# ucla-mobility/QuantV2X

Measured on AMD Instinct MI355X. Metric: frames/sec/node (N-agent int8 BEV fusion), higher is better.
Workload: dtype i8

## Files before the change

### include/qv2x.h

```cpp
#ifndef QV2X_H
#define QV2X_H

#include <stdint.h>

#ifdef __cplusplus
extern "C" {
#endif
#if defined(__GNUC__) || defined(__clang__)
#pragma GCC visibility push(default)
#endif

#define QV2X_OK 0
#define QV2X_EINVAL (-1)
#define QV2X_EALIGN (-2)
#define QV2X_MAX_GROUPS 4

const char* qv2x_last_error(void);
#define QV2X_ABI_VERSION 9
int qv2x_version(void);

int qv2x_fill_i8(int8_t* buf, int64_t bytes, int value, void* stream);

int64_t qv2x_voxelize_workspace_bytes(int n_points);
int qv2x_voxelize_f32(const float* points, int n_points, const float* lidar_range, const float* voxel_size, int agent,
                      int max_points, int max_voxels, void* workspace, int64_t workspace_bytes,
                      float* voxel_features, int32_t* voxel_coords, int32_t* voxel_num_points, int32_t* n_voxels, void* stream);

int64_t qv2x_voxelize_batch_workspace_bytes(int n_sweeps, const int32_t* n_points );
int qv2x_voxelize_batch_f32(const float* const* points , const int32_t* n_points , int n_sweeps,
                            const float* lidar_range, const float* voxel_size, int first_agent, int max_points, int capacity,
                            void* workspace, int64_t workspace_bytes, float* voxel_features, int32_t* voxel_coords,
                            int32_t* voxel_num_points, int32_t* voxel_counts, void* stream);

typedef struct {
    float w[64 * 10];
    float b[64];
    float d1, z1, d2, z2;
    float vox[3], off[3];
} qv2x_pfn_params;
int qv2x_pfn_scatter_i8(const float* voxel_features, const int32_t* voxel_coords, const int32_t* voxel_num_points,
                        int M, int max_points, const qv2x_pfn_params* params ,
                        int8_t* canvas, int N, int ny, int nx, void* stream);
int qv2x_pfn_unscatter_i8(const int32_t* voxel_coords, int M, int value, int8_t* canvas, int N, int ny, int nx, void* stream);

typedef struct {
    int32_t n, h, w, cin_total, stride, cout;
    int32_t ngroups;
    int32_t group_c0[QV2X_MAX_GROUPS], group_c[QV2X_MAX_GROUPS], group_zx[QV2X_MAX_GROUPS];
    int32_t out_ctotal, out_c0;
    int32_t relu;
    float out_delta, out_zp;
} qv2x_conv_desc;
int qv2x_conv3x3_i8(const qv2x_conv_desc* desc , const int8_t* in, const int8_t* w,
                    const float* scale, const int32_t* corr, const int32_t* aw, const float* bias,
                    int8_t* out, void* stream);

int qv2x_conv3x3_i8_wide_ok(const qv2x_conv_desc* desc );
int qv2x_conv3x3_i8_pack_wide(const qv2x_conv_desc* desc , const int8_t* w, int8_t* w_wide, void* stream);
int qv2x_conv3x3_i8_wide(const qv2x_conv_desc* desc , const int8_t* in, const int8_t* w_wide,
                         const float* scale, const int32_t* corr, const int32_t* aw, const float* bias,
                         int8_t* out, void* stream);

typedef struct {
    int32_t n, h, w;
    int32_t in_h, in_w;
    int32_t depth, stride0, relu;
    float out_delta[4], out_zp[4];
} qv2x_chain_desc;
int qv2x_conv3x3_i8_chain64(const qv2x_chain_desc* desc , const int8_t* in, const int8_t* w_chain,
                            const float* scale, const int32_t* corr, const int32_t* aw, const float* bias,
                            int8_t* out, void* stream);

typedef struct {
    int32_t n, h, w, cin, cout, s;
    int32_t in_zx;
    float in_delta;
    int32_t out_ctotal, out_c0, relu;
    float out_delta, out_zp;
    int32_t out_h, out_w;
} qv2x_deconv_desc;
int qv2x_deconv_i8(const qv2x_deconv_desc* desc , const int8_t* in, const float* w, const float* bias,
                   int8_t* out, void* stream);

int qv2x_deconv_i8_batch(const qv2x_deconv_desc* descs , int n, const int8_t* const* ins ,
                         const float* const* ws, const float* const* biases, int8_t* const* outs, void* stream);

typedef struct {
    int32_t n, h, w;
    int32_t levels, kc;
    int32_t in_zx;
    float in_delta;
    int32_t segs;
} qv2x_encode_desc;
int64_t qv2x_codebook_level_floats(int kc);
int qv2x_codebook_c2_f32(const float* codebook, int kc, float* c2, void* stream);
int qv2x_codebook_encode_f32(const qv2x_encode_desc* desc , const int8_t* in,
                             const float* const* level_weights ,
                             uint8_t* codes, void* stream);
int qv2x_codebook_encode_wave_f32(const qv2x_encode_desc* desc , const int8_t* in, const float* in_f32,
                                  const float* const* level_weights , uint8_t* codes, void* stream);

int qv2x_codebook_encode_collapsed_f32(const qv2x_encode_desc* desc , const int8_t* in, const float* g_packed, const float* bias,
                                       const float* tables, uint8_t* codes, void* stream);

int qv2x_codebook_encode_candidates_i8(const qv2x_encode_desc* desc , const int8_t* in, const int8_t* g_limbs, const double* bias_packed,
                                       const int32_t* tables, const float* tau , uint8_t* codes, uint32_t* list, uint32_t* counters,
                                       void* stream);
int qv2x_codebook_encode_listed_f32(const qv2x_encode_desc* desc , const int8_t* in, const float* const* level_weights ,
                                    const uint32_t* list, const uint32_t* list_count, uint8_t* codes, void* stream);

int qv2x_codebook_encode_candidates_seg_i8(const qv2x_encode_desc* desc , const int8_t* in, const int8_t* g_limbs, const double* bias_packed,
                                           const int32_t* tables, const float* tau , uint8_t* codes, uint32_t* list, uint32_t* counters,
                                           void* stream);

typedef struct {
    int32_t agents, h, w, levels, kc;
    int32_t max_cav, ego;
    int64_t code_agent_stride, code_level_stride;
    double h_metres, w_metres, discrete_ratio;
    int32_t fusion;
} qv2x_fuse_desc;
int qv2x_fuse_att_f32(const qv2x_fuse_desc* desc , const uint8_t* codes, const float* lut, const float* lut_bias,
                      const float* feats, const double* pairwise, float* fused, void* stream);

int qv2x_fuse_att_batch_f32(const qv2x_fuse_desc* desc , int n_scenes, const int64_t* scene_offset ,
                            const int32_t* scene_agents , const uint8_t* codes, const float* lut, const float* lut_bias,
                            const float* feats, const double* pairwise, float* fused, void* stream);

int qv2x_decode_lut_f32(const uint8_t* codes, int R, int levels, int kc, const float* lut, const float* lut_bias,
                        float* out, void* stream);

int qv2x_dequant_i8_f32(const int8_t* in, int n, int h, int w, int c, int zp, float delta, float* out, void* stream);

int qv2x_heads_f32(const float* x, int R, int hw, int cout, int cout_pad, const float* w, const float* bias,
                   const float* da, const float* za, float* out, void* stream);

int qv2x_fuse_heads_batch_f32(const qv2x_fuse_desc* desc , int n_scenes, const int64_t* scene_offset ,
                              const int32_t* scene_agents , const uint8_t* codes, const float* lut, const float* lut_bias,
                              const float* feats, const double* pairwise, int cout, int cout_pad, const float* w, const float* bias,
                              const float* da, const float* za, float* out, float* fused_tap, void* stream);

int qv2x_table_heads_f32(const uint8_t* codes, int R, int hw, int levels, int kc, int c0, int c1, const float* tables,
                         const float* bias, const float* da, const float* za, float* out0, float* out1, void* stream);

int qv2x_decode_heads_f32(const uint8_t* codes, int R, int hw, int levels, int kc, const float* lut, const float* lut_bias,
                          int cout, int cout_pad, const float* w, const float* bias, const float* da, const float* za,
                          float* out, void* stream);

int qv2x_single_heads_lut_f32(const uint8_t* codes, int R, int hw, int levels, int kc, int cout, const float* tables,
                              const float* bias, const float* da, const float* za, float* out, void* stream);

int qv2x_heads_pair_f32(const float* x, int R, int hw, int cout, int cout_pad, const float* w, const float* bias,
                        const float* da, const float* za, float* out,
                        const uint8_t* codes, int R1, int levels, int kc, const float* lut, const float* lut_bias,
                        int cout1, int cout_pad1, const float* w1, const float* bias1, const float* da1,
                        const float* za1, float* out1, void* stream);

typedef struct {
    int32_t h, w, anchors_per_cell, num_bins;
    float score_threshold, nms_threshold, dir_offset;
    float range[6];
    float transform[16];
    int32_t max_boxes;
    int32_t num_classes;
    int32_t range_xy_only;
    float max_extent, z_min, z_max;
} qv2x_postprocess_desc;
int64_t qv2x_postprocess_workspace_bytes(const qv2x_postprocess_desc* desc );
int qv2x_postprocess_f32(const qv2x_postprocess_desc* desc , const float* cls, const float* reg, const float* dir,
                         const float* anchors, void* workspace, int64_t workspace_bytes, float* out_corners,
                         float* out_scores, int32_t* out_labels, int32_t* out_count, void* stream);

int64_t qv2x_postprocess_batch_workspace_bytes(const qv2x_postprocess_desc* desc , int frames);
int qv2x_postprocess_batch_f32(const qv2x_postprocess_desc* desc , int frames, const float* cls, int64_t cls_frame_stride,
                               const float* reg, int64_t reg_frame_stride, const float* dir, int64_t dir_frame_stride,
                               const float* anchors, const float* transforms , void* workspace, int64_t workspace_bytes,
                               float* out_corners, float* out_scores, int32_t* out_labels, int32_t* out_count, void* stream);

int64_t qv2x_postprocess_late_workspace_bytes(const qv2x_postprocess_desc* desc , int ncav);
int qv2x_postprocess_late_f32(const qv2x_postprocess_desc* desc , int ncav, const float* const* cls, const float* const* reg,
                              const float* const* dir, const float* const* anchors, const float* transforms , void* workspace,
                              int64_t workspace_bytes, float* out_corners, float* out_scores, int32_t* out_labels, int32_t* out_count,
                              void* stream);

typedef struct {
    int32_t n, h, w;
    int32_t cin_total, cin0, cin;
    int32_t stride;
    int32_t cout;
    int32_t out_ctotal, out_c0, relu;
} qv2x_f32conv_desc;
int qv2x_conv3x3_f32(const qv2x_f32conv_desc* desc , const float* in, const float* w, const float* bias, float* out, void* stream);
int qv2x_deconv_f32(const qv2x_f32conv_desc* desc , const float* in, const float* w, const float* bias, float* out, void* stream);
int qv2x_pfn_scatter_f32(const float* voxel_features, const int32_t* voxel_coords, const int32_t* voxel_num_points, int M, int max_points,
                         const float* w, const float* b, const float* vox, const float* off, float* canvas, int N, int ny, int nx, void* stream);
int qv2x_codebook_encode_f32in(const qv2x_encode_desc* desc , const float* in, const float* const* level_weights ,
                               uint8_t* codes, void* stream);

int qv2x_pyramid_weighted_fuse_f32(const qv2x_fuse_desc* desc , int channels, const float* feats, const float* score,
                                   const double* pairwise, float* out, void* stream);


typedef struct {
    int32_t n, h, w, cin, cout, stride;
    int32_t mode, relu;
    int32_t out_ctotal, out_c0;
    float out_delta, out_zp;
    int32_t res_zx;
    float res_delta;
} qv2x_conv1x1_desc;
int qv2x_conv1x1_i8(const qv2x_conv1x1_desc* desc , const int8_t* in, const int8_t* w_frag, const float* scale,
                    const int32_t* corr, const int32_t* aw, const float* bias, const void* res, void* out, void* stream);

typedef struct {
    int32_t n, h, w, c, cg, stride, relu;
    float out_delta, out_zp;
} qv2x_gconv_desc;
int qv2x_gconv3x3_i8(const qv2x_gconv_desc* desc , const int8_t* in, const int8_t* w_frag, const float* scale,
                     const int32_t* corr, const int32_t* aw, const float* bias, int8_t* out, void* stream);

typedef struct {
    int32_t n, h, w, planes, width, cg;
    int32_t in_zx;
    float in_delta;
    float delta1, zp1, delta2, zp2, out_delta, out_zp;
} qv2x_bottleneck_desc;
int qv2x_bottleneck_i8(const qv2x_bottleneck_desc* desc , const int8_t* x, const int8_t* const* w, const float* const* scale,
                       const int32_t* const* corr, const int32_t* const* aw, const float* const* bias, int8_t* out, void* stream);

int qv2x_conv3x3_i8_res(const qv2x_conv_desc* desc , const int8_t* in, const int8_t* w, const float* scale, const int32_t* corr,
                        const int32_t* aw, const float* bias, int res_mode, const void* res, int res_zx, float res_delta,
                        int8_t* out, void* stream);

int qv2x_deconv_f32in(const qv2x_deconv_desc* desc , const float* in, const float* w, const float* bias, int8_t* out, void* stream);

int qv2x_codebook_decode_f32(const uint8_t* codes, int64_t agent_stride, int64_t level_stride, int agents, int hw, int levels,
                             int kc, int d, const float* lut, const float* bias, float* out, void* stream);

int64_t qv2x_codebook64_level_floats(int kc);
int qv2x_codebook64_c2_f32(const float* codebook, int kc, float* c2, void* stream);
int qv2x_codebook_encode64_f32(const qv2x_encode_desc* desc , int cin_total, const int8_t* in,
                               const float* const* level_weights , uint8_t* codes, void* stream);

int qv2x_codebook_encode64_f32in(const qv2x_encode_desc* desc , int cin_total, const float* in,
                                 const float* const* level_weights , uint8_t* codes, void* stream);

int qv2x_add_relu_f32(const float* a, const float* b, float* out, int64_t count, void* stream);
int qv2x_occ_sigmoid_f32(const float* in, int n, int h, int w, int c_total, float* occ, float* score, void* stream);
int qv2x_pyramid_weighted_fuse_f32p(const qv2x_fuse_desc* desc , int channels, const float* feats, const float* score,
                                    const double* pairwise, float* out, void* stream);

typedef struct {
    int32_t n, h, w, c;
    int32_t aw, corr;
    float scale, bias, out_delta, out_zp;
} qv2x_occ_desc;
int qv2x_occ_score_i8(const qv2x_occ_desc* desc , const int8_t* in, const int8_t* w, const float* score_lut, float* score,
                      uint8_t* occ_code, void* stream);

int qv2x_pyramid_weighted_fuse_i8(const qv2x_fuse_desc* desc , int channels, const int8_t* feats, int in_zx, float in_delta,
                                  const float* score, const double* pairwise, float* out, void* stream);

typedef struct {
    int32_t subm;
    int32_t k[3], s[3], p[3];
    int32_t in_shape[3], out_shape[3];
    int32_t agents, cin, cout;
    int32_t cap_in, cap_out;
    float out_delta, out_zp;
} qv2x_spconv_desc;
int qv2x_mean_vfe_f32(const float* voxel_features, const int32_t* voxel_num_points, const int32_t* n_voxels , int cap,
                      int max_points, float* out, void* stream);
int qv2x_sp_index_scatter(const int32_t* coords, const int32_t* n_rows , int cap, int agents, int D, int H, int W,
                          int32_t* volume, int set, void* stream);
int64_t qv2x_sp_out_sites_workspace_bytes(const qv2x_spconv_desc* desc );
int qv2x_sp_out_sites(const qv2x_spconv_desc* desc , const int32_t* in_coords, const int32_t* n_in, int32_t* out_volume,
                      int32_t* out_coords, int32_t* n_out, void* workspace, int64_t workspace_bytes, void* stream);
int qv2x_sp_rulebook(const qv2x_spconv_desc* desc , const int32_t* out_coords, const int32_t* n_out, const int32_t* in_volume,
                     int32_t* nbr, void* stream);
int qv2x_sp_conv_f32in(const qv2x_spconv_desc* desc , const float* feat, const int32_t* nbr, const int32_t* n_out, const float* w,
                       const float* bn_g, const float* bn_h, int8_t* out, void* stream);
int qv2x_sp_conv_i8(const qv2x_spconv_desc* desc , const int8_t* in, const int32_t* nbr, const int32_t* n_out, const int8_t* w_frag,
                    const float* scale, const int32_t* corr, const int32_t* aw, const float* bn_g, const float* bn_h, int8_t* out, void* stream);
int qv2x_sp_to_bev_i8(const int8_t* feat, const int32_t* coords, const int32_t* n_rows , int cap, int c, int c_padded, int agents,
                      int D, int H, int W, int fill, int8_t* bev, void* stream);

#define QV2X_COMM_ID_BYTES 128
int qv2x_comm_unique_id(void* id );
int qv2x_comm_init(const void* id , int world, int rank, void** comm);
int qv2x_comm_destroy(void* comm);
int qv2x_allgather_codes(void* comm, const uint8_t* send, uint8_t* recv, int64_t bytes_per_rank, void* stream);

int qv2x_pairwise_from_poses_f64(const uint8_t* gathered, int world, int64_t agent_stride_bytes, int64_t pose_offset_bytes,
                                 int max_cav, double* pairwise, void* stream);
int qv2x_pairwise_from_poses_batch_f64(const uint8_t* gathered, int world, int64_t agent_stride_bytes, int64_t pose_offset_bytes,
                                       int frames, int64_t frame_stride_bytes, int max_cav, double* pairwise, void* stream);

#define QV2X_WIRE_F32 0
#define QV2X_WIRE_U8 1
int qv2x_fuse_att_band_f32(const qv2x_fuse_desc* desc , int n_scenes, const int64_t* scene_offset ,
                           const int32_t* scene_agents , const uint8_t* codes, const float* lut, const float* lut_bias,
                           const float* feats, const double* pairwise, int64_t cell0, int64_t n_cells, float* fused, void* stream);
int qv2x_heads_band(const float* x, int n_scenes, int64_t n_cells, int cout, int cout_pad, const float* w, const float* bias,
                    const float* da, const float* za, int wire, const float* da_host , void* out, void* stream);
int qv2x_fuse_heads_band(const qv2x_fuse_desc* desc , int n_scenes, const int64_t* scene_offset ,
                         const int32_t* scene_agents , const uint8_t* codes, const float* lut, const float* lut_bias,
                         const float* feats, const double* pairwise, int64_t cell0, int64_t n_cells, int cout, int cout_pad,
                         const float* w, const float* bias, const float* da, const float* za, int wire, const float* da_host ,
                         void* out, float* fused_tap, void* stream);
int qv2x_assemble_bands(const uint8_t* slabs, int world, int64_t slab_bytes, int frames, int cout, int h, int w, int wire,
                        const float* da, const float* za, float* out, void* stream);

typedef struct {
    int32_t frames;
    int32_t det_cap;
    int32_t gt_cap;
    int32_t n_classes;
    int32_t n_ranges;
    int32_t n_thresholds;
    float ranges[4][2];
    float thresholds[4];
} qv2x_eval_desc;
int64_t qv2x_eval_workspace_bytes(const qv2x_eval_desc* desc );
int qv2x_eval_tp_fp_f32(const qv2x_eval_desc* desc , const float* det_corners, const float* det_scores, const int32_t* det_labels,
                        const int32_t* det_count, const float* gt_corners, const int32_t* gt_labels, const int32_t* gt_count,
                        void* workspace, int64_t workspace_bytes, int32_t* out_order, float* out_scores, uint8_t* out_flags,
                        int32_t* out_match, int32_t* out_gt, void* stream);

typedef struct {
    int32_t frames;
    int32_t agents;
    int32_t obj_cap;
    int32_t gt_cap;
    int32_t row_floats;
    int32_t order;
    int32_t mode;
    int32_t range_xy_only;
    float range[6];
    float iou_threshold;
} qv2x_gt_desc;
int qv2x_gt_boxes_f32(const qv2x_gt_desc* desc , const float* boxes, const uint8_t* mask, const int32_t* ids, const float* transforms,
                      const int32_t* agent_counts, float* gt_corners, int32_t* gt_labels, int32_t* gt_ids, int32_t* gt_counts,
                      int32_t* gt_totals, void* stream);

typedef struct {
    int32_t channels;
    int32_t candidates;
    int32_t n_levels;
    int32_t reserved;
    int64_t per_channel;
} qv2x_range_search_desc;
int64_t qv2x_range_search_workspace_bytes(const qv2x_range_search_desc* desc );
int qv2x_range_search_f32(const qv2x_range_search_desc* desc , const float* x, const float* delta, const float* zp, double* loss,
                          int32_t* best, void* workspace, void* stream);

#define QV2X_LSS_LOGITS 0
#define QV2X_LSS_PROBS 1
typedef struct {
    int32_t samples;
    int32_t views;
    int32_t depth_bins;
    int32_t fh, fw;
    int32_t features;
    int32_t nx[3];
    float dx[3], bx[3];
} qv2x_lss_desc;
int64_t qv2x_lss_workspace_bytes(const qv2x_lss_desc* desc );
int qv2x_lss_plan_f32(const qv2x_lss_desc* desc , const float* frustum, const float* rots, const float* trans, const float* intrins,
                      const float* post_rots, const float* post_trans, int32_t* cells_out, void* workspace, void* stream);
int qv2x_lss_splat_f32(const qv2x_lss_desc* desc , const float* depth, const float* feats, int mode, void* workspace, float* out,
                       void* stream);

typedef struct {
    int32_t views;
    int32_t h, w;
    int32_t reserved;
    int64_t view_stride;
    float out_delta, out_zp;
} qv2x_cam_stem_desc;
int qv2x_cam_stem_f32(const qv2x_cam_stem_desc* desc , const float* img, const float* wdeq, const float* bias, int8_t* out,
                      void* stream);

typedef struct {
    int32_t views;
    int32_t h, w;
    int32_t cin;
    int32_t depth_bins, features;
    float depth_delta, depth_zp;
    float feat_delta, feat_zp;
} qv2x_cam_heads_desc;
int qv2x_cam_heads_i8(const qv2x_cam_heads_desc* desc , const int8_t* in, const int8_t* w_frag, const float* scale,
                      const int32_t* corr, const int32_t* aw, const float* bias, float* depth, float* feats, void* stream);

#if defined(__GNUC__) || defined(__clang__)
#pragma GCC visibility pop
#endif
#ifdef __cplusplus
}
#endif
#endif
```

### quantv2x_amd/csrc/codebook_encode.h

```cpp
#pragma once
#include "common.h"

namespace qv2x {

constexpr int ENC_D = 256;
constexpr int ENC_WAVE_PAD = 16 * 256;

struct EncArgs {
    const int8_t* in; const float* in_f32; uint8_t* codes;
    const float* lvl[4];
    int n, h, w, levels, kc, ax, M;
    int segs, ke;
    float dx;
    int m_lo, m_hi;
    int list_slots = 1, list_tail_max = 0;
    const unsigned* list = nullptr; const unsigned* list_count = nullptr;
};

__device__ __host__ __forceinline__ int64_t level_floats_wg(int kc) { return 3LL * (ENC_D * ENC_D + ENC_D) + (int64_t)ENC_D * kc + (int64_t)kc * ENC_D + kc; }
__device__ __host__ __forceinline__ int64_t level_floats(int kc) { return level_floats_wg(kc) + 3LL * ENC_D * ENC_D + (int64_t)((kc + 63) / 64 * 64) * ENC_D + ENC_WAVE_PAD; }

struct ListPlan { int n[3], first[3], total, full; };
__device__ __forceinline__ ListPlan list_plan(const EncArgs& a) {
    ListPlan p;
    int t = 0;
#pragma unroll
    for (int c = 0; c < 3; ++c) { p.n[c] = (int)a.list_count[1 + c]; p.first[c] = t; t += (p.n[c] + 31) >> 5; }
    p.total = t;
    const int full = t / a.list_slots * a.list_slots;
    p.full = t - full > a.list_tail_max ? t : full;
    return p;
}
__device__ __forceinline__ void list_tile(const ListPlan& p, int tile, int& cls, int& i0) {
    cls = tile >= p.first[2] ? 2 : (tile >= p.first[1] ? 1 : 0);
    i0 = (tile - p.first[cls]) * 32;
}

int encode_wave_launch(const EncArgs& a, hipStream_t st);
int encode_wave_list_launch(const EncArgs& a, int waves, hipStream_t st);

}
```

### quantv2x_amd/csrc/codebook_encode.hip

```cpp
#include <cstdlib>

#include <atomic>

#include "codebook_encode.h"

namespace qv2x {

#ifdef QV2X_ENC_TRACE
__device__ unsigned long long g_enc_blk[4096][4];
#endif
#ifdef QV2X_ENC_FINE
__device__ long long g_enc_fine[2048][40];
#define EFINE(k) do { if (threadIdx.x == 0 && blockIdx.x < 2048) g_enc_fine[blockIdx.x][12 * l + (k)] = __builtin_amdgcn_s_memtime(); } while (0)
#else
#define EFINE(k) do { } while (0)
#endif

constexpr int LDF = 258;
__device__ __forceinline__ int kpos(int c) { return (c & ~3) | ((c & 1) << 1) | ((c >> 1) & 1); }
constexpr int D = 256;
#ifndef QV2X_ENC_LDS_PAD
#define QV2X_ENC_LDS_PAD 0
#endif

__device__ __forceinline__ void lds_barrier() {
    asm volatile("s_waitcnt lgkmcnt(0)" ::: "memory");
    __builtin_amdgcn_s_barrier();
}


struct GemmHead { float2 s0[4]; float b; };
__device__ __forceinline__ GemmHead gemm_head(const float2* __restrict__ wp, const float* __restrict__ bias, int wave, int lane) {
    const int par = lane >> 5, col = wave * 32 + (lane & 31);
    GemmHead h;
    h.b = bias[col];
    const float2* wl = wp + (size_t)col * 2 + par;
#pragma unroll
    for (int t = 0; t < 4; ++t) h.s0[t] = wl[(size_t)t * D * 2];
    return h;
}

template <int ERT>
__device__ __forceinline__ void gemm_rows_x32(const float* __restrict__ src, const float2* __restrict__ wp, const GemmHead& head,
                                              int wave, int lane, v16f (&acc)[ERT]) {
    const int par = lane >> 5, col = wave * 32 + (lane & 31);
    const float b = head.b;
#pragma unroll
    for (int i = 0; i < ERT; ++i)
#pragma unroll
        for (int r = 0; r < 16; ++r) acc[i][r] = b;
    const float2* wl = wp + (size_t)col * 2 + par;
    const float* al = src + (lane & 31) * LDF + 2 * par;
    auto loadB = [&](float2 (&dst)[4], int q0) {
#pragma unroll
        for (int t = 0; t < 4; ++t) dst[t] = wl[(size_t)(q0 + t) * D * 2];
    };
    auto compute4 = [&](const float2 (&bset)[4], int q0) {
        float2 av[4][ERT];
#pragma unroll
        for (int t = 0; t < 4; ++t)
#pragma unroll
            for (int i = 0; i < ERT; ++i) av[t][i] = *(const float2*)(al + i * 32 * LDF + (q0 + t) * 4);
#pragma unroll
        for (int t = 0; t < 4; ++t) {
#pragma unroll
            for (int i = 0; i < ERT; ++i) acc[i] = __builtin_amdgcn_mfma_f32_32x32x2f32(av[t][i].x, bset[t].x, acc[i], 0, 0, 0);
#pragma unroll
            for (int i = 0; i < ERT; ++i) acc[i] = __builtin_amdgcn_mfma_f32_32x32x2f32(av[t][i].y, bset[t].y, acc[i], 0, 0, 0);
        }
    };
    float2 s0[4], s1[4];
#pragma unroll
    for (int t = 0; t < 4; ++t) s0[t] = head.s0[t];
    for (int q0 = 0; q0 < 64; q0 += 8) {
        loadB(s1, q0 + 4);
        __builtin_amdgcn_sched_barrier(0);
        compute4(s0, q0);
        __builtin_amdgcn_sched_barrier(0);
        loadB(s0, q0 + 8);
        __builtin_amdgcn_sched_barrier(0);
        compute4(s1, q0 + 4);
        __builtin_amdgcn_sched_barrier(0);
    }
}

__device__ __forceinline__ unsigned long long dist_key(float d, int code) {
    unsigned b = __builtin_bit_cast(unsigned, d);
    b ^= (unsigned)((int)b >> 31) | 0x80000000u;
    return ((unsigned long long)b << 32) | (unsigned)code;
}

template <int ERT>
__device__ __forceinline__ void store_tile(float* __restrict__ dst, int wave, int lane, const v16f (&acc)[ERT]) {
#pragma unroll
    for (int i = 0; i < ERT; ++i)
#pragma unroll
        for (int r = 0; r < 16; ++r)
            dst[(i * 32 + mfma32_row(r, lane)) * LDF + kpos(wave * 32 + (lane & 31))] = acc[i][r];
}

constexpr int ENC_MAX_TILES = 16;
template <int ER> constexpr int enc_smem_floats() { return 2 * ER * LDF + 4 * ER + 4 * ER + 2 * ENC_MAX_TILES * ER + 4 * ER + QV2X_ENC_LDS_PAD; }

template <int ER, bool EXT, bool LIST = false>
__device__ __forceinline__ void encode_rows(const EncArgs& a, const int m0, float* __restrict__ smem, const unsigned* __restrict__ lst = nullptr,
                                            const int n_listed = 0, const int start = 0) {
    constexpr int ERT = ER / 32;
    const int segs = EXT ? a.segs : 1;
    float* bufA = smem;
    float* bufB = smem + ER * LDF;
    float* x2 = smem + 2 * ER * LDF;
    float* pval = x2 + 4 * ER;
    unsigned long long* pkey = (unsigned long long*)(pval + 4 * ER);
    int* code_s = (int*)(pkey + ENC_MAX_TILES * ER);

    const int tid = threadIdx.x, lane = tid & 63, wave = tid >> 6;
#ifdef QV2X_ENC_TRACE
    const unsigned long long t_start = __builtin_readcyclecounter();
    unsigned hwid, xcc;
    asm volatile("s_getreg_b32 %0, hwreg(HW_REG_HW_ID)" : "=s"(hwid));
    asm volatile("s_getreg_b32 %0, hwreg(HW_REG_XCC_ID)" : "=s"(xcc));
#endif
    {
        constexpr int TPR = 512 / ER;
        constexpr int CPT = D / TPR;
        const int row = tid / TPR, part = tid % TPR;
        int m = m0 + row;
        if (LIST) m = (int)lst[m < n_listed ? m : n_listed - 1];
        m = m < a.M ? m : a.M - 1;
        const int img = m / (a.h * a.w), rem = m - img * (a.h * a.w);
        const int y = rem / a.w, x = rem - y * a.w;
        const size_t pixel = (size_t)(img * (a.h + 2) + y + 1) * (a.w + 2) + x + 1;
        const int8_t* src = a.in + pixel * D + part * CPT;
        if (a.in_f32) {
            const float* sf = a.in_f32 + pixel * D + part * CPT;
#pragma unroll
            for (int c = 0; c < CPT / 4; ++c) {
                const v4f v = *(const v4f*)(sf + c * 4);
#pragma unroll
                for (int e = 0; e < 4; ++e) bufA[row * LDF + kpos(part * CPT + c * 4 + e)] = v[e];
            }
        } else
#pragma unroll
        for (int c = 0; c < CPT / 16; ++c) {
            const v4i raw = *(const v4i*)(src + c * 16);
#pragma unroll
            for (int e = 0; e < 16; ++e) {
                const int xs = (raw[e >> 2] << (24 - (e & 3) * 8)) >> 24;
                bufA[row * LDF + kpos(part * CPT + c * 16 + e)] = (float)(xs + a.ax) * a.dx;
            }
        }
    }
    GemmHead head = gemm_head((const float2*)a.lvl[0], a.lvl[0] + D * D, wave, lane);
    lds_barrier();

    v16f acc[ERT];
    for (int l = 0; l < a.levels; ++l) {
        const float* W = a.lvl[l];
        const float* stage_w = W;
        const float* stage_b = stage_w + D * D;
        const float* qhead_w = stage_b + D;
        const float* qhead_b = qhead_w + D * D;
        const float* lhead_w = qhead_b + D;
        const float* lhead_b = lhead_w + D * D;
        const float* cbp = lhead_b + D;
        const float* cb = cbp + (size_t)D * a.ke;
        const float* c2 = cb + (size_t)a.ke * D;

        EFINE(0);
        gemm_rows_x32(bufA, (const float2*)stage_w, head, wave, lane, acc);
        EFINE(1);
        const bool proven = LIST && l < start;
        if (proven) {
            head = gemm_head((const float2*)lhead_w, lhead_b, wave, lane);
            store_tile(bufB, wave, lane, acc);
            if (tid < ER * segs) {
                const int sg = tid / ER, r = tid - sg * ER;
                code_s[tid] = sg * a.kc + (int)a.codes[((size_t)l * segs + sg) * a.M + lst[m0 + r < n_listed ? m0 + r : n_listed - 1]];
            }
            lds_barrier();
        } else {
        head = gemm_head((const float2*)qhead_w, qhead_b, wave, lane);
        store_tile(bufB, wave, lane, acc);
        lds_barrier();
        EFINE(2);
        gemm_rows_x32(bufB, (const float2*)qhead_w, head, wave, lane, acc);
        EFINE(3);
        if (l + 1 < a.levels) head = gemm_head((const float2*)lhead_w, lhead_b, wave, lane);
        store_tile(bufA, wave, lane, acc);
        lds_barrier();
        EFINE(4);

        if (tid < ER * 4) {
            const int row = tid % ER, part = tid / ER;
            const float2* qr = (const float2*)(bufA + row * LDF + part * 64);
            float s = 0.0f;
#pragma unroll 4
            for (int j = 0; j < 16; ++j) {
                const float2 e = qr[2 * j], o = qr[2 * j + 1];
                s = fmaf(e.x, e.x, s); s = fmaf(o.x, o.x, s); s = fmaf(e.y, e.y, s); s = fmaf(o.y, o.y, s);
            }
            pval[part * ER + row] = s;
        }
        constexpr int TPR = 8 / ERT;
        const int ct0 = wave % TPR, rt = wave / TPR;
        const int ntile = (a.ke + 31) >> 5;
        float2 dhead[4];
        float c2v = 0.0f;
        if (ct0 < ntile) {
            const int code = ct0 * 32 + (lane & 31);
            const float2* cl = (const float2*)cbp + (size_t)code * 2 + (lane >> 5);
#pragma unroll
            for (int t = 0; t < 4; ++t) dhead[t] = cl[(size_t)t * a.ke * 2];
            c2v = c2[code];
        }
        lds_barrier();
        EFINE(5);
        if (tid < ER) {
            const float p0 = pval[tid], p1 = pval[ER + tid], p2 = pval[2 * ER + tid], p3 = pval[3 * ER + tid];
            if (segs == 1) x2[tid] = (p0 + p1) + (p2 + p3);
            else if (segs == 2) { x2[tid] = p0 + p1; x2[ER + tid] = p2 + p3; }
            else { x2[tid] = p0; x2[ER + tid] = p1; x2[2 * ER + tid] = p2; x2[3 * ER + tid] = p3; }
        }
        lds_barrier();
        EFINE(6);

#pragma unroll 1
        for (int ct = ct0; ct < ntile; ct += EXT ? TPR : ENC_MAX_TILES) {
            const int par = lane >> 5, code = ct * 32 + (lane & 31);
            v16f dacc;
#pragma unroll
            for (int r = 0; r < 16; ++r) dacc[r] = 0.0f;
            const float2* cl = (const float2*)cbp + (size_t)code * 2 + par;
            const float* al = bufA + (rt * 32 + (lane & 31)) * LDF + 2 * par;
            auto loadC = [&](float2 (&dst)[4], int q0) {
#pragma unroll
                for (int t = 0; t < 4; ++t) dst[t] = cl[(size_t)(q0 + t) * a.ke * 2];
            };
            auto dist4 = [&](const float2 (&bset)[4], int q0) {
                float2 av[4];
#pragma unroll
                for (int t = 0; t < 4; ++t) av[t] = *(const float2*)(al + (q0 + t) * 4);
#pragma unroll
                for (int t = 0; t < 4; ++t) {
                    dacc = __builtin_amdgcn_mfma_f32_32x32x2f32(av[t].x, bset[t].x, dacc, 0, 0, 0);
                    dacc = __builtin_amdgcn_mfma_f32_32x32x2f32(av[t].y, bset[t].y, dacc, 0, 0, 0);
                }
            };
            float2 s0[4], s1[4];
            if (ct == ct0) {
#pragma unroll
                for (int t = 0; t < 4; ++t) s0[t] = dhead[t];
            } else {
                loadC(s0, 0);
                c2v = c2[code];
            }
            for (int q0 = 0; q0 < 64; q0 += 8) {
                loadC(s1, q0 + 4);
                __builtin_amdgcn_sched_barrier(0);
                dist4(s0, q0);
                __builtin_amdgcn_sched_barrier(0);
                loadC(s0, q0 + 8);
                __builtin_amdgcn_sched_barrier(0);
                dist4(s1, q0 + 4);
                __builtin_amdgcn_sched_barrier(0);
            }
            EFINE(7);
            unsigned resk = 0xffffffffu;
            int resc = 0;
            const int l31 = lane & 31, hi = lane >> 5;
            const float* x2r = x2 + (segs == 1 ? 0 : (ct * 32) / a.kc) * ER;
#pragma unroll
            for (int r = 0; r < 16; ++r) {
                const int row = rt * 32 + mfma32_row(r, lane);
                const float d = (x2r[row] + c2v) - 2.0f * dacc[r];
                unsigned b = __builtin_bit_cast(unsigned, d);
                b ^= (unsigned)((int)b >> 31) | 0x80000000u;
                unsigned m = b, o;
                o = (unsigned)__builtin_amdgcn_update_dpp((int)m, (int)m, 0xB1, 0xf, 0xf, false); m = o < m ? o : m;
                o = (unsigned)__builtin_amdgcn_update_dpp((int)m, (int)m, 0x4E, 0xf, 0xf, false); m = o < m ? o : m;
                o = (unsigned)__builtin_amdgcn_update_dpp((int)m, (int)m, 0x141, 0xf, 0xf, false); m = o < m ? o : m;
                o = (unsigned)__builtin_amdgcn_update_dpp((int)m, (int)m, 0x140, 0xf, 0xf, false); m = o < m ? o : m;
                const auto sw = __builtin_amdgcn_permlane16_swap(m, m, false, false);
                m = sw[0] < sw[1] ? sw[0] : sw[1];
                const unsigned long long eq = __builtin_amdgcn_ballot_w64(b == m);
                const int c_lo = __builtin_ctz((unsigned)eq), c_hi = __builtin_ctz((unsigned)(eq >> 32));
                const int c = hi ? c_hi : c_lo;
                const bool mine = l31 == r;
                resk = mine ? m : resk;
                resc = mine ? c : resc;
            }
            if (l31 < 16) pkey[ct * ER + rt * 32 + mfma32_row(l31, lane)] = ((unsigned long long)resk << 32) | (unsigned)(ct * 32 + resc);
        }
        lds_barrier();
        EFINE(8);
        if (tid < ER) {
            const int tps = segs == 1 ? ntile : a.kc >> 5;
            for (int sg = 0; sg < segs; ++sg) {
                unsigned long long bk = pkey[(sg * tps) * ER + tid];
                for (int wv = 1; wv < tps; ++wv) {
                    const unsigned long long ok = pkey[(sg * tps + wv) * ER + tid];
                    bk = ok < bk ? ok : bk;
                }
                const int bi = (int)(unsigned)bk;
                code_s[sg * ER + tid] = bi;
                if (LIST) {
                    if (m0 + tid < n_listed) a.codes[((size_t)l * segs + sg) * a.M + lst[m0 + tid]] = (uint8_t)(bi - sg * a.kc);
                } else if (m0 + tid < a.m_hi) a.codes[((size_t)l * segs + sg) * a.M + m0 + tid] = (uint8_t)(bi - sg * a.kc);
            }
        }
        lds_barrier();
        EFINE(9);
        }

        if (l + 1 < a.levels) {
            const int col = wave * 32 + (lane & 31);
            const int* cs = code_s + ((wave * segs) >> 3) * ER;
            float cv[ERT][16];
#pragma unroll
            for (int i = 0; i < ERT; ++i)
#pragma unroll
                for (int r = 0; r < 16; ++r) cv[i][r] = cb[(size_t)cs[i * 32 + mfma32_row(r, lane)] * D + col];
            gemm_rows_x32(bufB, (const float2*)lhead_w, head, wave, lane, acc);
            EFINE(10);
            head = gemm_head((const float2*)a.lvl[l + 1], a.lvl[l + 1] + D * D, wave, lane);
#pragma unroll
            for (int i = 0; i < ERT; ++i)
#pragma unroll
                for (int r = 0; r < 16; ++r) bufA[(i * 32 + mfma32_row(r, lane)) * LDF + kpos(col)] = acc[i][r] - cv[i][r];
            lds_barrier();
            EFINE(11);
        }
    }
#ifdef QV2X_ENC_TRACE
    if (tid == 0 && blockIdx.x < 4096) {
        g_enc_blk[blockIdx.x][0] = t_start; g_enc_blk[blockIdx.x][1] = __builtin_readcyclecounter();
        g_enc_blk[blockIdx.x][2] = hwid; g_enc_blk[blockIdx.x][3] = xcc;
    }
#endif
}

template <int ER, bool EXT = false>
__global__ __launch_bounds__(512, ER == 32 ? 4 : 2) void codebook_encode_kernel(const EncArgs a) {
    __shared__ __attribute__((aligned(16))) float smem[enc_smem_floats<ER>()];
    encode_rows<ER, EXT>(a, a.m_lo + blockIdx.x * ER, smem);
}

template <bool EXT>
__global__ __launch_bounds__(512, 2) void codebook_encode_list_tail_kernel(const EncArgs a) {
    __shared__ __attribute__((aligned(16))) float smem[enc_smem_floats<32>()];
    const ListPlan plan = list_plan(a);
    for (int t = plan.full + (int)blockIdx.x; t < plan.total; t += (int)gridDim.x) {
        int cls, i0;
        list_tile(plan, t, cls, i0);
        encode_rows<32, EXT, true>(a, i0, smem, a.list + (size_t)cls * a.M, plan.n[cls], cls);
        __syncthreads();
    }
}

template <bool EXT>
__global__ __launch_bounds__(512, 2) void codebook_encode_mixed_kernel(const EncArgs a, const int n64) {
    __shared__ __attribute__((aligned(16))) float smem[enc_smem_floats<64>()];
    if ((int)blockIdx.x < n64) encode_rows<64, EXT>(a, a.m_lo + blockIdx.x * 64, smem);
    else encode_rows<32, EXT>(a, a.m_lo + n64 * 64 + ((int)blockIdx.x - n64) * 32, smem);
}

__global__ void codebook_c2_kernel(const float* __restrict__ cb, int kc, float* __restrict__ c2) {
    const int k = blockIdx.x * blockDim.x + threadIdx.x;
    if (k >= kc) return;
    float s[4];
    for (int q = 0; q < 4; ++q) {
        float acc = 0.0f;
        for (int i = 0; i < 64; ++i) { const float v = cb[(size_t)k * D + q * 64 + i]; acc = fmaf(v, v, acc); }
        s[q] = acc;
    }
    c2[k] = (s[0] + s[1]) + (s[2] + s[3]);
}

}

extern "C" int qv2x_codebook_c2_f32(const float* codebook, int kc, float* c2, void* stream) {
    using namespace qv2x;
    if (!codebook || !c2 || kc <= 0) return fail(QV2X_EINVAL, "qv2x_codebook_c2_f32: bad arguments");
    codebook_c2_kernel<<<(kc + 63) / 64, 64, 0, (hipStream_t)stream>>>(codebook, kc, c2);
    return hip_check(hipGetLastError(), "qv2x_codebook_c2_f32 launch");
}

extern "C" int64_t qv2x_codebook_level_floats(int kc) { return qv2x::level_floats(kc); }

static int encode_launch(const qv2x_encode_desc* d, const int8_t* in, const float* in_f32, const float* const* level_weights, uint8_t* codes, void* stream,
                         int form = 0);

extern "C" int qv2x_codebook_encode_wave_f32(const qv2x_encode_desc* d, const int8_t* in, const float* in_f32, const float* const* level_weights,
                                             uint8_t* codes, void* stream) {
    if (!in && !in_f32) return qv2x::fail(QV2X_EINVAL, "qv2x_codebook_encode_wave_f32: null pointer");
    return encode_launch(d, in_f32 ? (const int8_t*)in_f32 : in, in_f32, level_weights, codes, stream, 1);
}

extern "C" int qv2x_codebook_encode_f32(const qv2x_encode_desc* d, const int8_t* in, const float* const* level_weights,
                                        uint8_t* codes, void* stream) {
    return encode_launch(d, in, nullptr, level_weights, codes, stream);
}

extern "C" int qv2x_codebook_encode_f32in(const qv2x_encode_desc* d, const float* in, const float* const* level_weights,
                                          uint8_t* codes, void* stream) {
    if (!in) return qv2x::fail(QV2X_EINVAL, "qv2x_codebook_encode_f32in: null pointer");
    return encode_launch(d, (const int8_t*)in, in, level_weights, codes, stream);
}

extern "C" int qv2x_codebook_encode_listed_f32(const qv2x_encode_desc* d, const int8_t* in, const float* const* level_weights,
                                               const uint32_t* list, const uint32_t* list_count, uint8_t* codes, void* stream) {
    using namespace qv2x;
    if (!d || !in || !level_weights || !codes || !list || !list_count) return fail(QV2X_EINVAL, "qv2x_codebook_encode_listed_f32: null pointer");
    if (d->n <= 0 || d->h <= 0 || d->w <= 0 || d->levels < 1 || d->levels > 4) return fail(QV2X_EINVAL, "qv2x_codebook_encode_listed_f32: bad shape");
    const int segs = d->segs ? d->segs : 1;
    if (segs != 1 && segs != 2) return fail(QV2X_EINVAL, "qv2x_codebook_encode_listed_f32: seg_num 1 or 2 (got %d)", d->segs);
    if (d->kc < 32 || d->kc > 256 || d->kc % 32 || (segs > 1 && d->kc % 64) || segs * d->kc > 32 * ENC_MAX_TILES)
        return fail(QV2X_EINVAL, "qv2x_codebook_encode_listed_f32: dict_size must be a multiple of 32 up to 256 (of 64 with two segments): got %d x %d", segs, d->kc);
    if ((uintptr_t)in & 15) return fail(QV2X_EALIGN, "qv2x_codebook_encode_listed_f32: in must be 16-byte aligned");
    EncArgs a;
    a.in = in; a.in_f32 = nullptr; a.codes = codes; a.n = d->n; a.h = d->h; a.w = d->w; a.levels = d->levels; a.kc = d->kc;
    a.segs = segs; a.ke = segs * d->kc;
    const bool ext = segs > 1 || a.ke > 128;
    a.ax = 128 - d->in_zx; a.dx = d->in_delta; a.M = d->n * d->h * d->w; a.m_lo = 0; a.m_hi = a.M;
    a.list = list; a.list_count = list_count;
    for (int l = 0; l < 4; ++l) {
        a.lvl[l] = l < d->levels ? level_weights[l] : nullptr;
        if (l < d->levels && (!a.lvl[l] || ((uintptr_t)a.lvl[l] & 15))) return fail(QV2X_EALIGN, "qv2x_codebook_encode_listed_f32: level %d weights null or unaligned", l);
    }
    int cus = 256, dev = 0, v = 0;
    if (hipGetDevice(&dev) == hipSuccess && hipDeviceGetAttribute(&v, hipDeviceAttributeMultiprocessorCount, dev) == hipSuccess && v > 0) cus = v;
    const int tiles = (a.M + 31) / 32;
    int tail_knob = 0;
#ifdef QV2X_DEV_KNOBS
    static const int tail_env = getenv("QV2X_LIST_TAIL") ? atoi(getenv("QV2X_LIST_TAIL")) : 0;
    tail_knob = tail_env;
#endif
    a.list_slots = 4 * cus; a.list_tail_max = tail_knob > 0 ? tail_knob : 2 * cus;
    const int grid_tail = 2 * cus;
    if (tiles + 3 >= 2 * a.list_slots) {
        if (int rc = encode_wave_list_launch(a, a.list_slots, (hipStream_t)stream)) return rc;
    } else {
        a.list_slots = 1 << 30; a.list_tail_max = 1 << 30;
    }
    if (ext) codebook_encode_list_tail_kernel<true><<<tiles < grid_tail ? tiles : grid_tail, 512, 0, (hipStream_t)stream>>>(a);
    else codebook_encode_list_tail_kernel<false><<<tiles < grid_tail ? tiles : grid_tail, 512, 0, (hipStream_t)stream>>>(a);
    return hip_check(hipGetLastError(), "qv2x_codebook_encode_listed_f32 launch");
}

static int encode_launch(const qv2x_encode_desc* d, const int8_t* in, const float* in_f32, const float* const* level_weights, uint8_t* codes, void* stream,
                         int form) {
    using namespace qv2x;
    if (!d || !in || !level_weights || !codes) return fail(QV2X_EINVAL, "qv2x_codebook_encode_f32: null pointer");
    if (d->n <= 0 || d->h <= 0 || d->w <= 0 || d->levels < 1 || d->levels > 4) return fail(QV2X_EINVAL, "qv2x_codebook_encode_f32: bad shape");
    const int segs = d->segs ? d->segs : 1;
    if (segs != 1 && segs != 2 && segs != 4) return fail(QV2X_EINVAL, "qv2x_codebook_encode_f32: seg_num must be 1, 2 or 4 (got %d)", d->segs);
    if (d->kc < 32 || d->kc > 256 || d->kc % 32 || (segs > 1 && d->kc % 64) || segs * d->kc > 32 * ENC_MAX_TILES)
        return fail(QV2X_EINVAL, "qv2x_codebook_encode_f32: dict_size must be a multiple of 32 up to 256 (of 64 with seg_num > 1; seg_num * dict_size <= %d): "
                                 "got dict_size %d, seg_num %d", 32 * ENC_MAX_TILES, d->kc, segs);
    if ((uintptr_t)in & 15) return fail(QV2X_EALIGN, "qv2x_codebook_encode_f32: in must be 16-byte aligned");
    EncArgs a;
    a.in = in; a.in_f32 = in_f32; a.codes = codes; a.n = d->n; a.h = d->h; a.w = d->w; a.levels = d->levels; a.kc = d->kc;
    a.segs = segs; a.ke = segs * d->kc;
    const bool ext = segs > 1 || a.ke > 128;
    a.ax = 128 - d->in_zx; a.dx = d->in_delta; a.M = d->n * d->h * d->w; a.m_lo = 0; a.m_hi = a.M;
    for (int l = 0; l < 4; ++l) {
        a.lvl[l] = l < d->levels ? level_weights[l] : nullptr;
        if (l < d->levels && (!a.lvl[l] || ((uintptr_t)a.lvl[l] & 15))) return fail(QV2X_EALIGN, "qv2x_codebook_encode_f32: level %d weights null or unaligned", l);
    }
    int er_env = 0;
#ifdef QV2X_DEV_KNOBS
    static const int er_knob = [] { const char* e = getenv("QV2X_ENC_ROWS"); return e ? atoi(e) : 0; }();
    if (er_knob != 0 && er_knob != 32 && er_knob != 64 && er_knob != 96) return fail(QV2X_EINVAL, "QV2X_ENC_ROWS=%d: 32, 64 or 96", er_knob);
    er_env = er_knob;
#endif
    static std::atomic<int> cus_of[64];
    int cus = 256, dev = 0, v = 0;
    if (hipGetDevice(&dev) == hipSuccess && dev >= 0 && dev < 64) {
        cus = cus_of[dev].load(std::memory_order_relaxed);
        if (cus == 0) {
            cus = (hipDeviceGetAttribute(&v, hipDeviceAttributeMultiprocessorCount, dev) == hipSuccess && v > 0) ? v : 256;
            cus_of[dev].store(cus, std::memory_order_relaxed);
        }
    }
    hipStream_t st = (hipStream_t)stream;
    if (form == 1) return encode_wave_launch(a, st);
    const int slots = 4 * cus, waves = (a.M + 31) / 32;
    const int rounds = waves / slots, rest = waves - rounds * slots;
    int tail_max = 2 * cus;
#ifdef QV2X_DEV_KNOBS
    static const int tail_knob = [] { const char* e = getenv("QV2X_ENC_TAIL"); return e ? atoi(e) : -1; }();
    if (tail_knob >= 0) tail_max = tail_knob;
#endif
    if (er_env == 0 && rounds >= 1) {
        if (rest == 0 || rest > tail_max) return encode_wave_launch(a, st);
        EncArgs main = a, tail = a;
        main.m_hi = rounds * slots * 32;
        tail.m_lo = main.m_hi;
        if (int rc = encode_wave_launch(main, st)) return rc;
        if (ext) codebook_encode_kernel<32, true><<<rest, 512, 0, st>>>(tail);
        else codebook_encode_kernel<32><<<rest, 512, 0, st>>>(tail);
        return hip_check(hipGetLastError(), "qv2x_codebook_encode_f32 launch");
    }
    const int n64 = (a.M / 64) / cus * cus;
    const int er = er_env ? er_env : (n64 > 0 ? 96 : 32);
    if (er == 64) {
        if (ext) codebook_encode_kernel<64, true><<<(a.M + 63) / 64, 512, 0, st>>>(a);
        else codebook_encode_kernel<64><<<(a.M + 63) / 64, 512, 0, st>>>(a);
    } else if (er == 96 && n64 > 0) {
        if (ext) codebook_encode_mixed_kernel<true><<<n64 + (a.M - n64 * 64 + 31) / 32, 512, 0, st>>>(a, n64);
        else codebook_encode_mixed_kernel<false><<<n64 + (a.M - n64 * 64 + 31) / 32, 512, 0, st>>>(a, n64);
    } else if (ext) {
        codebook_encode_kernel<32, true><<<(a.M + 31) / 32, 512, 0, st>>>(a);
    } else {
        codebook_encode_kernel<32><<<(a.M + 31) / 32, 512, 0, st>>>(a);
    }
    return hip_check(hipGetLastError(), "qv2x_codebook_encode_f32 launch");
}

#ifdef QV2X_ENC_FINE
extern "C" __attribute__((visibility("default"))) int qv2x_debug_encode_fine(long long* host, int n) {
    return hipMemcpyFromSymbol(host, HIP_SYMBOL(qv2x::g_enc_fine), (size_t)n * 40 * sizeof(long long)) == hipSuccess ? 0 : -1;
}
#endif
#ifdef QV2X_ENC_TRACE
extern "C" __attribute__((visibility("default"))) int qv2x_debug_encode_blocks(unsigned long long* host, int n) {
    return (int)hipMemcpyFromSymbol(host, HIP_SYMBOL(qv2x::g_enc_blk), (size_t)n * 4 * sizeof(unsigned long long));
}
#endif
```

### quantv2x_amd/csrc/codebook_encode_cand.hip

```cpp
#include "common.h"

namespace qv2x {
namespace {

struct CandArgs {
    const int8_t* in; const int8_t* gpack; const double* bias; const int* tables;
    uint8_t* codes; unsigned* list; unsigned* counters;
    float tau[3][3];
    int n, h, w, hw, M, levels, kc, ke, zx, gbytes, tbytes;
    float delta;
};

constexpr int NPF = 8;
constexpr int LIMBS = 3;
template <int V> struct IC { static constexpr int value = V; };

__device__ __forceinline__ double shfl_xor_f64(double v, int m) {
    const long long b = __builtin_bit_cast(long long, v);
    const int lo = __shfl_xor((int)b, m), hi = __shfl_xor((int)(b >> 32), m);
    return __builtin_bit_cast(double, ((long long)hi << 32) | (unsigned)lo);
}

template <int CT, int SEGS, int PACK>
__global__ __launch_bounds__(256) __attribute__((amdgpu_waves_per_eu(1, 1))) void encode_candidates_kernel(const CandArgs a) {
    const int lane = threadIdx.x & 63, wave = __builtin_amdgcn_readfirstlane(threadIdx.x >> 6), j = lane & 31, hf = lane >> 5;
    const int m0 = ((int)blockIdx.x * 4 + wave) * (32 * CT);

    v4i xb[CT][8];
    int m[CT];
    float n0[CT], n1[CT];
#pragma unroll
    for (int ct = 0; ct < CT; ++ct) {
        m[ct] = m0 + 32 * ct + j;
        const int mc = m[ct] < a.M ? m[ct] : a.M - 1;
        const int img = mc / a.hw, rem = mc - img * a.hw, y = rem / a.w, x = rem - y * a.w;
        const int8_t* px = a.in + ((size_t)(img * (a.h + 2) + y + 1) * (a.w + 2) + x + 1) * 256 + 16 * hf;
#pragma unroll
        for (int s = 0; s < 8; ++s) xb[ct][s] = *(const v4i*)(px + 32 * s);
        unsigned s1 = 0, s2 = 0, sad = 0;
        const unsigned zx4 = (unsigned)a.zx * 0x01010101u;
#pragma unroll
        for (int s = 0; s < 8; ++s)
#pragma unroll
            for (int d = 0; d < 4; ++d) {
                const unsigned u = (unsigned)xb[ct][s][d] ^ 0x80808080u;
                s1 = __builtin_amdgcn_udot4(u, 0x01010101u, s1, false);
                s2 = __builtin_amdgcn_udot4(u, u, s2, false);
                sad = __builtin_amdgcn_sad_u8(u, zx4, sad);
            }
        s1 += __shfl_xor(s1, 32); s2 += __shfl_xor(s2, 32); sad += __shfl_xor(sad, 32);
        const int n2 = (int)s2 - 2 * a.zx * (int)s1 + 256 * a.zx * a.zx;
        n0[ct] = a.delta * sqrtf((float)n2);
        n1[ct] = (float)sad;
    }

    const __amdgpu_buffer_rsrc_t grs = __builtin_amdgcn_make_buffer_rsrc((void*)a.gpack, 0, a.gbytes, 0x00020000);
    int wo = 0;
    const int loff = lane * 16;
    auto gload = [&](int f) __attribute__((always_inline)) { return (v4i)__builtin_amdgcn_raw_buffer_load_b128(grs, loff, wo + f * 1024, 0); };
    v4i ring[NPF];
#pragma unroll
    for (int i = 0; i < NPF; ++i) ring[i] = gload(i);

    const __amdgpu_buffer_rsrc_t brs = __builtin_amdgcn_make_buffer_rsrc((void*)a.bias, 0, a.levels * a.ke * 8, 0x00020000);
    const __amdgpu_buffer_rsrc_t trs = __builtin_amdgcn_make_buffer_rsrc((void*)a.tables, 0, a.tbytes, 0x00020000);
    int o[2][SEGS][CT] = {};
    int first[CT];
#pragma unroll
    for (int ct = 0; ct < CT; ++ct) first[ct] = 3;
    const int ntile = a.kc >> 5;
    const int tsz = a.ke * a.ke;
    auto level = [&](auto lc) __attribute__((always_inline)) {
        constexpr int l = decltype(lc)::value;
        bool weak_l[CT];
#pragma unroll
        for (int ct = 0; ct < CT; ++ct) weak_l[ct] = false;
        auto segment = [&](auto sc) __attribute__((always_inline)) {
        constexpr int sg = decltype(sc)::value;
        double best[CT], second[CT];
#pragma unroll
        for (int ct = 0; ct < CT; ++ct) best[ct] = second[ct] = 1.0e300;
        v4i qb[2][2], qt[2][l > 0 ? l * SEGS : 1][CT];
        auto issue = [&](int T, int g, int slot) __attribute__((always_inline)) {
            const int col = sg * a.kc + 32 * T + 8 * g;
            const int kofs = l * a.ke + col;
            qb[slot][0] = (v4i)__builtin_amdgcn_raw_buffer_load_b128(brs, 32 * hf, kofs * 8, 0);
            qb[slot][1] = (v4i)__builtin_amdgcn_raw_buffer_load_b128(brs, 32 * hf + 16, kofs * 8, 0);
#pragma unroll
            for (int ct = 0; ct < CT; ++ct) {
#pragma unroll
                for (int jj = 0; jj < l; ++jj)
#pragma unroll
                    for (int sp = 0; sp < SEGS; ++sp)
                        qt[slot][jj * SEGS + sp][ct] = (v4i)__builtin_amdgcn_raw_buffer_load_b128(trs, o[jj][sp][ct], ((l * (l - 1) / 2 + jj) * tsz + col) * 4, 0);
            }
        };
#pragma unroll 1
        for (int T = 0; T < ntile; ++T) {
            v16i acc[LIMBS][CT];
#pragma unroll
            for (int lb = 0; lb < LIMBS; ++lb)
#pragma unroll
                for (int ct = 0; ct < CT; ++ct)
#pragma unroll
                    for (int r = 0; r < 16; ++r) acc[lb][ct][r] = 0;
#pragma unroll
            for (int f = 0; f < LIMBS * 8; ++f) {
                const v4i A = ring[f % NPF];
#pragma unroll
                for (int ct = 0; ct < CT; ++ct) acc[f >> 3][ct] = __builtin_amdgcn_mfma_i32_32x32x32_i8(A, xb[ct][f & 7], acc[f >> 3][ct], 0, 0, 0);
                ring[f % NPF] = gload(f + NPF);
                if (f == LIMBS * 8 - 6) issue(T, 0, 0);
                __builtin_amdgcn_sched_barrier(0);
            }
            wo += LIMBS * 8 * 1024;
#pragma unroll
            for (int g = 0; g < 4; ++g) {
                if (g < 3) issue(T, g + 1, (g + 1) & 1);
                __builtin_amdgcn_sched_barrier(0);
                const int sl = g & 1;
                double b[4];
                b[0] = __builtin_bit_cast(double, ((unsigned long long)(unsigned)qb[sl][0][1] << 32) | (unsigned)qb[sl][0][0]);
                b[1] = __builtin_bit_cast(double, ((unsigned long long)(unsigned)qb[sl][0][3] << 32) | (unsigned)qb[sl][0][2]);
                b[2] = __builtin_bit_cast(double, ((unsigned long long)(unsigned)qb[sl][1][1] << 32) | (unsigned)qb[sl][1][0]);
                b[3] = __builtin_bit_cast(double, ((unsigned long long)(unsigned)qb[sl][1][3] << 32) | (unsigned)qb[sl][1][2]);
#pragma unroll
                for (int ct = 0; ct < CT; ++ct) {
#pragma unroll
                    for (int e = 0; e < 4; ++e) {
                        const int r = 4 * g + e;
                        int lo = (acc[1][ct][r] << 8) + acc[0][ct][r];
#pragma unroll
                        for (int q = 0; q < l * SEGS; ++q) lo += qt[sl][q][ct][e];
                        double c = __builtin_fma((double)lo, (double)PACK, b[e]);
                        c = __builtin_fma((double)acc[2][ct][r], 65536.0 * PACK, c);
                        second[ct] = fmin(second[ct], fmax(best[ct], c));
                        best[ct] = fmin(best[ct], c);
                    }
                }
                __builtin_amdgcn_sched_barrier(0);
            }
        }
#pragma unroll
        for (int ct = 0; ct < CT; ++ct) {
            const double ob = shfl_xor_f64(best[ct], 32), os = shfl_xor_f64(second[ct], 32);
            const double nb = fmin(best[ct], ob), ns = fmin(fmax(best[ct], ob), fmin(second[ct], os));
            const int c = (int)((long long)nb & (PACK - 1));
            if (l < 2) o[l < 2 ? l : 0][sg][ct] = ((sg * a.kc + c) * a.ke + 4 * hf) * 4;
            const float t = ((a.tau[l][0] + a.tau[l][1] * n0[ct]) + (a.tau[l][2] * n0[ct]) * n0[ct]) + n1[ct];
            weak_l[ct] |= !(ns - nb > (double)PACK * (double)ceilf(t) + (double)(PACK - 1));
            if (hf == 0 && m[ct] < a.M) a.codes[(size_t)(l * SEGS + sg) * a.M + m[ct]] = (uint8_t)c;
        }
        };
        segment(IC<0>{});
        if constexpr (SEGS > 1) segment(IC<1>{});
#pragma unroll
        for (int ct = 0; ct < CT; ++ct)
            if (weak_l[ct] && first[ct] == 3) first[ct] = l;
    };
    level(IC<0>{});
    if (a.levels > 1) level(IC<1>{});
    if (a.levels > 2) level(IC<2>{});
    unsigned long long mask[3][CT];
    unsigned cnt[3] = {0, 0, 0};
#pragma unroll
    for (int c = 0; c < 3; ++c)
#pragma unroll
        for (int ct = 0; ct < CT; ++ct) {
            mask[c][ct] = __builtin_amdgcn_ballot_w64(first[ct] == c && hf == 0 && m[ct] < a.M);
            cnt[c] += (unsigned)__builtin_popcountll(mask[c][ct]);
        }
    __shared__ unsigned wcnt[4][3], wbase[3];
    if (lane == 0) { wcnt[wave][0] = cnt[0]; wcnt[wave][1] = cnt[1]; wcnt[wave][2] = cnt[2]; }
    __syncthreads();
    if (threadIdx.x < 3) {
        const unsigned tot = wcnt[0][threadIdx.x] + wcnt[1][threadIdx.x] + wcnt[2][threadIdx.x] + wcnt[3][threadIdx.x];
        wbase[threadIdx.x] = tot ? atomicAdd(a.counters + 1 + threadIdx.x, tot) : 0u;
        if (tot) atomicAdd(a.counters, tot);
    }
    __syncthreads();
    unsigned base[3];
#pragma unroll
    for (int c = 0; c < 3; ++c) {
        base[c] = wbase[c];
        for (int w2 = 0; w2 < wave; ++w2) base[c] += wcnt[w2][c];
    }
#pragma unroll
    for (int c = 0; c < 3; ++c) {
        unsigned at = __builtin_amdgcn_readfirstlane(base[c]);
#pragma unroll
        for (int ct = 0; ct < CT; ++ct) {
            if (first[ct] == c && hf == 0 && m[ct] < a.M)
                a.list[(size_t)c * a.M + at + (unsigned)__builtin_popcountll(mask[c][ct] & ((1ull << lane) - 1ull))] = (unsigned)m[ct];
            at += (unsigned)__builtin_popcountll(mask[c][ct]);
        }
    }
}

__global__ void zero_counters_kernel(unsigned* c) { if (threadIdx.x < 4) c[threadIdx.x] = 0; }

template <int CT, int SEGS, int PACK>
void launch(const CandArgs& a, hipStream_t st) {
    encode_candidates_kernel<CT, SEGS, PACK><<<(a.M + 128 * CT - 1) / (128 * CT), 256, 0, st>>>(a);
}

template <int PACK, int MAX_SEGS>
int candidates(const char* me, const qv2x_encode_desc* d, const int8_t* in, const int8_t* g_limbs, const double* bias_packed, const int32_t* tables,
               const float* tau, uint8_t* codes, uint32_t* list, uint32_t* counters, void* stream) {
    if (!d || !in || !g_limbs || !bias_packed || !tau || !codes || !list || !counters) return fail(QV2X_EINVAL, "%s: null pointer", me);
    if (d->n <= 0 || d->h <= 0 || d->w <= 0 || d->levels < 1 || d->levels > 3) return fail(QV2X_EINVAL, "%s: 1..3 levels", me);
    const int segs = d->segs ? d->segs : 1;
    if (segs < 1 || segs > MAX_SEGS) return fail(QV2X_EINVAL, "%s: seg_num 1 .. %d (got %d; the exact entry takes seg_num 1 | 2 | 4)", me, MAX_SEGS, d->segs);
    if (d->kc < 32 || d->kc > PACK || d->kc % 32 || (segs > 1 && d->kc % 64))
        return fail(QV2X_EINVAL, "%s: dict_size a multiple of 32 up to %d (of 64 with two segments; got %d x %d)", me, PACK, segs, d->kc);
    if (d->levels > 1 && !tables) return fail(QV2X_EINVAL, "%s: the residual levels need their tables", me);
    if (d->in_zx < 0 || d->in_zx > 255) return fail(QV2X_EINVAL, "%s: in_zx outside 0..255", me);
    if (((uintptr_t)in & 15) || ((uintptr_t)g_limbs & 15) || ((uintptr_t)tables & 15) || ((uintptr_t)bias_packed & 7))
        return fail(QV2X_EALIGN, "%s: 16-byte aligned maps, limbs and tables", me);
    CandArgs a;
    a.in = in; a.gpack = g_limbs; a.bias = bias_packed; a.tables = tables; a.codes = codes; a.list = list; a.counters = counters;
    for (int l = 0; l < 3; ++l)
        for (int i = 0; i < 3; ++i) a.tau[l][i] = l < d->levels ? tau[l * 3 + i] : 0.0f;
    a.n = d->n; a.h = d->h; a.w = d->w; a.hw = d->h * d->w; a.M = d->n * a.hw; a.levels = d->levels; a.kc = d->kc; a.ke = segs * d->kc; a.zx = d->in_zx;
    a.gbytes = d->levels * (a.ke / 32) * LIMBS * 8 * 1024;
    a.tbytes = (d->levels > 1 ? d->levels * (d->levels - 1) / 2 : 1) * a.ke * a.ke * 4;
    a.delta = d->in_delta;
    hipStream_t st = (hipStream_t)stream;
    zero_counters_kernel<<<1, 64, 0, st>>>(counters);
    int dev = 0, cus = 256, v = 0;
    if (hipGetDevice(&dev) == hipSuccess && hipDeviceGetAttribute(&v, hipDeviceAttributeMultiprocessorCount, dev) == hipSuccess && v > 0) cus = v;
    const bool large = a.M >= 4 * cus * 32 * (segs == 2 ? 3 : 4) * 2;
    if (segs == 1) large ? launch<4, 1, PACK>(a, st) : launch<2, 1, PACK>(a, st);
    else if constexpr (MAX_SEGS > 1) large ? launch<3, 2, PACK>(a, st) : launch<2, 2, PACK>(a, st);
    return hip_check(hipGetLastError(), me);
}

}
}

extern "C" int qv2x_codebook_encode_candidates_i8(const qv2x_encode_desc* d, const int8_t* in, const int8_t* g_limbs, const double* bias_packed,
                                                  const int32_t* tables, const float* tau, uint8_t* codes, uint32_t* list, uint32_t* counters,
                                                  void* stream) {
    return qv2x::candidates<128, 1>("qv2x_codebook_encode_candidates_i8", d, in, g_limbs, bias_packed, tables, tau, codes, list, counters, stream);
}

extern "C" int qv2x_codebook_encode_candidates_seg_i8(const qv2x_encode_desc* d, const int8_t* in, const int8_t* g_limbs, const double* bias_packed,
                                                      const int32_t* tables, const float* tau, uint8_t* codes, uint32_t* list, uint32_t* counters,
                                                      void* stream) {
    return qv2x::candidates<256, 2>("qv2x_codebook_encode_candidates_seg_i8", d, in, g_limbs, bias_packed, tables, tau, codes, list, counters, stream);
}
```

### quantv2x_amd/csrc/codebook_encode_wave.hip

```cpp
#include "codebook_encode.h"

namespace qv2x {

namespace {

constexpr int D = ENC_D;
constexpr int RS = 260;
constexpr int NPF = 4;

__device__ __forceinline__ v16f mfma(float a, float b, v16f c) { return __builtin_amdgcn_mfma_f32_32x32x2f32(a, b, c, 0, 0, 0); }


__device__ __forceinline__ void tile_to_lds(float* __restrict__ row, int h, int T, const v16f& acc) {
#pragma unroll
    for (int rq = 0; rq < 4; ++rq) {
        float* g = row + (4 * T + rq) * 8 + 2 * h;
        *(float2*)g = make_float2(acc[4 * rq], acc[4 * rq + 2]);
        *(float2*)(g + 4) = make_float2(acc[4 * rq + 1], acc[4 * rq + 3]);
    }
}

__device__ __forceinline__ void lds_to_operand(const float* __restrict__ row, int h, float (&m)[128]) {
#pragma unroll
    for (int g = 0; g < 32; ++g) {
        const v4f v = *(const v4f*)(row + g * 8 + 4 * h);
        m[4 * g] = v.x; m[4 * g + 1] = v.y; m[4 * g + 2] = v.z; m[4 * g + 3] = v.w;
    }
}

__device__ __forceinline__ void tile_vec(const float* __restrict__ p, int h, int T, v4f (&o)[4]) {
#pragma unroll
    for (int rq = 0; rq < 4; ++rq) o[rq] = *(const v4f*)(p + 32 * T + 8 * rq + 4 * h);
}

#ifdef QV2X_ENCW_FINE
__device__ long long g_encw_fine[4096][32];
#define WFINE(k) do { if (threadIdx.x == 0 && blockIdx.x < 4096) g_encw_fine[blockIdx.x][8 * l + (k)] = __builtin_readcyclecounter(); } while (0)
#define WFINE2(k) do { if (fine2 && threadIdx.x == 0 && blockIdx.x < 4096) g_encw_fine[blockIdx.x][24 + (k)] = __builtin_readcyclecounter(); } while (0)
#define WFINE2_ARM(v) fine2 = (v)
#else
#define WFINE(k) do { } while (0)
#define WFINE2(k) do { } while (0)
#define WFINE2_ARM(v) do { } while (0)
#endif

}

template <int V> struct IC { static constexpr int value = V; };

template <bool F32IN, int SEGS, bool LIST = false>
__global__ __attribute__((amdgpu_flat_work_group_size(64, 64), amdgpu_waves_per_eu(1, 1))) void codebook_encode_wave_kernel(const EncArgs a) {
    __shared__ __attribute__((aligned(16))) float smem[32 * RS];
    const int lane = threadIdx.x, j = lane & 31, h = lane >> 5;
    float* const row = smem + j * RS;
    ListPlan plan{};
    if (LIST) plan = list_plan(a);
#pragma unroll 1
    for (int round = 0; LIST ? round * (int)gridDim.x < plan.full : round == 0; ++round) {
    const int tile = LIST ? round * (int)gridDim.x + ((round & 1) ? (int)gridDim.x - 1 - (int)blockIdx.x : (int)blockIdx.x) : (int)blockIdx.x;
    if (LIST && tile >= plan.full) continue;
    int mrow;
    bool owned;
    int start = 0;
    if (LIST) {
        int cls, i0;
        list_tile(plan, tile, cls, i0);
        owned = i0 + j < plan.n[cls];
        mrow = (int)a.list[(size_t)cls * a.M + (owned ? i0 + j : plan.n[cls] - 1)];
        start = cls;
    } else {
        mrow = a.m_lo + tile * 32 + j;
        owned = mrow < a.m_hi;
    }

    float xq[128], z[128];
    {
        int m = mrow;
        m = m < a.M ? m : a.M - 1;
        const int img = m / (a.h * a.w), rem = m - img * (a.h * a.w);
        const int y = rem / a.w, x = rem - y * a.w;
        const size_t pixel = (size_t)(img * (a.h + 2) + y + 1) * (a.w + 2) + x + 1;
        if (F32IN) {
            const v4f* sf = (const v4f*)(a.in_f32 + pixel * D);
#pragma unroll
            for (int q = 0; q < 64; ++q) {
                const v4f v = sf[q];
                xq[2 * q] = h ? v.y : v.x;
                xq[2 * q + 1] = h ? v.w : v.z;
            }
        } else {
            const v4i* src = (const v4i*)(a.in + pixel * D);
            const float fax = (float)(a.ax - 128);
#pragma unroll
            for (int c = 0; c < 16; ++c) {
                const v4i raw = src[c];
#pragma unroll
                for (int d = 0; d < 4; ++d) {
                    const unsigned u = ((unsigned)raw[d] ^ 0x80808080u) >> (8 * h);
                    xq[8 * c + 2 * d] = ((float)(u & 0xffu) + fax) * a.dx;
                    xq[8 * c + 2 * d + 1] = ((float)((u >> 16) & 0xffu) + fax) * a.dx;
                }
            }
        }
    }

    for (int l = 0; l < a.levels; ++l) {
        const float* W = a.lvl[l];
        const float* stage_b = W + D * D;
        const float* qhead_b = stage_b + D + D * D;
        const float* lhead_b = qhead_b + D + D * D;
        const float* cb = lhead_b + D + (size_t)D * a.ke;
        const float* c2 = cb + (size_t)a.ke * D;
        const __amdgpu_buffer_rsrc_t wrs = __builtin_amdgcn_make_buffer_rsrc((void*)(W + level_floats_wg(a.ke)), 0, 0x7fffffff, 0x00020000);
        int wo = 0;
        const int loff = lane * 16;
        auto wload = [&](int grp) __attribute__((always_inline)) {
            return __builtin_bit_cast(v4f, __builtin_amdgcn_raw_buffer_load_b128(wrs, loff, wo + grp * 1024, 0));
        };
        const bool last = l + 1 == a.levels;
        const int npair = (a.ke + 63) >> 6;

        v4f bn[2][4];
        auto next_vec = [&](const float* p, int P) __attribute__((always_inline)) {
            tile_vec(p, h, 2 * P, bn[0]);
            tile_vec(p, h, 2 * P + 1, bn[1]);
        };
        auto next_c2 = [&](int P) __attribute__((always_inline)) {
            tile_vec(c2, h, 2 * P, bn[0]);
            if (64 * P + 32 < a.ke) tile_vec(c2, h, 2 * P + 1, bn[1]);
            else
#pragma unroll
                for (int i = 0; i < 4; ++i) bn[1][i] = v4f{INFINITY, INFINITY, INFINITY, INFINITY};
        };
        auto next_c2s = [&](int s0, int s1, int P) __attribute__((always_inline)) {
            tile_vec(c2 + s0 * a.kc, h, P, bn[0]);
            tile_vec(c2 + s1 * a.kc, h, P, bn[1]);
        };
        next_vec(stage_b, 0);
        __builtin_amdgcn_sched_barrier(0);
        v4f ring[2 * NPF];
#pragma unroll
        for (int i = 0; i < 2 * NPF; ++i) ring[i] = wload(i);
        __builtin_amdgcn_sched_barrier(0);

        v16f acc[2];
#ifdef QV2X_ENCW_FINE
        bool fine2 = false;
#endif
        auto tile2g = [&](const float (&m)[128], const bool biased, auto&& hook, auto ng_c, auto off0_c, auto off1_c) __attribute__((always_inline)) {
            constexpr int NG = decltype(ng_c)::value, OFF0 = decltype(off0_c)::value, OFF1 = decltype(off1_c)::value;
            WFINE2(0);
#pragma unroll
            for (int t = 0; t < 2; ++t)
#pragma unroll
                for (int r = 0; r < 16; ++r) acc[t][r] = biased ? bn[t][r >> 2][r & 3] : 0.0f;
            WFINE2(1);
#pragma unroll
            for (int g = 0; g < NG; ++g) {
                const v4f A0 = ring[(2 * g) % (2 * NPF)], A1 = ring[(2 * g + 1) % (2 * NPF)];
                acc[0] = mfma(A0.x, m[OFF0 + 4 * g], acc[0]);
                acc[1] = mfma(A1.x, m[OFF1 + 4 * g], acc[1]);
                __builtin_amdgcn_sched_barrier(0);
                acc[0] = mfma(A0.y, m[OFF0 + 4 * g + 1], acc[0]);
                acc[1] = mfma(A1.y, m[OFF1 + 4 * g + 1], acc[1]);
                __builtin_amdgcn_sched_barrier(0);
                acc[0] = mfma(A0.z, m[OFF0 + 4 * g + 2], acc[0]);
                acc[1] = mfma(A1.z, m[OFF1 + 4 * g + 2], acc[1]);
                __builtin_amdgcn_sched_barrier(0);
                acc[0] = mfma(A0.w, m[OFF0 + 4 * g + 3], acc[0]);
                acc[1] = mfma(A1.w, m[OFF1 + 4 * g + 3], acc[1]);
                if (g == NG - NPF - 1) hook();
                if (NG == 32 && g == 7) WFINE2(2);
                if (NG == 32 && g == 15) WFINE2(3);
                if (NG == 32 && g == 23) WFINE2(4);
#ifndef QV2X_ENCW_ABL_NOLOAD
                ring[(2 * g) % (2 * NPF)] = wload(2 * (g + NPF));
                ring[(2 * g + 1) % (2 * NPF)] = wload(2 * (g + NPF) + 1);
#endif
                __builtin_amdgcn_sched_barrier(0);
            }
#ifndef QV2X_ENCW_ABL_SAMEW
            wo += NG * 2048;
#endif
            WFINE2(5);
        };
        auto tile2 = [&](const float (&m)[128], const bool biased, auto&& hook) __attribute__((always_inline)) {
            tile2g(m, biased, hook, IC<32>{}, IC<0>{}, IC<0>{});
        };

        WFINE(0);
#pragma unroll 1
        for (int P = 0; P < 4; ++P) {
            WFINE2_ARM(l == 1 && P == 1);
            tile2(xq, true, [&]() __attribute__((always_inline)) { next_vec(P < 3 ? stage_b : qhead_b, P < 3 ? P + 1 : 0); });
            tile_to_lds(row, h, 2 * P, acc[0]);
            tile_to_lds(row, h, 2 * P + 1, acc[1]);
            WFINE2(6);
            WFINE2_ARM(false);
        }
        WFINE(1);
        lds_to_operand(row, h, z);
        WFINE(2);
        unsigned bcs = 0;
        if (LIST && l < start) {
            wo = SEGS == 1 ? (8 + npair) * 65536 : 8 * 65536 + (SEGS / 2) * (a.kc >> 5) * (32 / SEGS) * 2048;
            next_vec(lhead_b, 0);
#pragma unroll
            for (int i = 0; i < 2 * NPF; ++i) ring[i] = wload(i);
#pragma unroll
            for (int sg = 0; sg < SEGS; ++sg) bcs |= (unsigned)a.codes[((size_t)l * SEGS + sg) * a.M + mrow] << (8 * sg);
        } else {
#pragma unroll 1
        for (int P = 0; P < 4; ++P) {
            tile2(z, true, [&]() __attribute__((always_inline)) { if (P < 3) next_vec(qhead_b, P + 1); else if (SEGS == 1) next_c2(0); else next_c2s(0, 1, 0); });
            tile_to_lds(row, h, 2 * P, acc[0]);
            tile_to_lds(row, h, 2 * P + 1, acc[1]);
        }
        WFINE(3);
        lds_to_operand(row, h, xq);
        float x2s[4];
        {
            const float* qh = row + 128 * h;
            float p[2];
#pragma unroll
            for (int c = 0; c < 2; ++c) {
                float s = 0.0f;
#pragma unroll
                for (int g = 0; g < 8; ++g) {
                    const v4f e = *(const v4f*)(qh + (8 * c + g) * 8), o = *(const v4f*)(qh + (8 * c + g) * 8 + 4);
                    s = fmaf(e.x, e.x, s); s = fmaf(o.x, o.x, s); s = fmaf(e.y, e.y, s); s = fmaf(o.y, o.y, s);
                    s = fmaf(e.z, e.z, s); s = fmaf(o.z, o.z, s); s = fmaf(e.w, e.w, s); s = fmaf(o.w, o.w, s);
                }
                p[c] = s;
            }
            const float mine = p[0] + p[1];
            const float other = __shfl_xor(mine, 32);
            if (a.segs == 1) {
                x2s[0] = x2s[1] = x2s[2] = x2s[3] = mine + other;
            } else if (a.segs == 2) {
                x2s[0] = h ? other : mine; x2s[1] = h ? mine : other; x2s[2] = x2s[3] = 0.0f;
            } else {
                const float o0 = __shfl_xor(p[0], 32), o1 = __shfl_xor(p[1], 32);
                x2s[0] = h ? o0 : p[0]; x2s[1] = h ? o1 : p[1]; x2s[2] = h ? p[0] : o0; x2s[3] = h ? p[1] : o1;
            }
        }
        WFINE(4);
        if constexpr (SEGS == 1) {
        float best = INFINITY;
        int bc = 0;
        const int ppseg = npair / a.segs;
#pragma unroll 1
        for (int P = 0; P < npair; ++P) {
            const int seg = a.segs == 1 ? 0 : P / ppseg, cbase = seg * a.kc;
            const float x2 = seg == 0 ? x2s[0] : (seg == 1 ? x2s[1] : (seg == 2 ? x2s[2] : x2s[3]));
            v4f c2t[2][4];
#pragma unroll
            for (int t = 0; t < 2; ++t)
#pragma unroll
                for (int i = 0; i < 4; ++i) c2t[t][i] = bn[t][i];
            tile2(xq, false, [&]() __attribute__((always_inline)) { if (P + 1 < npair) next_c2(P + 1); else if (!last) next_vec(lhead_b, 0); });
#pragma unroll
            for (int t = 0; t < 2; ++t)
#pragma unroll
                for (int r = 0; r < 16; ++r) {
                    const float s = x2 + c2t[t][r >> 2][r & 3];
                    const float d = s - 2.0f * acc[t][r];
                    const int code = 64 * P + 32 * t + 8 * (r >> 2) + 4 * h + (r & 3) - cbase;
                    const bool lt = d < best;
                    best = lt ? d : best;
                    bc = lt ? code : bc;
                }
            if (a.segs == 1 ? P + 1 == npair : (P + 1) % ppseg == 0) {
                const float od = __shfl_xor(best, 32);
                const int oc = __shfl_xor(bc, 32);
                if (od < best || (od == best && oc < bc)) bc = oc;
                if (h == 0 && owned) a.codes[((size_t)l * a.segs + seg) * a.M + mrow] = (uint8_t)bc;
                bcs |= (unsigned)bc << (8 * seg);
                best = INFINITY; bc = 0;
            }
        }
        } else {
            const int ntile = a.kc >> 5;
            auto seg_pairs = [&](auto sa_c, auto sb_c, const bool more_after) __attribute__((always_inline)) {
                constexpr int SA = decltype(sa_c)::value, SB = decltype(sb_c)::value, NG = 32 / SEGS;
                float best[2] = {INFINITY, INFINITY};
                int bc[2] = {0, 0};
#pragma unroll 1
                for (int P = 0; P < ntile; ++P) {
                    v4f c2t[2][4];
#pragma unroll
                    for (int t = 0; t < 2; ++t)
#pragma unroll
                        for (int i = 0; i < 4; ++i) c2t[t][i] = bn[t][i];
                    tile2g(xq, false, [&]() __attribute__((always_inline)) {
                        if (P + 1 < ntile) next_c2s(SA, SB, P + 1);
                        else if (more_after) next_c2s(SA + 2, SB + 2, 0);
                        else if (!last) next_vec(lhead_b, 0);
                    }, IC<NG>{}, IC<4 * NG * SA>{}, IC<4 * NG * SB>{});
#pragma unroll
                    for (int t = 0; t < 2; ++t) {
                        const float x2 = x2s[t ? SB : SA];
#pragma unroll
                        for (int r = 0; r < 16; ++r) {
                            const float sv = x2 + c2t[t][r >> 2][r & 3];
                            const float d = sv - 2.0f * acc[t][r];
                            const int code = 32 * P + 8 * (r >> 2) + 4 * h + (r & 3);
                            const bool lt = d < best[t];
                            best[t] = lt ? d : best[t];
                            bc[t] = lt ? code : bc[t];
                        }
                    }
                }
#pragma unroll
                for (int t = 0; t < 2; ++t) {
                    const int seg = t ? SB : SA;
                    const float od = __shfl_xor(best[t], 32);
                    const int oc = __shfl_xor(bc[t], 32);
                    if (od < best[t] || (od == best[t] && oc < bc[t])) bc[t] = oc;
                    if (h == 0 && owned) a.codes[((size_t)l * SEGS + seg) * a.M + mrow] = (uint8_t)bc[t];
                    bcs |= (unsigned)bc[t] << (8 * seg);
                }
            };
            if constexpr (SEGS == 2) seg_pairs(IC<0>{}, IC<1>{}, false);
            else { seg_pairs(IC<0>{}, IC<1>{}, true); seg_pairs(IC<2>{}, IC<3>{}, false); }
        }
        }
        WFINE(5);
        if (last) break;
#pragma unroll 1
        for (int P = 0; P < 4; ++P) {
            const int seg = (P * a.segs) >> 2;
            const float* cw = cb + (size_t)(seg * a.kc + (int)((bcs >> (8 * seg)) & 0xffu)) * D;
            v4f cv[2][4];
            tile_vec(cw, h, 2 * P, cv[0]);
            tile_vec(cw, h, 2 * P + 1, cv[1]);
            __builtin_amdgcn_sched_barrier(0);
            tile2(z, true, [&]() __attribute__((always_inline)) { if (P < 3) next_vec(lhead_b, P + 1); });
#pragma unroll
            for (int t = 0; t < 2; ++t) {
#pragma unroll
                for (int r = 0; r < 16; ++r) acc[t][r] = acc[t][r] - cv[t][r >> 2][r & 3];
                tile_to_lds(row, h, 2 * P + t, acc[t]);
            }
        }
        WFINE(6);
        lds_to_operand(row, h, xq);
        WFINE(7);
    }
    }
}

int encode_wave_launch(const EncArgs& a, hipStream_t st) {
    const unsigned grid = (unsigned)((a.m_hi - a.m_lo + 31) / 32);
    if (a.segs == 2) {
        if (a.in_f32) codebook_encode_wave_kernel<true, 2><<<grid, 64, 0, st>>>(a);
        else codebook_encode_wave_kernel<false, 2><<<grid, 64, 0, st>>>(a);
    } else if (a.segs == 4) {
        if (a.in_f32) codebook_encode_wave_kernel<true, 4><<<grid, 64, 0, st>>>(a);
        else codebook_encode_wave_kernel<false, 4><<<grid, 64, 0, st>>>(a);
    } else if (a.in_f32) codebook_encode_wave_kernel<true, 1><<<grid, 64, 0, st>>>(a);
    else codebook_encode_wave_kernel<false, 1><<<grid, 64, 0, st>>>(a);
    return hip_check(hipGetLastError(), "qv2x_codebook_encode_f32 (wave form) launch");
}


int encode_wave_list_launch(const EncArgs& a, int waves, hipStream_t st) {
    if ((a.segs != 1 && a.segs != 2) || a.in_f32) return fail(QV2X_EINVAL, "qv2x_codebook_encode_listed_f32: seg_num 1 | 2, i8 rows");
    if (a.segs == 2) codebook_encode_wave_kernel<false, 2, true><<<(unsigned)waves, 64, 0, st>>>(a);
    else codebook_encode_wave_kernel<false, 1, true><<<(unsigned)waves, 64, 0, st>>>(a);
    return hip_check(hipGetLastError(), "qv2x_codebook_encode_listed_f32 launch");
}

}

#ifdef QV2X_ENCW_FINE
extern "C" __attribute__((visibility("default"))) int qv2x_debug_encw_fine(long long* host, int n) {
    return hipMemcpyFromSymbol(host, HIP_SYMBOL(qv2x::g_encw_fine), (size_t)n * 32 * sizeof(long long)) == hipSuccess ? 0 : -1;
}
#endif
```

### quantv2x_amd/encode_two_stage.py

```python
from typing import Dict

import numpy as np

U = 2.0 ** -24
LIMBS = 3
G_MAX_INT = 2 ** 23 - 2 ** 15 - 2 ** 7 - 1


def _sn(m):
    return float(np.linalg.norm(m, 2)) if m.size else 0.0


def _kappa(w, block=8):
    k = w.shape[1]
    return float(sum(min(block, k - i0) * _sn(w[:, :min(k, i0 + block)]) for i0 in range(0, k, block)))


class _Aff:

    def __init__(self, p=0.0, r=0.0):
        self.p, self.r = float(p), float(r)

    def __add__(self, o):
        return _Aff(self.p + o.p, self.r + o.r)

    def scale(self, c):
        return _Aff(self.p * c, self.r * c)


def encode_error_bound(state: Dict[str, np.ndarray], levels: int, delta: float, segs: int = 1):
    g = lambda l, n: state[f"codebook/{l}/{n}"].astype(np.float64)
    u1 = U / (1.0 - U)
    ub = u1 / (1.0 - 256.0 * u1)
    eye = np.eye(256)
    A, shift, back = eye.copy(), np.zeros(256), []
    srcs = [(eye.copy(), _Aff(U, 0.0), "x0 = fl(n * delta)")]
    ea, eb, ec, report = [], [], [], []

    def offset(shift, back):
        return float(np.linalg.norm(shift) + sum(sum(float(n.max()) for n in np.split(np.linalg.norm(g(j, "codebook") @ B.T, axis=1), segs))
                                                 for j, B in enumerate(back)))

    def norm_bound(A, shift, back, srcs):
        d = _Aff()
        for M, e, _ in srcs:
            d = d + e.scale(_sn(M))
        return _Aff(_sn(A), offset(shift, back)) + d

    def layer(W, b, vin: _Aff):
        return _Aff(ub * _kappa(W) * vin.p, ub * (256.0 * float(np.linalg.norm(b)) + _kappa(W) * vin.r) + 1e-30)

    for l in range(levels):
        S, bs, Q, bq, Cb = g(l, "stage_w"), g(l, "stage_b"), g(l, "qhead_w"), g(l, "qhead_b"), g(l, "codebook")
        vx = norm_bound(A, shift, back, srcs)
        srcs = [(S @ M, e, n) for M, e, n in srcs] + [(eye.copy(), layer(S, bs, vx), f"stage{l}")]
        A, shift, back = S @ A, S @ shift + bs, [S @ B for B in back]
        vz = norm_bound(A, shift, back, srcs)
        sq = [(Q @ M, e, n) for M, e, n in srcs] + [(eye.copy(), layer(Q, bq, vz), f"qhead{l}")]
        vq = norm_bound(Q @ A, Q @ shift + bq, [Q @ B for B in back], sq)
        cn = np.linalg.norm(Cb, axis=1)
        cmax, c2max = float(cn.max()), float((cn ** 2).max())
        e = _Aff()
        for M, eps, name in sq:
            wpair = 0.0
            for K in np.split(Cb @ M, segs):
                gram = K @ K.T
                dg = np.diag(gram)
                wpair = max(wpair, float(np.sqrt(max(0.0, (dg[:, None] + dg[None, :] - 2.0 * gram).max()))))
            e = e + eps.scale(2.0 * wpair)
            report.append((l, name, wpair, eps.p, eps.r))
        e = e + vq.scale(2.0 * 2.0 * 256.0 * ub * cmax)
        e = e + vq.scale(2.0 * 2.0 * U * cmax * (1.0 + 256.0 * ub))
        fin = 2.0 * U * (2.0 + U)
        x2 = fin * (1.0 + 2.0 ** -17)
        ea.append(e.r + (fin * (1.0 + 1e-5) + 2.0 * 67.0 * U) * c2max + x2 * vq.r * vq.r)
        eb.append(e.p + x2 * 2.0 * vq.p * vq.r)
        ec.append(x2 * vq.p * vq.p)
        if l < levels - 1:
            Lh, bl = g(l, "lhead_w"), g(l, "lhead_b")
            srcs = [(Lh @ M, e_, n) for M, e_, n in srcs] + [(eye.copy(), layer(Lh, bl, vz), f"lhead{l}")]
            A, shift, back = Lh @ A, Lh @ shift + bl, [Lh @ B for B in back] + [eye.copy()]
            vn = norm_bound(A, shift, back, srcs)
            srcs = srcs + [(eye.copy(), vn.scale(U / (1.0 - U)), f"sub{l}")]
    host = 1.0 + 1e-6
    return np.array(ea) * host, np.array(eb) * host, np.array(ec) * host, report


def pack_factor(segs: int, kc: int) -> int:
    return 128 if segs == 1 and kc <= 128 else 256


CANDIDATE_ENTRY = {128: "qv2x_codebook_encode_candidates_i8", 256: "qv2x_codebook_encode_candidates_seg_i8"}


def candidate_tables(state: Dict[str, np.ndarray], levels: int, in_delta: float, in_zx: int, segs: int = 1) -> Dict[str, np.ndarray]:
    from .engine import collapse_encoder_f64
    G, gb, tabs = collapse_encoder_f64(state, levels)
    ke = G.shape[0] // levels
    kc = ke // segs
    if any(state[f"codebook/{l}/codebook"].shape[0] != ke for l in range(levels)):
        raise ValueError("two-stage encode: every level needs the same dict_size")
    if segs == 1:
        if kc % 32 or kc > 256 or levels > 3:
            raise ValueError("two-stage encode: dict_size 32 | 64 | 96 | 128 | ... | 256, up to three levels")
    elif segs != 2 or kc * segs != ke or kc % 64 or kc > 256 or levels > 3:
        raise ValueError("two-stage encode: seg_num 1 | 2, dict_size a multiple of 64 up to 256 with two segments, up to three levels")
    n_t = segs * max(levels - 1, 0)
    tlim = 2.0 ** 29 / max(2, n_t)
    blim = 2.0 ** 44 if pack_factor(segs, kc) == 128 else 2.0 ** 43
    gs = float(in_delta) * G
    tmax = max([float(np.abs(t).max()) for t in tabs.values()] + [0.0])
    h = max(float(np.abs(gs).max()) / G_MAX_INT, tmax / (tlim - 2.0), float(np.abs(gb).max()) / (blim - 2.0 ** 32))
    gi = np.rint(gs / h).astype(np.int64)
    limbs, rest = [], gi.copy()
    for _ in range(LIMBS):
        d = ((rest + 128) % 256) - 128
        limbs.append(d.astype(np.int8))
        rest = (rest - d) // 256
    if rest.any():
        raise ValueError("two-stage encode: G on the grid does not fit the candidate stage's int8 limbs")
    bias = np.rint(gb / h).astype(np.int64) + (128 - int(in_zx)) * gi.sum(1)
    tables = np.stack([np.rint(tabs[(l, j)] / h) for l in range(levels) for j in range(l)]) if levels > 1 else np.zeros((1, ke, ke))
    if np.abs(tables).max() >= tlim or np.abs(bias).max() >= blim:
        raise ValueError("two-stage encode: table / bias entries leave the fixed-point range of the candidate stage")
    lane = np.arange(64)
    score = (np.arange(levels * ke // 32)[:, None, None, None] * 32 + (lane & 31)[None, None, :, None])
    chan = (32 * np.arange(8)[None, :, None, None] + 16 * (lane >> 5)[None, None, :, None] + np.arange(16)[None, None, None, :])
    packed = np.stack([lb[score, chan] for lb in limbs], axis=1)
    packed = packed.reshape(levels, ke // 32, LIMBS, 8, 64, 16)
    ea, eb, ec, report = encode_error_bound(state, levels, in_delta, segs)
    fp = 1.0 + 1e-4
    tau = np.zeros((levels, 3))
    for l in range(levels):
        own = 1.0 + segs * l + 2.0
        tau[l] = [(ea[l] / h + own) * fp, eb[l] / h * fp, ec[l] / h * fp]
    return {"gpack": np.ascontiguousarray(packed, dtype=np.int8), "bias": np.ascontiguousarray(bias, dtype=np.int64),
            "tables": np.ascontiguousarray(tables, dtype=np.int32), "tau": np.ascontiguousarray(tau, dtype=np.float32), "h": h,
            "g_int": gi, "bound": (ea, eb, ec), "report": report, "segs": segs, "kc": kc, "pack": pack_factor(segs, kc)}


def candidate_emulate(codes_u8: np.ndarray, tabs: Dict[str, np.ndarray], in_delta: float, in_zx: int):
    gi, bias, tables, tau, h = tabs["g_int"], tabs["bias"], tabs["tables"], tabs["tau"], tabs["h"]
    levels = tau.shape[0]
    segs = int(tabs.get("segs", 1))
    ke = gi.shape[0] // levels
    kc = ke // segs
    P = float(tabs.get("pack", 128))
    b = codes_u8.astype(np.float64) - 128.0
    s = b @ gi.astype(np.float64).T + bias.astype(np.float64)[None]
    n = codes_u8.astype(np.int64) - int(in_zx)
    n1, n2 = np.abs(n).sum(1), (n * n).sum(1)
    n0 = (np.float32(in_delta) * np.sqrt(n2.astype(np.float32))).astype(np.float32)
    out = np.zeros((levels * segs, codes_u8.shape[0]), np.uint8)
    flags = np.zeros((levels * segs, codes_u8.shape[0]), bool)
    gaps = np.zeros((levels * segs, codes_u8.shape[0]))
    for l in range(levels):
        sc = s[:, l * ke:(l + 1) * ke].copy()
        for j in range(l):
            for sp in range(segs):
                sc += tables[l * (l - 1) // 2 + j][sp * kc + out[j * segs + sp].astype(np.int64)].astype(np.float64)
        t = (((tau[l, 0] + tau[l, 1] * n0) + (tau[l, 2] * n0) * n0) + n1.astype(np.float32)).astype(np.float32)
        assert t.dtype == np.float32 and n0.dtype == np.float32
        t = t.astype(np.float64)
        for sg in range(segs):
            v = sc[:, sg * kc:(sg + 1) * kc]
            order = np.argsort(v, axis=1, kind="stable")
            best, second = np.take_along_axis(v, order[:, :1], 1)[:, 0], np.take_along_axis(v, order[:, 1:2], 1)[:, 0]
            p = l * segs + sg
            out[p] = order[:, 0]
            k2 = order[:, 1]
            flags[p] = (P * second + k2) - (P * best + out[p]) <= P * np.ceil(t) + (P - 1.0)
            gaps[p] = (second - best) * h
    return out, flags.any(0), flags, gaps
```

### quantv2x_amd/engine.py

```python
from __future__ import annotations

import ctypes as C
from typing import Dict, List, NamedTuple, Optional

import numpy as np
import torch
import torch.nn as nn

from . import lib as L
from .ptq_state import export_ptq_state, load_ptq_state

_HEADS = ("cls_head", "reg_head", "dir_head")


def _dev(a: np.ndarray, dev) -> torch.Tensor:
    return torch.from_numpy(np.ascontiguousarray(a)).to(dev).contiguous()


def _pack_k4(w: np.ndarray) -> np.ndarray:
    j, k = w.shape
    assert k % 4 == 0
    return np.ascontiguousarray(w.T.reshape(k // 4, 4, j).transpose(0, 2, 1), dtype=np.float32)


def decode_tables(state: Dict[str, np.ndarray], levels: int, width: int = 256):
    g = lambda l, n: state[f"codebook/{l}/{n}"].astype(np.float64)
    tables, const, chain = [], np.zeros(width), np.eye(width)
    for l in range(levels):
        front = chain @ g(l, "restore_w")
        tables.append((front @ g(l, "dqhead_w") @ g(l, "codebook").T).T)
        const = const + front @ g(l, "dqhead_b") + chain @ g(l, "restore_b")
        if l < levels - 1:
            const = const + front @ g(l, "side_b")
            chain = front @ g(l, "side_w")
    return np.ascontiguousarray(np.stack(tables), dtype=np.float32), np.ascontiguousarray(const, dtype=np.float32)


def collapse_encoder_f64(state: Dict[str, np.ndarray], levels: int):
    g = lambda l, n: state[f"codebook/{l}/{n}"].astype(np.float64)
    kc = int(state["codebook/0/codebook"].shape[0])
    front, shift = np.eye(256), np.zeros(256)
    back = []
    G, gb, tables = [], [], {}
    for l in range(levels):
        Ws, bs, Wq, bq, Cb = g(l, "stage_w"), g(l, "stage_b"), g(l, "qhead_w"), g(l, "qhead_b"), g(l, "codebook")
        Gp = -2.0 * Cb @ Wq @ Ws
        gp = (Cb * Cb).sum(1) - 2.0 * Cb @ (Wq @ bs + bq)
        G.append(Gp @ front)
        gb.append(Gp @ shift + gp)
        for j, Bj in enumerate(back):
            tables[(l, j)] = -(Gp @ Bj @ g(j, "codebook").T).T
        if l < levels - 1:
            A = g(l, "lhead_w") @ Ws
            d = g(l, "lhead_w") @ bs + g(l, "lhead_b")
            front, shift = A @ front, A @ shift + d
            back = [A @ Bj for Bj in back] + [np.eye(256)]
    return np.concatenate(G), np.concatenate(gb), tables


def collapse_encoder(state: Dict[str, np.ndarray], levels: int, in_delta: float, in_zx: int):
    Gall, gall, tables = collapse_encoder_f64(state, levels)
    kc = Gall.shape[0] // levels
    bias = gall + in_delta * (0.0 - in_zx) * Gall.sum(1)
    Gs = in_delta * Gall
    nct = levels * kc // 32
    lane = np.arange(64)
    col = (np.arange(nct)[:, None, None] * 32 + (lane & 31)[None, None, :])
    k = (2 * np.arange(128)[None, :, None] + (lane >> 5)[None, None, :])
    packed = Gs[col, k]
    tab = np.stack([tables[(l, j)] for l in range(levels) for j in range(l)]) if levels > 1 else np.zeros((1, kc, kc))
    return (np.ascontiguousarray(packed, dtype=np.float32), np.ascontiguousarray(bias, dtype=np.float32), np.ascontiguousarray(tab, dtype=np.float32))


def _pack_k4p(w: np.ndarray) -> np.ndarray:
    return np.ascontiguousarray(_pack_k4(w)[:, :, [0, 2, 1, 3]])


def _pack_wave(w: np.ndarray) -> np.ndarray:
    j, k = w.shape
    assert k == 256
    if j % 64:
        w = np.concatenate([w, np.zeros((64 - j % 64, k), w.dtype)])
    return np.ascontiguousarray(w.reshape(-1, 2, 32, 32, 4, 2).transpose(0, 3, 1, 5, 2, 4), dtype=np.float32)


ENC_WAVE_PAD = 16 * 256


def _pack_wave_seg(cb: np.ndarray, segs: int) -> np.ndarray:
    ke, k = cb.shape
    kc, d = ke // segs, 256 // segs
    assert k == 256 and segs in (2, 4) and kc % 32 == 0
    blocks = np.stack([cb[sg * kc:(sg + 1) * kc, sg * d:(sg + 1) * d] for sg in range(segs)])
    b = blocks.reshape(segs // 2, 2, kc // 32, 32, d // 8, 4, 2)
    return np.ascontiguousarray(b.transpose(0, 2, 4, 1, 6, 3, 5), dtype=np.float32)


def wave_section(stage_w, qhead_w, lhead_w, cb, segs: int = 1) -> np.ndarray:
    cbs = _pack_wave(cb) if segs == 1 else _pack_wave_seg(cb, segs)
    sec = np.concatenate([_pack_wave(stage_w).reshape(-1), _pack_wave(qhead_w).reshape(-1), cbs.reshape(-1), _pack_wave(lhead_w).reshape(-1)])
    full = 3 * 65536 + (cb.shape[0] + 63) // 64 * 64 * 256
    return np.concatenate([sec, np.zeros(full - sec.size + ENC_WAVE_PAD, np.float32)])


class _ConvLayer:

    def __init__(self, state, name, in_groups, stride, dev, pad_cin=0, pad_cout=0):
        code = state[name + "/w_code"]
        dw = state[name + "/w_delta"].astype(np.float32)
        zw = state[name + "/w_zp"].astype(np.int64)
        bias_np = state[name + "/bias"].astype(np.float32)
        if pad_cin > code.shape[1]:
            fill = np.broadcast_to(np.clip(zw, 0, 255).astype(np.uint8)[:, None, None, None], (code.shape[0], pad_cin - code.shape[1], 3, 3))
            code = np.concatenate([code, fill], axis=1)
        if pad_cout > code.shape[0]:
            extra = pad_cout - code.shape[0]
            code = np.concatenate([code, np.full((extra,) + code.shape[1:], 128, np.uint8)])
            dw, zw = np.concatenate([dw, np.ones(extra, np.float32)]), np.concatenate([zw, np.full(extra, 128, np.int64)])
            bias_np = np.concatenate([bias_np, np.zeros(extra, np.float32)])
        cout = code.shape[0]
        ws = code.astype(np.int64) - 128
        aw = 128 - zw
        parts, corr, scale = [], [], []
        for (c0, c, dx, zx) in in_groups:
            blk = ws[:, c0:c0 + c].transpose(0, 2, 3, 1).reshape(cout, -1)
            parts.append(blk)
            ax = 128 - int(zx)
            corr.append(ax * blk.sum(axis=1) + blk.shape[1] * ax * aw)
            scale.append(np.float32(dx) * dw)
        self.name, self.stride, self.cout = name, stride, cout
        self.groups = [(int(c0), int(c), int(zx)) for (c0, c, _, zx) in in_groups]
        self.w = _dev(np.concatenate(parts, axis=1).astype(np.int8), dev)
        self.w_wide = None
        self.scale = _dev(np.stack(scale).astype(np.float32), dev)
        self.corr = _dev(np.stack(corr).astype(np.int32), dev)
        self.aw = _dev(aw.astype(np.int32), dev)
        self.bias = _dev(bias_np, dev)
        self.out_q = (float(np.float32(state[name + "/a_delta"])), int(state[name + "/a_zp"]))
        assert np.abs(np.stack(corr)).max() < 2 ** 31


class _ChainLayers:
    MAX_DEPTH = 4

    @staticmethod
    def eligible(convs) -> bool:
        return (1 <= len(convs) <= _ChainLayers.MAX_DEPTH and all(c.cout == 64 and len(c.groups) == 1 and c.groups[0][1] == 64 for c in convs)
                and all(c.stride == 1 for c in convs[1:]))

    def __init__(self, convs, dev):
        self.convs = convs
        self.name = convs[-1].name
        packed = []
        for c in convs:
            w = c.w.cpu().numpy().reshape(2, 32, 9, 2, 2, 16)
            packed.append(w.transpose(0, 2, 3, 4, 1, 5))
        self.w = _dev(np.stack(packed).astype(np.int8), dev)
        cat = lambda ts: torch.cat([t.reshape(-1) for t in ts]).contiguous()
        self.scale, self.corr = cat([c.scale for c in convs]), cat([c.corr for c in convs])
        self.aw, self.bias = cat([c.aw for c in convs]), cat([c.bias for c in convs])
        self.stride0 = convs[0].stride
        self.out_q = convs[-1].out_q


class _DeconvLayer:
    def __init__(self, state, name, in_q, dev):
        code = state[name + "/w_code"].astype(np.float32)
        dw = state[name + "/w_delta"].astype(np.float32).reshape(-1, 1, 1, 1)
        zw = state[name + "/w_zp"].astype(np.float32).reshape(-1, 1, 1, 1)
        wdeq = ((code - zw) * dw).astype(np.float32)
        cin, cout, s, _ = wdeq.shape
        cols = wdeq.transpose(0, 2, 3, 1).reshape(cin, s * s * cout)
        self.w = _dev(_pack_k4p(cols.T), dev)
        self.bias = _dev(state[name + "/bias"].astype(np.float32), dev)
        self.name, self.cin, self.cout, self.s, self.in_q = name, cin, cout, s, in_q
        self.out_q = (float(np.float32(state[name + "/a_delta"])), int(state[name + "/a_zp"]))


class _Heads:

    def __init__(self, state, suffix, dev):
        ws, bs, das, zas = [], [], [], []
        for h in _HEADS:
            n = h + suffix
            code = state[n + "/w_code"].astype(np.float32).reshape(state[n + "/w_code"].shape[0], -1)
            w = ((code - state[n + "/w_zp"].astype(np.float32)[:, None]) * state[n + "/w_delta"].astype(np.float32)[:, None])
            ws.append(w.astype(np.float32))
            bs.append(state[n + "/bias"].astype(np.float32))
            off = bool(state[n + "/a_off"])
            das.append(np.full(w.shape[0], -1.0 if off else float(np.float32(state[n + "/a_delta"])), np.float32))
            zas.append(np.full(w.shape[0], 0.0 if off else float(state[n + "/a_zp"]), np.float32))
        self._stack(ws, bs, das, zas, dev)

    @classmethod
    def folded_fp32(cls, state, suffix, dev):
        hd = cls.__new__(cls)
        ws = [state[h + suffix + "/w"] for h in _HEADS]
        hd._stack(ws, [state[h + suffix + "/bias"] for h in _HEADS], [np.full(w.shape[0], -1.0, np.float32) for w in ws],
                  [np.zeros(w.shape[0], np.float32) for w in ws], dev)
        return hd

    def _stack(self, ws, bs, das, zas, dev):
        self.splits = [w.shape[0] for w in ws]
        self.cout = sum(self.splits)
        self.cout_pad = (self.cout + 31) // 32 * 32
        if self.cout_pad > 96:
            raise NotImplementedError("heads: at most 96 stacked output channels")
        pad = self.cout_pad - self.cout
        w = np.concatenate(ws + [np.zeros((pad, 256), np.float32)])
        self.w = _dev(_pack_k4p(w), dev)
        self.bias = _dev(np.concatenate(bs + [np.zeros(pad, np.float32)]), dev)
        self.da = _dev(np.concatenate(das + [np.full(pad, -1.0, np.float32)]), dev)
        self.za = _dev(np.concatenate(zas + [np.zeros(pad, np.float32)]), dev)
        self._w_np, self._b_np = np.concatenate(ws).astype(np.float64), np.concatenate(bs).astype(np.float64)
        self.da_np = np.ascontiguousarray(np.concatenate(das))
        self.lut_tables = None

    def collapse_over_decode(self, lut: np.ndarray, lut_bias: np.ndarray, dev):
        t = np.einsum("lkd,cd->lkc", lut.astype(np.float64), self._w_np)
        b = lut_bias.astype(np.float64) @ self._w_np.T + self._b_np
        self.lut_tables = (_dev(t.astype(np.float32), dev), _dev(b.astype(np.float32), dev))


def scene_layout(data_dict: dict, n_total: int):
    pairwise = data_dict["pairwise_t_matrix"]
    if pairwise.dtype != torch.float64 or not pairwise.is_contiguous():
        pairwise = pairwise.to(torch.float64).contiguous()
    if pairwise.shape[0] == 1:
        return pairwise, [n_total]
    rl = data_dict["record_len"]
    if isinstance(rl, torch.Tensor) and rl.is_cuda and torch.cuda.is_current_stream_capturing():
        raise ValueError("record_len on the GPU cannot be read during HIP-graph capture: pass a CPU tensor")
    return pairwise, [int(v) for v in (rl.tolist() if isinstance(rl, torch.Tensor) else rl)]


def split_heads(preds: torch.Tensor, splits, suffix: str = "") -> dict:
    c, r, _ = splits
    out = {"cls_preds" + suffix: preds[:, :c], "reg_preds" + suffix: preds[:, c:c + r], "dir_preds" + suffix: preds[:, c + r:]}
    if not suffix:
        out["preds_tensor"] = preds
    return out


def capture_call(call):
    side = torch.cuda.Stream()
    side.wait_stream(torch.cuda.current_stream())
    with torch.cuda.stream(side):
        for _ in range(2):
            call()
    torch.cuda.current_stream().wait_stream(side)
    graph = torch.cuda.CUDAGraph()
    with torch.cuda.graph(graph):
        out = call()

    def replay():
        graph.replay()
        return out
    replay.graph = graph
    return replay


def capture_forward(module: nn.Module, data_dict: dict):
    rl = data_dict.get("record_len")
    if data_dict["pairwise_t_matrix"].shape[0] > 1 and isinstance(rl, torch.Tensor) and rl.is_cuda:
        data_dict = dict(data_dict, record_len=rl.cpu())
    return capture_call(lambda: module.forward(data_dict))


def assemble_heter_codes(owner: str, engines: dict, slot_cache: dict, agents: list, data_dict: dict, encode, taps: Optional[dict]) -> torch.Tensor:
    unknown = sorted(set(agents) - set(engines))
    if unknown:
        raise NotImplementedError(f"{owner}: no engine for modality {unknown}")
    slots = slot_cache.get(tuple(agents))
    if slots is None:
        if torch.cuda.is_current_stream_capturing():
            raise L.Qv2xError(f"{owner}: agent layout {agents} is new and the stream is capturing -- its slot indices are an H2D copy; "
                              "run one eager forward of this layout first (capture does)")
        slots = {m: torch.as_tensor([i for i, a in enumerate(agents) if a == m], dtype=torch.int64, device=e.dev) for m, e in engines.items()}
        slot_cache[tuple(agents)] = slots
    e = next(iter(engines.values()))
    n_total, hw, lv = len(agents), e.fh * e.fw, e.levels
    enc = torch.empty((lv, n_total * hw), dtype=torch.uint8, device=e.dev)
    for m, eng in engines.items():
        k = int(slots[m].numel())
        if not k:
            continue
        mt = {} if taps is not None else None
        codes = encode(eng, data_dict["inputs_" + m], k, mt).view(lv, k, hw)
        enc.view(lv, n_total, hw).index_copy_(1, slots[m], codes)
        if taps is not None:
            taps["modality/" + m] = mt
    return enc


def pillar_inputs(inputs: dict, pfn: bool = True):
    vf = inputs["voxel_features"].contiguous()
    co = inputs["voxel_coords"].to(torch.int32).contiguous()
    npnt = inputs["voxel_num_points"].to(torch.int32).contiguous()
    if pfn and (vf.dtype != torch.float32 or vf.dim() != 3 or tuple(vf.shape[1:]) != (32, 4)):
        raise ValueError("voxel_features must be float32 [M, 32, 4]")
    return vf, co, npnt


def pfn_params(state: Dict[str, np.ndarray]):
    s, n = state, "encoder_m1.pillar_vfe.pfn_layers.0.linear"
    wq = ((s[n + "/w_code"].astype(np.float32) - s[n + "/w_zp"].astype(np.float32)[:, None])
          * s[n + "/w_delta"].astype(np.float32)[:, None]).astype(np.float32)
    if wq.shape != (64, 10):
        raise NotImplementedError("deployed PFN expects Linear(10 -> 64)")
    p = L.PfnParams()
    p.w[:] = wq.reshape(-1).tolist()
    p.b[:] = s[n + "/bias"].astype(np.float32).tolist()
    p.d1, p.z1 = float(np.float32(s[n + "/a_delta"])), float(s[n + "/a_zp"])
    p.d2, p.z2 = float(np.float32(s["pfn/a2_delta"])), float(s["pfn/a2_zp"])
    p.vox[:] = [float(np.float32(v)) for v in s["meta/voxel"]]
    p.off[:] = [float(np.float32(v)) for v in s["meta/offset"]]
    return p, (p.d2, int(p.z2))


def level_blob_host(state: Dict[str, np.ndarray], l: int, ke: int, D: int, segs: int):
    W = 64 if D == 64 else 256
    last = f"codebook/{l}/lhead_w" not in state

    def padded(n, *shape):
        out = np.zeros(shape, np.float32)
        if not (last and n.startswith("lhead")):
            a = state[f"codebook/{l}/{n}"]
            out[tuple(slice(0, k) for k in a.shape)] = a
        return out
    stage, qhead, lhead, cb = padded("stage_w", W, W), padded("qhead_w", W, W), padded("lhead_w", W, W), padded("codebook", ke, W)
    parts = [_pack_k4p(stage), padded("stage_b", W), _pack_k4p(qhead), padded("qhead_b", W), _pack_k4p(lhead), padded("lhead_b", W),
             _pack_k4p(cb), cb, np.zeros(ke, np.float32)]
    flat = np.concatenate([p.reshape(-1) for p in parts])
    c2_off = flat.size - ke
    if W == 256:
        flat = np.concatenate([flat, wave_section(stage, qhead, lhead, cb, segs)])
    return flat, c2_off - ke * W, c2_off


def level_blob(lib, state: Dict[str, np.ndarray], l: int, ke: int, D: int, segs: int, dev) -> torch.Tensor:
    flat, cb_off, c2_off = level_blob_host(state, l, ke, D, segs)
    floats, c2fn, name = ((lib.qv2x_codebook64_level_floats, lib.qv2x_codebook64_c2_f32, "qv2x_codebook64_c2_f32") if D == 64
                          else (lib.qv2x_codebook_level_floats, lib.qv2x_codebook_c2_f32, "qv2x_codebook_c2_f32"))
    assert flat.size == floats(ke)
    blob = _dev(flat, dev)
    L.check(c2fn(C.c_void_p(blob.data_ptr() + 4 * cb_off), ke, C.c_void_p(blob.data_ptr() + 4 * c2_off), L.current_stream()), name)
    return blob


class CodebookConstants(NamedTuple):
    enc_levels: int
    segs: int
    levels: int
    ke: int
    kc: int
    D: int
    lut_host: np.ndarray
    lut_bias_host: np.ndarray
    lut: torch.Tensor
    lut_bias: torch.Tensor
    level_blobs: List[torch.Tensor]
    level_ptrs: object


def codebook_constants(lib, state: Dict[str, np.ndarray], dev, refuse) -> CodebookConstants:
    s = state
    enc_levels, segs = int(s["meta/codebook_levels"]), int(s.get("meta/codebook_segs", 1))
    ke, D = (int(v) for v in s["codebook/0/codebook"].shape)
    kc, levels = ke // segs, enc_levels * segs
    refuse(ke, kc, D, segs)
    lut, lut_bias = decode_tables(s, enc_levels, D)
    lut = lut.reshape(levels, kc, D)
    blobs = [level_blob(lib, s, l, ke, D, segs, dev) for l in range(enc_levels)]
    return CodebookConstants(enc_levels, segs, levels, ke, kc, D, lut, lut_bias, _dev(lut, dev), _dev(lut_bias, dev), blobs,
                             (C.c_void_p * enc_levels)(*[b.data_ptr() for b in blobs]))


def _pairwise_from_poses(self, gathered: torch.Tensor, world: int, agent_stride: int, pose_offset: int, max_cav: int, out: torch.Tensor):
    L.check(self.lib.qv2x_pairwise_from_poses_f64(L.ptr(gathered), world, agent_stride, pose_offset, max_cav, L.ptr(out),
                                                  L.current_stream()), "qv2x_pairwise_from_poses_f64")


class DeployedPostStage(nn.Module):
    fuse_heads_min_tiles = 4 * 1280
    fuse_heads_max_agents = 4
    single_agent_tables = True
    band_one_launch = None
    _band_rows = None

    def __init__(self, state: Dict[str, np.ndarray], device, emit_single_preds: Optional[bool]):
        super().__init__()
        self.lib = L.load()
        if not torch.cuda.is_available():
            raise L.Qv2xError(f"{type(self).__name__} needs an MI355X (torch.cuda.is_available() is False)")
        self.state, self.dev = state, torch.device(device)
        s, dev = state, self.dev
        if str(s.get("meta/fusion_method", "att")) not in ("att", "max"):
            raise NotImplementedError(f"deployed path: fusion_method {s['meta/fusion_method']!r} ('att' = AttFusion and 'max' = MaxFusion are built here)")
        self.fusion = 1 if str(s.get("meta/fusion_method", "att")) == "max" else 0
        self.nx, self.ny, _ = (int(v) for v in s["meta/grid"])
        self.hm, self.wm = (float(v) for v in s["meta/HW_metres"])
        self.ratio = float(s["meta/discrete_ratio"])
        self.layer_nums = [int(v) for v in s["meta/layer_nums"]]
        self.strides = [int(v) for v in s["meta/layer_strides"]]
        self.ups = [int(v) for v in s["meta/upsample_strides"]]
        self.has_codebook = bool(s["meta/has_codebook"])
        self.emit_single = bool(s["meta/supervise_single"]) if emit_single_preds is None else bool(emit_single_preds)
        self._lut_host = (None, None)
        if self.has_codebook:
            c = codebook_constants(self.lib, s, dev, self._refuse_codebook)
            self.enc_levels, self.segs, self.levels, self.ke, self.kc = c.enc_levels, c.segs, c.levels, c.ke, c.kc
            self.lut, self.lut_bias, self.level_blobs, self.level_ptrs = c.lut, c.lut_bias, c.level_blobs, c.level_ptrs
            self._lut_host = (c.lut_host, c.lut_bias_host)

    @staticmethod
    def _refuse_codebook(ke, kc, D, segs):
        if ke > 512 or kc > 256:
            raise NotImplementedError(f"deployed codebook path: seg_num * dict_size <= 512, dict_size <= 256 (got {segs} x {kc}): "
                                      "the encode kernels' tile budget (qv2x_codebook_encode_f32)")
        if D != 256:
            raise NotImplementedError(f"deployed codebook path: a codebook as wide as the 256-channel shared feature (got {D})")

    def _set_heads(self, heads: _Heads, heads_single: Optional[_Heads], tables: bool):
        self.heads, self.heads_single = heads, heads_single
        self.table_heads, self.single_by_tables, self.single_by_global_tables = None, False, False
        if not (tables and self.has_codebook):
            return
        (lut, lut_bias), dev = self._lut_host, self.dev
        self.single_by_tables = (self.heads_single is not None and self.levels <= 4
                                 and self.levels * self.kc * self.heads_single.cout * 4 <= 60 * 1024)
        self.single_by_global_tables = (not self.single_by_tables and self.heads_single is not None and self.levels <= 16
                                        and self.heads_single.cout % 4 == 0 and self.heads_single.cout <= 128)
        if self.single_by_tables or self.single_by_global_tables:
            self.heads_single.collapse_over_decode(lut, lut_bias, dev)
        sets = [self.heads] + ([self.heads_single] if self.heads_single is not None else [])
        ct = sum(h.cout for h in sets)
        ct4 = (ct + 3) // 4 * 4
        st = ct4 if (ct4 // 4) % 2 else ct4 + 4
        in_lds = self.levels <= 4 and (self.levels * self.kc * st + 4 * ct4) * 4 <= 160 * 1024
        if in_lds or (self.levels <= 16 and ct % 4 == 0 and ct <= 128):
            t = np.concatenate([np.einsum("lkd,cd->lkc", lut.astype(np.float64), h._w_np) for h in sets], axis=2)
            b = np.concatenate([lut_bias.astype(np.float64) @ h._w_np.T + h._b_np for h in sets])
            cat = lambda name: torch.cat([getattr(h, name)[:h.cout] for h in sets]).contiguous()
            self.table_heads = (_dev(t.astype(np.float32), dev), _dev(b.astype(np.float32), dev), cat("da"), cat("za"),
                                self.heads.cout, self.heads_single.cout if self.heads_single is not None else 0)

    def _run_heads(self, hd: _Heads, rows, nb, hw):
        out = torch.empty((nb, hd.cout, self.fh, self.fw), dtype=torch.float32, device=self.dev)
        L.check(self.lib.qv2x_heads_f32(L.ptr(rows), nb * hw, hw, hd.cout, hd.cout_pad, L.ptr(hd.w), L.ptr(hd.bias),
                                        L.ptr(hd.da), L.ptr(hd.za), L.ptr(out), L.current_stream()), "qv2x_heads_f32")
        return out

    def wire_shape(self):
        self._workspace(1)
        return self.levels, self.fh * self.fw

    pairwise_from_poses = _pairwise_from_poses

    def pairwise_frames_from_poses(self, gathered: torch.Tensor, world: int, agent_stride: int, pose_offset: int, frames: int, frame_stride: int,
                                   max_cav: int, out: torch.Tensor):
        L.check(self.lib.qv2x_pairwise_from_poses_batch_f64(L.ptr(gathered), world, agent_stride, pose_offset, frames, frame_stride, max_cav,
                                                            L.ptr(out), L.current_stream()), "qv2x_pairwise_from_poses_batch_f64")

    def fuse_frames_and_heads(self, gathered: torch.Tensor, agent_stride: int, level_stride: int, frame_stride: int, pairwise: torch.Tensor,
                              n_agents: int, ego: int, own_codes: Optional[torch.Tensor], frames: int) -> dict:
        lens = [n_agents] * frames
        form = self._post_form(lens, None, own_codes is not None and frame_stride == self.fh * self.fw)
        return self._post(form, L.ptr(gathered), agent_stride, level_stride, None, pairwise, [f * frame_stride for f in range(frames)], lens, ego,
                          own_codes, frames)

    def band_shape(self):
        self._workspace(1)
        return self.heads.cout, self.fh, self.fw

    def head_wire_supported(self, wire: str) -> bool:
        if wire not in L.WIRES:
            raise ValueError(f"wire: one of {sorted(L.WIRES)}, got {wire!r}")
        return wire == "f32" or bool((self.heads.da_np > 0).all())

    def fuse_frames_and_heads_band(self, gathered: torch.Tensor, agent_stride: int, level_stride: int, frame_stride: int, pairwise: torch.Tensor,
                                   n_agents: int, ego: int, frames: int, y0: int, y1: int, out_slab: torch.Tensor, wire: str = "f32"):
        if not self.head_wire_supported(wire):
            raise L.Qv2xError("band wire 'u8': a head without an output quantizer has no codes to send")
        hd, n_cells, esz = self.heads, (y1 - y0) * self.fw, (1 if wire == "u8" else 4)
        if not 0 <= y0 <= y1 <= self.fh:
            raise ValueError(f"band rows [{y0}, {y1}) outside the map's {self.fh} rows")
        if out_slab.dtype != torch.uint8 or out_slab.numel() < frames * hd.cout * n_cells * esz:
            raise ValueError("out_slab: u8, at least frames * cout * band cells * element size bytes")
        if n_cells == 0:
            return
        one_launch = self.band_one_launch
        if one_launch is None:
            one_launch = frames * n_cells // 32 >= self.fuse_heads_min_tiles and n_agents <= self._one_launch_agents()
        rows = None
        if not one_launch:
            key = (frames, n_cells)
            if self._band_rows is None or self._band_rows[0] != key:
                self._band_rows = (key, torch.empty((frames, n_cells, 256), dtype=torch.float32, device=self.dev))
            rows = self._band_rows[1]
        base, st = out_slab.data_ptr(), L.current_stream()
        for s0, n, d, offs, cnts, lut, lb in self._scene_chunks(agent_stride, level_stride, pairwise, [f * frame_stride for f in range(frames)],
                                                                [n_agents] * frames, ego):
            out = C.c_void_p(base + s0 * hd.cout * n_cells * esz)
            if one_launch:
                L.check(self.lib.qv2x_fuse_heads_band(C.byref(d), n, offs, cnts, L.ptr(gathered), lut, lb, None, L.ptr(pairwise[s0]),
                                                      y0 * self.fw, n_cells, hd.cout, hd.cout_pad, L.ptr(hd.w), L.ptr(hd.bias), L.ptr(hd.da),
                                                      L.ptr(hd.za), L.WIRES[wire], L.ptr(hd.da_np), out, None, st), "qv2x_fuse_heads_band")
            else:
                L.check(self.lib.qv2x_fuse_att_band_f32(C.byref(d), n, offs, cnts, L.ptr(gathered), lut, lb, None, L.ptr(pairwise[s0]),
                                                        y0 * self.fw, n_cells, L.ptr(rows[s0]), st), "qv2x_fuse_att_band_f32")
                L.check(self.lib.qv2x_heads_band(L.ptr(rows[s0]), n, n_cells, hd.cout, hd.cout_pad, L.ptr(hd.w), L.ptr(hd.bias),
                                                 L.ptr(hd.da), L.ptr(hd.za), L.WIRES[wire], L.ptr(hd.da_np), out, st), "qv2x_heads_band")

    def assemble_bands(self, gathered_slabs: torch.Tensor, world: int, frames: int, wire: str, out: torch.Tensor):
        hd = self.heads
        L.check(self.lib.qv2x_assemble_bands(L.ptr(gathered_slabs), world, gathered_slabs.shape[1], frames, hd.cout, self.fh, self.fw, L.WIRES[wire],
                                             L.ptr(hd.da), L.ptr(hd.za), L.ptr(out), L.current_stream()), "qv2x_assemble_bands")

    def band_output(self, preds: torch.Tensor, own_codes: Optional[torch.Tensor], frames: int) -> dict:
        out = split_heads(preds, self.heads.splits)
        if own_codes is not None:
            out.update(self.single_preds(own_codes, frames))
        return out

    def decode_rows(self, codes, n_rows_total):
        out = torch.empty((n_rows_total, 256), dtype=torch.float32, device=self.dev)
        L.check(self.lib.qv2x_decode_lut_f32(L.ptr(codes), n_rows_total, self.levels, self.kc, L.ptr(self.lut),
                                             L.ptr(self.lut_bias), L.ptr(out), L.current_stream()), "qv2x_decode_lut_f32")
        return out

    def _fuse_desc(self, agent_stride, level_stride, pairwise_b, n, ego):
        d = L.FuseDesc()
        d.agents, d.h, d.w = n, self.fh, self.fw
        d.levels, d.kc = (self.levels, self.kc) if self.has_codebook else (1, 1)
        d.max_cav, d.ego = pairwise_b.shape[0], ego
        d.code_agent_stride, d.code_level_stride = agent_stride, level_stride
        d.h_metres, d.w_metres, d.discrete_ratio = self.hm, self.wm, self.ratio
        d.fusion = self.fusion
        return d

    def fuse(self, codes_ptr, agent_stride, level_stride, feats, pairwise_b, n, out, ego=0):
        d = self._fuse_desc(agent_stride, level_stride, pairwise_b, n, ego)
        lut, lb = self._lut_ptrs()
        L.check(self.lib.qv2x_fuse_att_f32(C.byref(d), codes_ptr, lut, lb, L.ptr(feats) if feats is not None else None,
                                           L.ptr(pairwise_b), L.ptr(out), L.current_stream()), "qv2x_fuse_att_f32")

    def _lut_ptrs(self):
        return (L.ptr(self.lut), L.ptr(self.lut_bias)) if self.has_codebook else (None, None)

    def _scene_chunks(self, agent_stride, level_stride, pairwise, offsets, counts, ego):
        lut, lb = self._lut_ptrs()
        for s0 in range(0, len(counts), 64):
            s1 = min(len(counts), s0 + 64)
            d = self._fuse_desc(agent_stride, level_stride, pairwise[s0], max(counts[s0:s1]), ego)
            yield s0, s1 - s0, d, (C.c_int64 * (s1 - s0))(*offsets[s0:s1]), (C.c_int32 * (s1 - s0))(*counts[s0:s1]), lut, lb

    def fuse_scenes(self, codes_ptr, agent_stride, level_stride, feats, pairwise, offsets, counts, out, ego=0):
        for s0, n, d, offs, cnts, lut, lb in self._scene_chunks(agent_stride, level_stride, pairwise, offsets, counts, ego):
            L.check(self.lib.qv2x_fuse_att_batch_f32(C.byref(d), n, offs, cnts, codes_ptr, lut, lb,
                                                     L.ptr(feats) if feats is not None else None, L.ptr(pairwise[s0]), L.ptr(out[s0]),
                                                     L.current_stream()), "qv2x_fuse_att_batch_f32")

    def _self_transforms_are_identity(self, pairwise: torch.Tensor) -> bool:
        if pairwise.is_cuda:
            if torch.cuda.is_current_stream_capturing():
                return True
            ref = getattr(self, "_ident_ref", None)
            if ref is not None and ref[0]() is pairwise and ref[1] == pairwise._version:
                return ref[2]
            t00 = pairwise[:, 0, 0].cpu()
        else:
            t00 = pairwise[:, 0, 0]
        ok = bool((t00 == torch.eye(4, dtype=t00.dtype)).all())
        if pairwise.is_cuda:
            import weakref
            self._ident_ref = (weakref.ref(pairwise), pairwise._version, ok)
        return ok

    def _one_launch_agents(self) -> int:
        batched = self.has_codebook and self.levels == 3
        return self.fuse_heads_max_agents if batched else min(self.fuse_heads_max_agents, 1)

    def _table_heads_out(self, codes, n: int) -> dict:
        tab, tb, da, za, c0, c1 = self.table_heads
        hw = self.fh * self.fw
        preds = torch.empty((n, c0, self.fh, self.fw), dtype=torch.float32, device=self.dev)
        sp = torch.empty((n, c1, self.fh, self.fw), dtype=torch.float32, device=self.dev) if c1 else None
        L.check(self.lib.qv2x_table_heads_f32(L.ptr(codes), n * hw, hw, self.levels, self.kc, c0, c1, L.ptr(tab), L.ptr(tb), L.ptr(da), L.ptr(za),
                                              L.ptr(preds), L.ptr(sp) if sp is not None else None, L.current_stream()), "qv2x_table_heads_f32")
        out = split_heads(preds, self.heads.splits)
        if sp is not None:
            out.update(split_heads(sp, self.heads_single.splits, "_single"))
        return out

    def fuse_heads_scenes(self, codes_ptr, agent_stride, level_stride, feats, pairwise, offsets, counts, ego=0, fused_tap=None):
        hd, hw = self.heads, self.fh * self.fw
        out = torch.empty((len(counts), hd.cout, self.fh, self.fw), dtype=torch.float32, device=self.dev)
        for s0, n, d, offs, cnts, lut, lb in self._scene_chunks(agent_stride, level_stride, pairwise, offsets, counts, ego):
            L.check(self.lib.qv2x_fuse_heads_batch_f32(C.byref(d), n, offs, cnts, codes_ptr, lut, lb,
                                                       L.ptr(feats) if feats is not None else None, L.ptr(pairwise[s0]),
                                                       hd.cout, hd.cout_pad, L.ptr(hd.w), L.ptr(hd.bias), L.ptr(hd.da), L.ptr(hd.za), L.ptr(out[s0]),
                                                       L.ptr(fused_tap[s0]) if fused_tap is not None else None, L.current_stream()),
                    "qv2x_fuse_heads_batch_f32")
        return out

    def _post_form(self, lens: List[int], taps: Optional[dict], identity) -> str:
        if (taps is None and self.table_heads is not None and self.single_agent_tables and all(n == 1 for n in lens)
                and (identity() if callable(identity) else identity)):
            return "tables"
        if taps is None and len(lens) * self.fh * self.fw // 32 >= self.fuse_heads_min_tiles and max(lens) <= self._one_launch_agents():
            return "one_launch"
        return "fused"

    def _post(self, form: str, codes_ptr, agent_stride, level_stride, feats, pairwise, offsets, lens: List[int], ego: int,
              own: Optional[torch.Tensor], n_own: int, taps: Optional[dict] = None) -> dict:
        if form == "tables":
            return self._table_heads_out(own, len(lens))
        hw, nb = self.fh * self.fw, len(lens)
        single = self.heads_single is not None and own is not None
        sp = None
        if form == "one_launch":
            preds = self.fuse_heads_scenes(codes_ptr, agent_stride, level_stride, feats, pairwise, offsets, lens, ego)
            if single:
                sp = self._decode_heads_single(own, n_own)
        else:
            fused = torch.empty((nb, hw, 256), dtype=torch.float32, device=self.dev)
            self.fuse_scenes(codes_ptr, agent_stride, level_stride, feats, pairwise, offsets, lens, fused, ego)
            if single:
                preds, sp = self._heads_pair(fused, nb, own, n_own)
            else:
                preds = self._run_heads(self.heads, fused, nb, hw)
            if taps is not None:
                taps["fused"] = fused
        if self.heads_single is not None and sp is None and feats is not None:
            sp = self._run_heads(self.heads_single, feats, sum(lens), hw)
        out = split_heads(preds, self.heads.splits)
        if sp is not None:
            out.update(split_heads(sp, self.heads_single.splits, "_single"))
        return out

    def fuse_and_heads(self, codes, agent_stride, level_stride, pairwise_b, n_agents, ego=0) -> dict:
        return self.fuse_heads_and_single(codes, agent_stride, level_stride, pairwise_b, n_agents, ego, None, 0)

    def _decode_heads_single(self, codes, n_agents: int):
        hw = self.fh * self.fw
        hd = self.heads_single
        sp = torch.empty((n_agents, hd.cout, self.fh, self.fw), dtype=torch.float32, device=self.dev)
        if self.single_by_tables:
            tab, tb = hd.lut_tables
            L.check(self.lib.qv2x_single_heads_lut_f32(L.ptr(codes), n_agents * hw, hw, self.levels, self.kc, hd.cout, L.ptr(tab), L.ptr(tb),
                                                       L.ptr(hd.da), L.ptr(hd.za), L.ptr(sp), L.current_stream()), "qv2x_single_heads_lut_f32")
            return sp
        if self.single_by_global_tables:
            tab, tb = hd.lut_tables
            L.check(self.lib.qv2x_table_heads_f32(L.ptr(codes), n_agents * hw, hw, self.levels, self.kc, hd.cout, 0, L.ptr(tab), L.ptr(tb),
                                                  L.ptr(hd.da), L.ptr(hd.za), L.ptr(sp), None, L.current_stream()), "qv2x_table_heads_f32")
            return sp
        L.check(self.lib.qv2x_decode_heads_f32(L.ptr(codes), n_agents * hw, hw, self.levels, self.kc, L.ptr(self.lut), L.ptr(self.lut_bias),
                                               hd.cout, hd.cout_pad, L.ptr(hd.w), L.ptr(hd.bias), L.ptr(hd.da), L.ptr(hd.za),
                                               L.ptr(sp), L.current_stream()), "qv2x_decode_heads_f32")
        return sp

    def _heads_pair(self, fused, nb, codes, n_agents):
        hw = self.fh * self.fw
        hd, hs = self.heads, self.heads_single
        if self.single_by_tables or self.single_by_global_tables:
            return self._run_heads(hd, fused, nb, hw), self._decode_heads_single(codes, n_agents)
        preds = torch.empty((nb, hd.cout, self.fh, self.fw), dtype=torch.float32, device=self.dev)
        sp = torch.empty((n_agents, hs.cout, self.fh, self.fw), dtype=torch.float32, device=self.dev)
        L.check(self.lib.qv2x_heads_pair_f32(L.ptr(fused), nb * hw, hw, hd.cout, hd.cout_pad, L.ptr(hd.w), L.ptr(hd.bias), L.ptr(hd.da),
                                             L.ptr(hd.za), L.ptr(preds), L.ptr(codes), n_agents * hw, self.levels, self.kc,
                                             L.ptr(self.lut), L.ptr(self.lut_bias), hs.cout, hs.cout_pad, L.ptr(hs.w), L.ptr(hs.bias),
                                             L.ptr(hs.da), L.ptr(hs.za), L.ptr(sp), L.current_stream()), "qv2x_heads_pair_f32")
        return preds, sp

    def fuse_heads_and_single(self, codes, agent_stride, level_stride, pairwise_b, n_agents, ego, own_codes, n_own: int = 1) -> dict:
        pairwise = pairwise_b.to(torch.float64).contiguous()[None]
        return self._post("fused", L.ptr(codes), agent_stride, level_stride, None, pairwise, [0], [n_agents], ego, own_codes, n_own)

    def single_preds(self, codes, n_agents: int) -> dict:
        if self.heads_single is None:
            return {}
        return split_heads(self._decode_heads_single(codes, n_agents), self.heads_single.splits, "_single")

    @torch.no_grad()
    def forward(self, data_dict: dict, taps: Optional[dict] = None) -> dict:
        agents = data_dict["agent_modality_list"]
        n_total = len(agents)
        if any(a != "m1" for a in agents):
            raise NotImplementedError("deployed path: every agent is the LiDAR modality 'm1' (a heterogeneous model deploys as DeployedHeterModel)")
        enc = self.encode_agents(data_dict["inputs_m1"], n_total, taps)
        return self.finish(enc, n_total, data_dict, taps)

    @torch.no_grad()
    def finish(self, enc, n_total: int, data_dict: dict, taps: Optional[dict] = None) -> dict:
        pairwise, lens = scene_layout(data_dict, n_total)
        hw = self.fh * self.fw
        feats = None if self.has_codebook else self._shared_features(enc, n_total)
        form = self._post_form(lens, taps, lambda: self._self_transforms_are_identity(data_dict["pairwise_t_matrix"]))
        if form != "tables" and not pairwise.is_cuda:
            if torch.cuda.is_current_stream_capturing():
                raise ValueError("pairwise_t_matrix on the host cannot be uploaded during HIP-graph capture: pass a device tensor")
            pairwise = pairwise.to(self.dev)
        starts = [sum(lens[:bi]) for bi in range(len(lens))]
        if self.has_codebook:
            out = self._post(form, L.ptr(enc), hw, n_total * hw, None, pairwise, [st * hw for st in starts], lens, 0, enc, n_total, taps)
        else:
            out = self._post(form, None, 0, 0, feats, pairwise, [st * hw * 256 for st in starts], lens, 0, None, n_total, taps)
        if taps is not None:
            taps["codes"] = enc if self.has_codebook else None
            taps["features"] = feats
        return out

    def capture(self, data_dict: dict):
        return capture_forward(self, data_dict)


class DeployedModel(DeployedPostStage):

    def __init__(self, state: Dict[str, np.ndarray], device="cuda", emit_single_preds: Optional[bool] = None):
        super().__init__(state, device, emit_single_preds)
        s, dev = state, self.dev

        self.encoder_kind = str(s["meta/encoder"]) if "meta/encoder" in s else "point_pillar"
        if self.encoder_kind == "second":
            last = int(s["second/n_layers"]) - 1
            q = (float(np.float32(s[f"second/{last}/a_delta"])), int(s[f"second/{last}/a_zp"]))
            self.canvas_c, self.canvas_q, self.pfn = int(s["meta/canvas_channels"]), q, None
            self.second: Dict[int, object] = {}
            self.second_max_voxels, self.second_max_points = 70000, 5
        else:
            self.pfn, q = pfn_params(s)
            self.canvas_c, self.canvas_q = 64, q

        self.blocks: List[List[_ConvLayer]] = []
        self.chains: List[Optional[_ChainLayers]] = []
        self.deblocks: List[_DeconvLayer] = []
        cat_groups, c0 = [], 0
        cin = self.canvas_c
        for lvl in range(len(self.layer_nums)):
            convs = []
            for i in range(self.layer_nums[lvl] + 1):
                layer = _ConvLayer(s, f"backbone_m1.blocks.{lvl}.{i + 1}", [(0, cin, q[0], q[1])],
                                   self.strides[lvl] if i == 0 else 1, dev)
                convs.append(layer)
                q, cin = layer.out_q, layer.cout
            self.blocks.append(convs)
            self.chains.append(_ChainLayers(convs, dev) if _ChainLayers.eligible(convs) else None)
            de = _DeconvLayer(s, f"backbone_m1.deblocks.{lvl}.0", q, dev)
            self.deblocks.append(de)
            cat_groups.append((c0, de.cout, de.out_q[0], de.out_q[1]))
            c0 += de.cout
        self.cat_channels = c0
        self.shrink0 = _ConvLayer(s, "shrinker_m1.layers.0.double_conv.0", cat_groups, 1, dev)
        self.shrink1 = _ConvLayer(s, "shrinker_m1.layers.0.double_conv.1",
                                  [(0, self.shrink0.cout, *self.shrink0.out_q)], 1, dev)
        if self.shrink1.cout != 256:
            raise NotImplementedError("deployed path expects a 256-channel shared feature")
        self.compress = bool(s.get("meta/compress", False))
        self.final = self.shrink1
        if self.compress:
            if self.has_codebook:
                raise NotImplementedError("deployed path: compressor and codebook together")
            narrow = int(s["compressor.encoder.0/w_code"].shape[0])
            pad = (narrow + 63) // 64 * 64
            self.comp = [_ConvLayer(s, "compressor.encoder.0", [(0, 256, *self.shrink1.out_q)], 1, dev, pad_cout=pad)]
            self.comp.append(_ConvLayer(s, "compressor.decoder.0", [(0, pad, *self.comp[0].out_q)], 1, dev, pad_cin=pad))
            self.comp.append(_ConvLayer(s, "compressor.decoder.1", [(0, 256, *self.comp[1].out_q)], 1, dev))
            self.comp_channels = narrow
            self.final = self.comp[-1]
        self._set_heads(_Heads(s, "", dev), _Heads(s, "_single", dev) if (self.emit_single and "cls_head_single/w_code" in s) else None,
                        tables=True)
        self._bufs: Dict[int, dict] = {}
        self.use_wide_conv, self.batch_deconvs, self.use_chains = True, True, True
        self.chain_max_agents = 1
        self._collapsed, self._two_stage, self.two_stage_refused = None, None, None
        self.encode_form = "auto"
        self.encode_mode = "two_stage" if self.two_stage_supported() else "exact"

    def _padded(self, n, h, w, c, q):
        t = torch.empty((n, h + 2, w + 2, c), dtype=torch.int8, device=self.dev)
        t.fill_(int(q[1]) - 128)
        return t

    def _workspace(self, n: int) -> dict:
        if n in self._bufs:
            return self._bufs[n]
        b = {}
        h, w = self.ny, self.nx
        if self.encoder_kind == "second":
            from .engine_second import DeployedSecondEncoder
            self.second[n] = DeployedSecondEncoder(self.state, self.dev, agents=n, max_voxels=self.second_max_voxels, max_points=self.second_max_points)
            b["canvas"] = self.second[n].bev
        else:
            b["canvas"] = self._padded(n, h, w, 64, self.canvas_q)
        b["lvl"] = []
        for lvl, convs in enumerate(self.blocks):
            h, w = (h + 2 - 3) // self.strides[lvl] + 1, (w + 2 - 3) // self.strides[lvl] + 1
            zps = {c.out_q[1] for c in convs}
            if len(zps) != 1:
                raise NotImplementedError("conv outputs of one backbone level must share a zero point (post-ReLU: 0)")
            pair = [self._padded(n, h, w, convs[0].cout, convs[0].out_q) for _ in range(2)]
            b["lvl"].append((pair, h, w))
        (_, h0, w0) = b["lvl"][0]
        self.fh, self.fw = h0 * self.ups[0], w0 * self.ups[0]
        for lvl, (_, hl, wl) in enumerate(b["lvl"]):
            if (hl * self.ups[lvl], wl * self.ups[lvl]) != (self.fh, self.fw):
                raise ValueError(f"deblock {lvl} upsamples {hl}x{wl} by {self.ups[lvl]} to {hl * self.ups[lvl]}x{wl * self.ups[lvl]}, "
                                 f"level 0 gives {self.fh}x{self.fw}: the grid does not line up across backbone levels")
        cat = torch.empty((n, self.fh + 2, self.fw + 2, self.cat_channels), dtype=torch.int8, device=self.dev)
        c0 = 0
        for de in self.deblocks:
            cat[..., c0:c0 + de.cout] = int(de.out_q[1]) - 128
            c0 += de.cout
        b["cat"] = cat
        b["s0"] = self._padded(n, self.fh, self.fw, self.shrink0.cout, self.shrink0.out_q)
        b["s1"] = self._padded(n, self.fh, self.fw, self.shrink1.cout, self.shrink1.out_q)
        if self.compress:
            b["comp"] = [self._padded(n, self.fh, self.fw, c.cout, c.out_q) for c in self.comp]
        hw = self.fh * self.fw
        if self.has_codebook:
            b["codes"] = torch.empty((self.levels, n, hw), dtype=torch.uint8, device=self.dev)
        if self.two_stage_supported():
            if self._two_stage is None and self.encode_mode == "two_stage":
                self._build_two_stage()
            b["enc_list"] = torch.zeros(3 * n * hw, dtype=torch.int32, device=self.dev)
            b["enc_counters"] = torch.zeros(4, dtype=torch.int32, device=self.dev)
        if not self.has_codebook or self.heads_single is not None:
            b["feats"] = torch.empty((n, hw, 256), dtype=torch.float32, device=self.dev)
        self._bufs[n] = b
        return b

    def _conv(self, layer: _ConvLayer, x, n, h, w, out, out_ctotal=None, out_c0=0):
        d = L.ConvDesc()
        d.n, d.h, d.w, d.cin_total, d.stride, d.cout = n, h, w, x.shape[-1], layer.stride, layer.cout
        d.ngroups = len(layer.groups)
        for i, (c0, c, zx) in enumerate(layer.groups):
            d.group_c0[i], d.group_c[i], d.group_zx[i] = c0, c, zx
        d.out_ctotal = out.shape[-1] if out_ctotal is None else out_ctotal
        d.out_c0, d.relu = out_c0, 1
        d.out_delta, d.out_zp = layer.out_q[0], float(layer.out_q[1])
        if self.use_wide_conv and self.lib.qv2x_conv3x3_i8_wide_ok(C.byref(d)):
            if layer.w_wide is None:
                layer.w_wide = torch.empty_like(layer.w)
                L.check(self.lib.qv2x_conv3x3_i8_pack_wide(C.byref(d), L.ptr(layer.w), L.ptr(layer.w_wide), L.current_stream()), layer.name)
            L.check(self.lib.qv2x_conv3x3_i8_wide(C.byref(d), L.ptr(x), L.ptr(layer.w_wide), L.ptr(layer.scale), L.ptr(layer.corr),
                                                  L.ptr(layer.aw), L.ptr(layer.bias), L.ptr(out), L.current_stream()), layer.name)
            return
        L.check(self.lib.qv2x_conv3x3_i8(C.byref(d), L.ptr(x), L.ptr(layer.w), L.ptr(layer.scale), L.ptr(layer.corr),
                                         L.ptr(layer.aw), L.ptr(layer.bias), L.ptr(out), L.current_stream()), layer.name)

    def _chain(self, ch: _ChainLayers, x, n, h, w, out):
        d = L.ChainDesc()
        d.n, d.in_h, d.in_w = n, h, w
        d.h, d.w = out.shape[1] - 2, out.shape[2] - 2
        d.depth, d.stride0, d.relu = len(ch.convs), ch.stride0, 1
        for i, c in enumerate(ch.convs):
            d.out_delta[i], d.out_zp[i] = c.out_q[0], float(c.out_q[1])
        L.check(self.lib.qv2x_conv3x3_i8_chain64(C.byref(d), L.ptr(x), L.ptr(ch.w), L.ptr(ch.scale), L.ptr(ch.corr), L.ptr(ch.aw),
                                                 L.ptr(ch.bias), L.ptr(out), L.current_stream()), ch.name)

    def _deconv_desc(self, de: _DeconvLayer, n, h, w, out, out_c0):
        d = L.DeconvDesc()
        d.n, d.h, d.w, d.cin, d.cout, d.s = n, h, w, de.cin, de.cout, de.s
        d.in_zx, d.in_delta = int(de.in_q[1]), float(de.in_q[0])
        d.out_ctotal, d.out_c0, d.relu = out.shape[-1], out_c0, 1
        d.out_delta, d.out_zp = de.out_q[0], float(de.out_q[1])
        d.out_h, d.out_w = out.shape[1] - 2, out.shape[2] - 2
        return d

    def _deconv(self, de: _DeconvLayer, x, n, h, w, out, out_c0):
        d = self._deconv_desc(de, n, h, w, out, out_c0)
        L.check(self.lib.qv2x_deconv_i8(C.byref(d), L.ptr(x), L.ptr(de.w), L.ptr(de.bias), L.ptr(out), L.current_stream()), de.name)

    def _deconv_batch(self, items, n):
        k = len(items)
        descs = (L.DeconvDesc * k)(*[self._deconv_desc(de, n, h, w, out, c0) for (de, x, h, w, out, c0) in items])
        arr = lambda ts: (C.c_void_p * k)(*[t.data_ptr() for t in ts])
        L.check(self.lib.qv2x_deconv_i8_batch(descs, k, arr([it[1] for it in items]), arr([it[0].w for it in items]),
                                              arr([it[0].bias for it in items]), arr([it[4] for it in items]), L.current_stream()),
                "qv2x_deconv_i8_batch")

    def conv_plan(self, n_agents: int):
        b = self._workspace(n_agents)
        use_chains = self.use_chains and n_agents <= self.chain_max_agents
        key = ("plan", use_chains)
        if key in b:
            return b[key]
        plan = []
        x, h, w, c0 = b["canvas"], self.ny, self.nx, 0
        for lvl, convs in enumerate(self.blocks):
            pair, ho, wo = b["lvl"][lvl]
            macs = [n_agents * ho * wo * layer.cout * layer.w.shape[1] for layer in convs]
            if use_chains and self.chains[lvl] is not None:
                out = pair[(len(convs) - 1) % 2]
                plan.append(("chain", self.chains[lvl], x, h, w, out, 0, sum(macs)))
                x, h, w = out, ho, wo
            else:
                for i, layer in enumerate(convs):
                    out = pair[i % 2]
                    plan.append(("conv", layer, x, h, w, out, 0, macs[i]))
                    x, h, w = out, ho, wo
            de = self.deblocks[lvl]
            plan.append(("deconv", de, x, h, w, b["cat"], c0, n_agents * h * w * de.cin * de.cout * de.s * de.s))
            c0 += de.cout
        hw = n_agents * self.fh * self.fw
        plan.append(("conv", self.shrink0, b["cat"], self.fh, self.fw, b["s0"], 0, hw * self.shrink0.cout * self.shrink0.w.shape[1]))
        plan.append(("conv", self.shrink1, b["s0"], self.fh, self.fw, b["s1"], 0, hw * self.shrink1.cout * self.shrink1.w.shape[1]))
        if self.compress:
            x = b["s1"]
            for c, out in zip(self.comp, b["comp"]):
                plan.append(("conv", c, x, self.fh, self.fw, out, 0, hw * c.cout * c.w.shape[1]))
                x = out
        b[key] = plan
        return plan

    def run_plan(self, n_agents: int, only=None, taps: Optional[dict] = None):
        pending = []

        def flush():
            if len(pending) == 1:
                de, x, h, w, out, c0 = pending[0]
                self._deconv(de, x, n_agents, h, w, out, c0)
            elif pending:
                self._deconv_batch(pending, n_agents)
            pending.clear()

        for (kind, layer, x, h, w, out, c0, _) in self.conv_plan(n_agents):
            if only is not None and not only(kind, layer):
                continue
            if kind == "chain":
                self._chain(layer, x, n_agents, h, w, out)
                if taps is not None:
                    taps[layer.name] = out.clone()
            elif kind == "conv":
                if layer is self.shrink0:
                    flush()
                self._conv(layer, x, n_agents, h, w, out)
                if taps is not None:
                    taps[layer.name] = out.clone()
            else:
                pending.append((layer, x, h, w, out, c0))
                if not self.batch_deconvs:
                    flush()
        flush()

    def pillars_to_canvas(self, inputs: dict, n_agents: int, resident: bool = False):
        b = self._workspace(n_agents)
        st = L.current_stream()
        vf, co, npnt = pillar_inputs(inputs, pfn=self.encoder_kind != "second")
        if self.encoder_kind == "second":
            return self.second[n_agents]({"voxel_features": vf, "voxel_coords": co, "voxel_num_points": npnt})
        canvas = b["canvas"]
        capturing = torch.cuda.is_current_stream_capturing()
        if not resident and b.get("fill_less_graphs", False):
            raise L.Qv2xError("pillars_to_canvas(resident=False) on a workspace whose captured graphs rely on the clean resident canvas: "
                              "use resident=True + clear_pillars, or another DeployedModel")
        if not (resident and b.get("canvas_clean", False)):
            L.check(self.lib.qv2x_fill_i8(L.ptr(canvas), canvas.numel(), int(self.pfn.z2) - 128, st), "qv2x_fill_i8")
        elif capturing:
            b["fill_less_graphs"] = True
        b["canvas_clean"] = False
        L.check(self.lib.qv2x_pfn_scatter_i8(L.ptr(vf), L.ptr(co), L.ptr(npnt), vf.shape[0], 32, C.byref(self.pfn),
                                             L.ptr(canvas), n_agents, self.ny, self.nx, st), "qv2x_pfn_scatter_i8")
        return canvas

    def _restore_canvas(self, n_agents: int):
        b = self._workspace(n_agents)
        if self.encoder_kind != "second" and not torch.cuda.is_current_stream_capturing():
            L.check(self.lib.qv2x_fill_i8(L.ptr(b["canvas"]), b["canvas"].numel(), int(self.pfn.z2) - 128, L.current_stream()), "qv2x_fill_i8")
            b["canvas_clean"] = True

    def clear_pillars(self, inputs: dict, n_agents: int):
        if self.encoder_kind == "second":
            return
        b = self._workspace(n_agents)
        co = inputs["voxel_coords"].to(torch.int32).contiguous()
        L.check(self.lib.qv2x_pfn_unscatter_i8(L.ptr(co), co.shape[0], int(self.pfn.z2) - 128, L.ptr(b["canvas"]), n_agents, self.ny, self.nx,
                                               L.current_stream()), "qv2x_pfn_unscatter_i8")
        b["canvas_clean"] = True

    def encode_codes(self, n_agents: int, out: Optional[torch.Tensor] = None):
        b = self._workspace(n_agents)
        codes = b["codes"] if out is None else out
        if codes.dtype != torch.uint8 or not codes.is_contiguous() or codes.numel() != self.levels * n_agents * self.fh * self.fw:
            raise ValueError("encode_codes: out must be a contiguous uint8 tensor [levels, n_agents, H*W]")
        d = L.EncodeDesc()
        d.n, d.h, d.w, d.levels, d.kc, d.segs = n_agents, self.fh, self.fw, self.enc_levels, self.kc, self.segs
        d.in_zx, d.in_delta = int(self.shrink1.out_q[1]), float(self.shrink1.out_q[0])
        two_stage = self.encode_mode == "two_stage" and self.encode_form == "auto"
        if two_stage and self._two_stage is None:
            self._refuse_during_capture("encode_mode 'two_stage'")
            self._build_two_stage()
            two_stage = self.encode_mode == "two_stage"
        if self.encode_mode == "collapsed":
            if self.segs != 1 or self.kc > 128:
                raise NotImplementedError("encode_mode 'collapsed': seg_num 1 and dict_size <= 128 (the exact encode takes the rest)")
            if self._collapsed is None:
                self._refuse_during_capture("encode_mode 'collapsed'")
                self._collapsed = tuple(_dev(t, self.dev) for t in collapse_encoder(self.state, self.enc_levels, d.in_delta, d.in_zx))
            gp, bias, tab = self._collapsed
            L.check(self.lib.qv2x_codebook_encode_collapsed_f32(C.byref(d), L.ptr(b["s1"]), L.ptr(gp), L.ptr(bias), L.ptr(tab), L.ptr(codes),
                                                                L.current_stream()), "qv2x_codebook_encode_collapsed_f32")
            return codes
        if two_stage:
            return self._encode_two_stage(d, b, codes)
        if self.encode_mode not in ("exact", "two_stage"):
            raise ValueError(f"encode_mode {self.encode_mode!r}: 'exact' (every cell through the reference's op order), 'two_stage' (the same "
                             "indices: exact integer candidates, the chain only where the bound cannot decide) or 'collapsed' (opt-in, approximate)")
        if self.encode_form == "wave":
            L.check(self.lib.qv2x_codebook_encode_wave_f32(C.byref(d), L.ptr(b["s1"]), None, self.level_ptrs, L.ptr(codes),
                                                           L.current_stream()), "qv2x_codebook_encode_wave_f32")
            return codes
        L.check(self.lib.qv2x_codebook_encode_f32(C.byref(d), L.ptr(b["s1"]), self.level_ptrs, L.ptr(codes),
                                                  L.current_stream()), "qv2x_codebook_encode_f32")
        return codes

    def two_stage_supported(self) -> bool:
        if not self.has_codebook or self.enc_levels > 3 or self.kc > 256:
            return False
        return bool(self.kc % 32 == 0 if self.segs == 1 else self.segs == 2 and self.kc % 64 == 0)

    def _refuse_during_capture(self, what: str):
        if torch.cuda.is_current_stream_capturing():
            raise L.Qv2xError(f"{what}: its operands are built on the host and uploaded -- not inside a HIP-graph capture; encode once "
                              "in this mode before capturing")

    def _build_two_stage(self):
        if not self.two_stage_supported():
            raise NotImplementedError("encode_mode 'two_stage': seg_num 1 | 2, dict_size <= 256, up to three levels (encode_mode 'exact' takes the rest)")
        from .encode_two_stage import candidate_tables
        try:
            t = candidate_tables(self.state, self.enc_levels, float(self.shrink1.out_q[0]), int(self.shrink1.out_q[1]), self.segs)
            k = np.arange(t["bias"].shape[0], dtype=np.int64) % self.kc
            pf = int(t["pack"])
            packed = (pf * t["bias"] + k).astype(np.float64)
            if not np.array_equal(packed.astype(np.int64), pf * t["bias"] + k):
                raise ValueError("two-stage encode: packed scores not exact in float64")
            self._two_stage = (_dev(t["gpack"], self.dev), _dev(packed, self.dev), _dev(t["tables"], self.dev),
                               (C.c_float * (3 * self.enc_levels))(*[float(v) for v in t["tau"].reshape(-1)]), t)
        except Exception as e:
            self.encode_mode, self.two_stage_refused = "exact", str(e) or type(e).__name__

    def candidate_entry(self) -> str:
        from .encode_two_stage import CANDIDATE_ENTRY, pack_factor
        return CANDIDATE_ENTRY[pack_factor(self.segs, self.kc)]

    def _encode_two_stage(self, d, b, codes):
        gp, bias, tab, tau, _ = self._two_stage
        name = self.candidate_entry()
        L.check(getattr(self.lib, name)(C.byref(d), L.ptr(b["s1"]), L.ptr(gp), L.ptr(bias), L.ptr(tab), tau, L.ptr(codes),
                                        L.ptr(b["enc_list"]), L.ptr(b["enc_counters"]), L.current_stream()), name)
        L.check(self.lib.qv2x_codebook_encode_listed_f32(C.byref(d), L.ptr(b["s1"]), self.level_ptrs, L.ptr(b["enc_list"]), L.ptr(b["enc_counters"]),
                                                         L.ptr(codes), L.current_stream()), "qv2x_codebook_encode_listed_f32")
        return codes

    def encode_refine_stats(self, n_agents: int) -> dict:
        if not (self.encode_mode == "two_stage" and self.encode_form == "auto") or "enc_counters" not in self._bufs.get(n_agents, {}):
            raise L.Qv2xError(f"encode_refine_stats({n_agents}): no two-stage encode of {n_agents} frames here (encode_mode "
                              f"{self.encode_mode!r}, encode_form {self.encode_form!r}, workspaces {sorted(self._bufs)})")
        c = self._bufs[n_agents]["enc_counters"].cpu().numpy().astype(np.int64)
        cells = n_agents * self.fh * self.fw
        return {"cells": cells, "refined": int(c[0]), "refined_fraction": float(c[0]) / cells, "first_flagged_at_level": [int(v) for v in c[1:1 + self.enc_levels]]}

    def encode_into(self, inputs: dict, frames: int, codes_out: torch.Tensor):
        self.pillars_to_canvas(inputs, frames, resident=True)
        try:
            self.run_plan(frames)
            self.clear_pillars(inputs, frames)
        except BaseException:
            self._restore_canvas(frames)
            raise
        return self.encode_codes(frames, out=codes_out)

    def encode_agents(self, inputs: dict, n_agents: int, taps: Optional[dict] = None):
        b = self._workspace(n_agents)
        canvas = self.pillars_to_canvas(inputs, n_agents, resident=True)
        try:
            self.run_plan(n_agents, taps=taps)
            if taps is not None:
                taps["canvas"], taps["cat"] = canvas.clone(), b["cat"]
            self.clear_pillars(inputs, n_agents)
        except BaseException:
            self._restore_canvas(n_agents)
            raise
        if taps is not None:
            taps[self.shrink0.name], taps[self.shrink1.name] = b["s0"], b["s1"]
        if taps is not None and self.compress:
            for c, out in zip(self.comp, b["comp"]):
                taps[c.name] = out
        return self.encode_codes(n_agents) if self.has_codebook else (b["comp"][-1] if self.compress else b["s1"])

    def _shared_features(self, shrinker_out, n_total: int):
        q = self.final.out_q
        feats = self._workspace(n_total)["feats"]
        L.check(self.lib.qv2x_dequant_i8_f32(L.ptr(shrinker_out), n_total, self.fh, self.fw, 256, int(q[1]), float(q[0]), L.ptr(feats),
                                             L.current_stream()), "qv2x_dequant_i8_f32")
        return feats


class DeployedHeterModel(nn.Module):

    def __init__(self, states: Dict[str, Dict[str, np.ndarray]], ego_modality: Optional[str] = None, device="cuda", **kw):
        super().__init__()
        if not states:
            raise ValueError("DeployedHeterModel: no modality")
        self.engines = {m: DeployedModel(st, device=device, **kw) for m, st in states.items()}
        self.main = self.engines[ego_modality if ego_modality in self.engines else next(iter(self.engines))]
        for m, e in self.engines.items():
            e._workspace(1)
            if not e.has_codebook:
                raise NotImplementedError("deployed heterogeneous path: codebook models (the code planes are what the modalities share)")
            if (e.fh, e.fw, e.levels, e.kc) != (self.main.fh, self.main.fw, self.main.levels, self.main.kc):
                raise ValueError(f"modality {m}: feature map {e.fh} x {e.fw} / codebook {e.levels} x {e.kc} differs from the ego modality's")
        self.dev = self.main.dev
        self._slots: Dict[tuple, Dict[str, torch.Tensor]] = {}

    @torch.no_grad()
    def forward(self, data_dict: dict, taps: Optional[dict] = None) -> dict:
        agents = list(data_dict["agent_modality_list"])
        enc = assemble_heter_codes("DeployedHeterModel", self.engines, self._slots, agents, data_dict,
                                   lambda eng, inputs, k, mt: eng.encode_agents(inputs, k, mt), taps)
        return self.main.finish(enc, len(agents), data_dict, taps)

    def capture(self, data_dict: dict):
        return capture_forward(self, data_dict)


def deploy_heter(qt_model, device="cuda", **kw) -> DeployedHeterModel:
    model = qt_model.model if hasattr(qt_model, "model") else qt_model
    states = {m: export_ptq_state(qt_model, modality=m) for m in model.modality_name_list}
    return DeployedHeterModel(states, ego_modality=getattr(model, "ego_modality", None), device=device, **kw)


def deploy(qt_model=None, state: Optional[Dict[str, np.ndarray]] = None, path: Optional[str] = None,
           device="cuda", **kw) -> DeployedModel:
    if state is None:
        if path is not None:
            state = load_ptq_state(path)
        elif any(hasattr(m, "weight_quantizer") for m in qt_model.modules()):
            inner = qt_model.model if hasattr(qt_model, "model") else qt_model
            if len(getattr(inner, "modality_name_list", ["m1"])) > 1:
                if hasattr(inner, "pyramid_backbone"):
                    from .engine_pyramid import deploy_heter_pyramid
                    return deploy_heter_pyramid(qt_model, device=device)
                return deploy_heter(qt_model, device=device, **kw)
            state = export_ptq_state(qt_model)
        elif hasattr(qt_model, "pyramid_backbone"):
            from .engine_pyramid_fp32 import export_fp32_pyramid_state
            state = export_fp32_pyramid_state(qt_model)
        else:
            from .engine_fp32 import export_fp32_state
            state = export_fp32_state(qt_model)
    if str(state.get("meta/mode", "w8a8")) == "fp32":
        if str(state.get("meta/fusion_method", "att")) == "pyramid":
            from .engine_pyramid_fp32 import DeployedPyramidFp32Model
            return DeployedPyramidFp32Model(state, device=device, **kw)
        from .engine_fp32 import DeployedFp32Model
        return DeployedFp32Model(state, device=device, **kw)
    if str(state.get("meta/fusion_method", "att")) == "pyramid":
        from .engine_pyramid import DeployedPyramidModel
        return DeployedPyramidModel(state, device=device, **kw)
    return DeployedModel(state, device=device, **kw)
```

### quantv2x_amd/lib.py

```python
from __future__ import annotations

import ctypes as C
import os

_HERE = os.path.dirname(os.path.abspath(__file__))
LIB_PATH = os.path.join(_HERE, "libqv2x.so")
MAX_GROUPS = 4
ABI_VERSION = 9

SYMBOLS = [
    "qv2x_last_error", "qv2x_version", "qv2x_fill_i8", "qv2x_pfn_scatter_i8", "qv2x_pfn_unscatter_i8", "qv2x_conv3x3_i8",
    "qv2x_conv3x3_i8_wide_ok", "qv2x_conv3x3_i8_pack_wide", "qv2x_conv3x3_i8_wide", "qv2x_conv3x3_i8_chain64",
    "qv2x_deconv_i8", "qv2x_deconv_i8_batch", "qv2x_codebook_level_floats", "qv2x_codebook_c2_f32", "qv2x_codebook_encode_f32", "qv2x_codebook_encode_wave_f32", "qv2x_fuse_att_f32", "qv2x_fuse_att_batch_f32", "qv2x_fuse_heads_batch_f32",
    "qv2x_decode_lut_f32", "qv2x_single_heads_lut_f32", "qv2x_table_heads_f32", "qv2x_dequant_i8_f32", "qv2x_heads_f32", "qv2x_decode_heads_f32", "qv2x_heads_pair_f32", "qv2x_voxelize_workspace_bytes", "qv2x_voxelize_f32",
    "qv2x_postprocess_workspace_bytes", "qv2x_postprocess_f32", "qv2x_postprocess_late_workspace_bytes", "qv2x_postprocess_late_f32",
    "qv2x_conv3x3_f32", "qv2x_deconv_f32", "qv2x_pfn_scatter_f32", "qv2x_codebook_encode_f32in",
    "qv2x_pyramid_weighted_fuse_f32", "qv2x_pyramid_weighted_fuse_i8", "qv2x_conv1x1_i8", "qv2x_gconv3x3_i8", "qv2x_conv3x3_i8_res",
    "qv2x_deconv_f32in", "qv2x_codebook_decode_f32", "qv2x_occ_score_i8",
    "qv2x_codebook64_level_floats", "qv2x_codebook64_c2_f32", "qv2x_codebook_encode64_f32", "qv2x_codebook_encode64_f32in",
    "qv2x_add_relu_f32", "qv2x_occ_sigmoid_f32", "qv2x_pyramid_weighted_fuse_f32p", "qv2x_bottleneck_i8",
    "qv2x_comm_unique_id", "qv2x_comm_init", "qv2x_comm_destroy", "qv2x_allgather_codes", "qv2x_pairwise_from_poses_f64", "qv2x_pairwise_from_poses_batch_f64",
    "qv2x_codebook_encode_collapsed_f32", "qv2x_codebook_encode_candidates_i8", "qv2x_codebook_encode_candidates_seg_i8", "qv2x_codebook_encode_listed_f32", "qv2x_mean_vfe_f32", "qv2x_sp_index_scatter", "qv2x_sp_out_sites_workspace_bytes", "qv2x_sp_out_sites", "qv2x_sp_rulebook", "qv2x_sp_conv_f32in", "qv2x_sp_conv_i8", "qv2x_sp_to_bev_i8",
    "qv2x_fuse_att_band_f32", "qv2x_heads_band", "qv2x_fuse_heads_band", "qv2x_assemble_bands",
    "qv2x_voxelize_batch_workspace_bytes", "qv2x_voxelize_batch_f32", "qv2x_postprocess_batch_workspace_bytes", "qv2x_postprocess_batch_f32",
    "qv2x_eval_workspace_bytes", "qv2x_eval_tp_fp_f32", "qv2x_gt_boxes_f32",
    "qv2x_range_search_workspace_bytes", "qv2x_range_search_f32",
    "qv2x_lss_workspace_bytes", "qv2x_lss_plan_f32", "qv2x_lss_splat_f32",
    "qv2x_cam_stem_f32", "qv2x_cam_heads_i8",
]
WIRES = {"f32": 0, "u8": 1}
COMM_ID_BYTES = 128


class PfnParams(C.Structure):
    _fields_ = [("w", C.c_float * 640), ("b", C.c_float * 64),
                ("d1", C.c_float), ("z1", C.c_float), ("d2", C.c_float), ("z2", C.c_float),
                ("vox", C.c_float * 3), ("off", C.c_float * 3)]


class ConvDesc(C.Structure):
    _fields_ = [("n", C.c_int32), ("h", C.c_int32), ("w", C.c_int32), ("cin_total", C.c_int32),
                ("stride", C.c_int32), ("cout", C.c_int32), ("ngroups", C.c_int32),
                ("group_c0", C.c_int32 * MAX_GROUPS), ("group_c", C.c_int32 * MAX_GROUPS),
                ("group_zx", C.c_int32 * MAX_GROUPS),
                ("out_ctotal", C.c_int32), ("out_c0", C.c_int32), ("relu", C.c_int32),
                ("out_delta", C.c_float), ("out_zp", C.c_float)]


class ChainDesc(C.Structure):
    _fields_ = [("n", C.c_int32), ("h", C.c_int32), ("w", C.c_int32), ("in_h", C.c_int32), ("in_w", C.c_int32),
                ("depth", C.c_int32), ("stride0", C.c_int32), ("relu", C.c_int32),
                ("out_delta", C.c_float * 4), ("out_zp", C.c_float * 4)]


class DeconvDesc(C.Structure):
    _fields_ = [("n", C.c_int32), ("h", C.c_int32), ("w", C.c_int32), ("cin", C.c_int32), ("cout", C.c_int32),
                ("s", C.c_int32), ("in_zx", C.c_int32), ("in_delta", C.c_float),
                ("out_ctotal", C.c_int32), ("out_c0", C.c_int32), ("relu", C.c_int32),
                ("out_delta", C.c_float), ("out_zp", C.c_float), ("out_h", C.c_int32), ("out_w", C.c_int32)]


class F32ConvDesc(C.Structure):
    _fields_ = [("n", C.c_int32), ("h", C.c_int32), ("w", C.c_int32), ("cin_total", C.c_int32), ("cin0", C.c_int32), ("cin", C.c_int32),
                ("stride", C.c_int32), ("cout", C.c_int32), ("out_ctotal", C.c_int32), ("out_c0", C.c_int32), ("relu", C.c_int32)]


class Conv1x1Desc(C.Structure):
    _fields_ = [("n", C.c_int32), ("h", C.c_int32), ("w", C.c_int32), ("cin", C.c_int32), ("cout", C.c_int32), ("stride", C.c_int32),
                ("mode", C.c_int32), ("relu", C.c_int32), ("out_ctotal", C.c_int32), ("out_c0", C.c_int32),
                ("out_delta", C.c_float), ("out_zp", C.c_float), ("res_zx", C.c_int32), ("res_delta", C.c_float)]


class BottleneckDesc(C.Structure):
    _fields_ = [("n", C.c_int32), ("h", C.c_int32), ("w", C.c_int32), ("planes", C.c_int32), ("width", C.c_int32), ("cg", C.c_int32),
                ("in_zx", C.c_int32), ("in_delta", C.c_float), ("delta1", C.c_float), ("zp1", C.c_float), ("delta2", C.c_float), ("zp2", C.c_float),
                ("out_delta", C.c_float), ("out_zp", C.c_float)]


class GconvDesc(C.Structure):
    _fields_ = [("n", C.c_int32), ("h", C.c_int32), ("w", C.c_int32), ("c", C.c_int32), ("cg", C.c_int32), ("stride", C.c_int32),
                ("relu", C.c_int32), ("out_delta", C.c_float), ("out_zp", C.c_float)]


class SpconvDesc(C.Structure):
    _fields_ = [("subm", C.c_int32), ("k", C.c_int32 * 3), ("s", C.c_int32 * 3), ("p", C.c_int32 * 3),
                ("in_shape", C.c_int32 * 3), ("out_shape", C.c_int32 * 3), ("agents", C.c_int32), ("cin", C.c_int32), ("cout", C.c_int32),
                ("cap_in", C.c_int32), ("cap_out", C.c_int32), ("out_delta", C.c_float), ("out_zp", C.c_float)]


class OccDesc(C.Structure):
    _fields_ = [("n", C.c_int32), ("h", C.c_int32), ("w", C.c_int32), ("c", C.c_int32), ("aw", C.c_int32), ("corr", C.c_int32),
                ("scale", C.c_float), ("bias", C.c_float), ("out_delta", C.c_float), ("out_zp", C.c_float)]


class EncodeDesc(C.Structure):
    _fields_ = [("n", C.c_int32), ("h", C.c_int32), ("w", C.c_int32), ("levels", C.c_int32), ("kc", C.c_int32),
                ("in_zx", C.c_int32), ("in_delta", C.c_float), ("segs", C.c_int32)]


class FuseDesc(C.Structure):
    _fields_ = [("agents", C.c_int32), ("h", C.c_int32), ("w", C.c_int32), ("levels", C.c_int32), ("kc", C.c_int32),
                ("max_cav", C.c_int32), ("ego", C.c_int32),
                ("code_agent_stride", C.c_int64), ("code_level_stride", C.c_int64),
                ("h_metres", C.c_double), ("w_metres", C.c_double), ("discrete_ratio", C.c_double), ("fusion", C.c_int32)]


class PostprocessDesc(C.Structure):
    _fields_ = [("h", C.c_int32), ("w", C.c_int32), ("anchors_per_cell", C.c_int32), ("num_bins", C.c_int32),
                ("score_threshold", C.c_float), ("nms_threshold", C.c_float), ("dir_offset", C.c_float),
                ("range", C.c_float * 6), ("transform", C.c_float * 16), ("max_boxes", C.c_int32),
                ("num_classes", C.c_int32), ("range_xy_only", C.c_int32),
                ("max_extent", C.c_float), ("z_min", C.c_float), ("z_max", C.c_float)]


class EvalDesc(C.Structure):
    _fields_ = [("frames", C.c_int32), ("det_cap", C.c_int32), ("gt_cap", C.c_int32), ("n_classes", C.c_int32), ("n_ranges", C.c_int32),
                ("n_thresholds", C.c_int32), ("ranges", (C.c_float * 2) * 4), ("thresholds", C.c_float * 4)]


class GtDesc(C.Structure):
    _fields_ = [("frames", C.c_int32), ("agents", C.c_int32), ("obj_cap", C.c_int32), ("gt_cap", C.c_int32), ("row_floats", C.c_int32),
                ("order", C.c_int32), ("mode", C.c_int32), ("range_xy_only", C.c_int32), ("range", C.c_float * 6), ("iou_threshold", C.c_float)]


class RangeSearchDesc(C.Structure):
    _fields_ = [("channels", C.c_int32), ("candidates", C.c_int32), ("n_levels", C.c_int32), ("reserved", C.c_int32), ("per_channel", C.c_int64)]


class LssDesc(C.Structure):
    _fields_ = [("samples", C.c_int32), ("views", C.c_int32), ("depth_bins", C.c_int32), ("fh", C.c_int32), ("fw", C.c_int32),
                ("features", C.c_int32), ("nx", C.c_int32 * 3), ("dx", C.c_float * 3), ("bx", C.c_float * 3)]


class CamStemDesc(C.Structure):
    _fields_ = [("views", C.c_int32), ("h", C.c_int32), ("w", C.c_int32), ("reserved", C.c_int32), ("view_stride", C.c_int64),
                ("out_delta", C.c_float), ("out_zp", C.c_float)]


class CamHeadsDesc(C.Structure):
    _fields_ = [("views", C.c_int32), ("h", C.c_int32), ("w", C.c_int32), ("cin", C.c_int32), ("depth_bins", C.c_int32), ("features", C.c_int32),
                ("depth_delta", C.c_float), ("depth_zp", C.c_float), ("feat_delta", C.c_float), ("feat_zp", C.c_float)]


class Qv2xError(RuntimeError):
    pass


_lib = None


def load() -> C.CDLL:
    global _lib
    if _lib is not None:
        return _lib
    if not os.path.exists(LIB_PATH):
        raise Qv2xError(f"{LIB_PATH} is missing: build it with `python -c 'import __graft_entry__ as g; g.build()'` "
                        "(hipcc --offload-arch=gfx950).  There is no CPU fallback for the deployed path.")
    lib = C.CDLL(LIB_PATH)
    missing = [s for s in SYMBOLS if not hasattr(lib, s)]
    if missing:
        raise Qv2xError(f"libqv2x.so does not export {missing}")
    vp = C.c_void_p
    lib.qv2x_last_error.restype = C.c_char_p
    lib.qv2x_version.restype = C.c_int
    if lib.qv2x_version() != ABI_VERSION:
        raise Qv2xError(f"libqv2x.so has ABI {lib.qv2x_version()}, this binding mirrors ABI {ABI_VERSION} (include/qv2x.h): rebuild the library")
    lib.qv2x_fill_i8.argtypes = [vp, C.c_int64, C.c_int, vp]
    lib.qv2x_pfn_scatter_i8.argtypes = [vp, vp, vp, C.c_int, C.c_int, C.POINTER(PfnParams), vp, C.c_int, C.c_int, C.c_int, vp]
    lib.qv2x_pfn_unscatter_i8.argtypes = [vp, C.c_int, C.c_int, vp, C.c_int, C.c_int, C.c_int, vp]
    lib.qv2x_conv3x3_i8.argtypes = [C.POINTER(ConvDesc), vp, vp, vp, vp, vp, vp, vp, vp]
    lib.qv2x_conv3x3_i8_wide.argtypes = [C.POINTER(ConvDesc), vp, vp, vp, vp, vp, vp, vp, vp]
    lib.qv2x_conv3x3_i8_chain64.argtypes = [C.POINTER(ChainDesc), vp, vp, vp, vp, vp, vp, vp, vp]
    lib.qv2x_conv3x3_i8_pack_wide.argtypes = [C.POINTER(ConvDesc), vp, vp, vp]
    lib.qv2x_conv3x3_i8_wide_ok.argtypes = [C.POINTER(ConvDesc)]
    lib.qv2x_deconv_i8.argtypes = [C.POINTER(DeconvDesc), vp, vp, vp, vp, vp]
    lib.qv2x_deconv_i8_batch.argtypes = [C.POINTER(DeconvDesc), C.c_int, C.POINTER(vp), C.POINTER(vp), C.POINTER(vp), C.POINTER(vp), vp]
    lib.qv2x_codebook_level_floats.argtypes = [C.c_int]
    lib.qv2x_codebook_level_floats.restype = C.c_int64
    lib.qv2x_codebook_c2_f32.argtypes = [vp, C.c_int, vp, vp]
    lib.qv2x_codebook_encode_f32.argtypes = [C.POINTER(EncodeDesc), vp, C.POINTER(vp), vp, vp]
    lib.qv2x_codebook_encode_wave_f32.argtypes = [C.POINTER(EncodeDesc), vp, vp, C.POINTER(vp), vp, vp]
    lib.qv2x_fuse_att_f32.argtypes = [C.POINTER(FuseDesc), vp, vp, vp, vp, vp, vp, vp]
    lib.qv2x_fuse_att_batch_f32.argtypes = [C.POINTER(FuseDesc), C.c_int, C.POINTER(C.c_int64), C.POINTER(C.c_int32), vp, vp, vp, vp, vp, vp, vp]
    lib.qv2x_decode_lut_f32.argtypes = [vp, C.c_int, C.c_int, C.c_int, vp, vp, vp, vp]
    lib.qv2x_fuse_heads_batch_f32.argtypes = [C.POINTER(FuseDesc), C.c_int, C.POINTER(C.c_int64), C.POINTER(C.c_int32), vp, vp, vp, vp, vp,
                                              C.c_int, C.c_int, vp, vp, vp, vp, vp, vp, vp]
    lib.qv2x_heads_f32.argtypes = [vp, C.c_int, C.c_int, C.c_int, C.c_int, vp, vp, vp, vp, vp, vp]
    lib.qv2x_decode_heads_f32.argtypes = [vp, C.c_int, C.c_int, C.c_int, C.c_int, vp, vp, C.c_int, C.c_int, vp, vp, vp, vp, vp, vp]
    lib.qv2x_table_heads_f32.argtypes = [vp, C.c_int, C.c_int, C.c_int, C.c_int, C.c_int, C.c_int, vp, vp, vp, vp, vp, vp, vp]
    lib.qv2x_single_heads_lut_f32.argtypes = [vp, C.c_int, C.c_int, C.c_int, C.c_int, C.c_int, vp, vp, vp, vp, vp, vp]
    lib.qv2x_heads_pair_f32.argtypes = [vp, C.c_int, C.c_int, C.c_int, C.c_int, vp, vp, vp, vp, vp,
                                        vp, C.c_int, C.c_int, C.c_int, vp, vp, C.c_int, C.c_int, vp, vp, vp, vp, vp, vp]
    lib.qv2x_dequant_i8_f32.argtypes = [vp, C.c_int, C.c_int, C.c_int, C.c_int, C.c_int, C.c_float, vp, vp]
    lib.qv2x_codebook_encode_collapsed_f32.argtypes = [C.POINTER(EncodeDesc), vp, vp, vp, vp, vp, vp]
    lib.qv2x_codebook_encode_candidates_i8.argtypes = [C.POINTER(EncodeDesc), vp, vp, vp, vp, C.POINTER(C.c_float), vp, vp, vp, vp]
    lib.qv2x_codebook_encode_candidates_seg_i8.argtypes = [C.POINTER(EncodeDesc), vp, vp, vp, vp, C.POINTER(C.c_float), vp, vp, vp, vp]
    lib.qv2x_codebook_encode_listed_f32.argtypes = [C.POINTER(EncodeDesc), vp, C.POINTER(vp), vp, vp, vp, vp]
    lib.qv2x_mean_vfe_f32.argtypes = [vp, vp, vp, C.c_int, C.c_int, vp, vp]
    lib.qv2x_sp_index_scatter.argtypes = [vp, vp, C.c_int, C.c_int, C.c_int, C.c_int, C.c_int, vp, C.c_int, vp]
    lib.qv2x_sp_out_sites_workspace_bytes.argtypes = [C.POINTER(SpconvDesc)]
    lib.qv2x_sp_out_sites_workspace_bytes.restype = C.c_int64
    lib.qv2x_sp_out_sites.argtypes = [C.POINTER(SpconvDesc), vp, vp, vp, vp, vp, vp, C.c_int64, vp]
    lib.qv2x_sp_rulebook.argtypes = [C.POINTER(SpconvDesc), vp, vp, vp, vp, vp]
    lib.qv2x_sp_conv_f32in.argtypes = [C.POINTER(SpconvDesc), vp, vp, vp, vp, vp, vp, vp, vp]
    lib.qv2x_sp_conv_i8.argtypes = [C.POINTER(SpconvDesc), vp, vp, vp, vp, vp, vp, vp, vp, vp, vp, vp]
    lib.qv2x_sp_to_bev_i8.argtypes = [vp, vp, vp, C.c_int, C.c_int, C.c_int, C.c_int, C.c_int, C.c_int, C.c_int, C.c_int, vp, vp]
    lib.qv2x_voxelize_workspace_bytes.argtypes = [C.c_int]
    lib.qv2x_voxelize_workspace_bytes.restype = C.c_int64
    lib.qv2x_voxelize_f32.argtypes = [vp, C.c_int, C.POINTER(C.c_float), C.POINTER(C.c_float), C.c_int, C.c_int, C.c_int,
                                      vp, C.c_int64, vp, vp, vp, vp, vp]
    lib.qv2x_voxelize_batch_workspace_bytes.argtypes = [C.c_int, C.POINTER(C.c_int32)]
    lib.qv2x_voxelize_batch_workspace_bytes.restype = C.c_int64
    lib.qv2x_voxelize_batch_f32.argtypes = [C.POINTER(vp), C.POINTER(C.c_int32), C.c_int, C.POINTER(C.c_float), C.POINTER(C.c_float),
                                            C.c_int, C.c_int, C.c_int, vp, C.c_int64, vp, vp, vp, vp, vp]
    lib.qv2x_postprocess_batch_workspace_bytes.argtypes = [C.POINTER(PostprocessDesc), C.c_int]
    lib.qv2x_postprocess_batch_workspace_bytes.restype = C.c_int64
    lib.qv2x_postprocess_batch_f32.argtypes = [C.POINTER(PostprocessDesc), C.c_int, vp, C.c_int64, vp, C.c_int64, vp, C.c_int64, vp, vp,
                                               vp, C.c_int64, vp, vp, vp, vp, vp]
    lib.qv2x_eval_workspace_bytes.argtypes = [C.POINTER(EvalDesc)]
    lib.qv2x_eval_workspace_bytes.restype = C.c_int64
    lib.qv2x_eval_tp_fp_f32.argtypes = [C.POINTER(EvalDesc), vp, vp, vp, vp, vp, vp, vp, vp, C.c_int64, vp, vp, vp, vp, vp, vp]
    lib.qv2x_gt_boxes_f32.argtypes = [C.POINTER(GtDesc), vp, vp, vp, vp, vp, vp, vp, vp, vp, vp, vp]
    lib.qv2x_range_search_workspace_bytes.argtypes = [C.POINTER(RangeSearchDesc)]
    lib.qv2x_range_search_workspace_bytes.restype = C.c_int64
    lib.qv2x_range_search_f32.argtypes = [C.POINTER(RangeSearchDesc), vp, vp, vp, vp, vp, vp, vp]
    lib.qv2x_lss_workspace_bytes.argtypes = [C.POINTER(LssDesc)]
    lib.qv2x_lss_workspace_bytes.restype = C.c_int64
    lib.qv2x_lss_plan_f32.argtypes = [C.POINTER(LssDesc), vp, vp, vp, vp, vp, vp, vp, vp, vp]
    lib.qv2x_lss_splat_f32.argtypes = [C.POINTER(LssDesc), vp, vp, C.c_int, vp, vp, vp]
    lib.qv2x_cam_stem_f32.argtypes = [C.POINTER(CamStemDesc), vp, vp, vp, vp, vp]
    lib.qv2x_cam_heads_i8.argtypes = [C.POINTER(CamHeadsDesc), vp, vp, vp, vp, vp, vp, vp, vp, vp]
    lib.qv2x_postprocess_workspace_bytes.argtypes = [C.POINTER(PostprocessDesc)]
    lib.qv2x_postprocess_workspace_bytes.restype = C.c_int64
    lib.qv2x_postprocess_f32.argtypes = [C.POINTER(PostprocessDesc), vp, vp, vp, vp, vp, C.c_int64, vp, vp, vp, vp, vp]
    lib.qv2x_postprocess_late_workspace_bytes.argtypes = [C.POINTER(PostprocessDesc), C.c_int]
    lib.qv2x_postprocess_late_workspace_bytes.restype = C.c_int64
    lib.qv2x_postprocess_late_f32.argtypes = [C.POINTER(PostprocessDesc), C.c_int, C.POINTER(vp), C.POINTER(vp), C.POINTER(vp), C.POINTER(vp),
                                              C.POINTER(C.c_float), vp, C.c_int64, vp, vp, vp, vp, vp]
    lib.qv2x_conv3x3_f32.argtypes = [C.POINTER(F32ConvDesc), vp, vp, vp, vp, vp]
    lib.qv2x_deconv_f32.argtypes = [C.POINTER(F32ConvDesc), vp, vp, vp, vp, vp]
    lib.qv2x_pfn_scatter_f32.argtypes = [vp, vp, vp, C.c_int, C.c_int, C.POINTER(C.c_float), C.POINTER(C.c_float), C.POINTER(C.c_float),
                                         C.POINTER(C.c_float), vp, C.c_int, C.c_int, C.c_int, vp]
    lib.qv2x_codebook_encode_f32in.argtypes = [C.POINTER(EncodeDesc), vp, C.POINTER(vp), vp, vp]
    lib.qv2x_pyramid_weighted_fuse_f32.argtypes = [C.POINTER(FuseDesc), C.c_int, vp, vp, vp, vp, vp]
    lib.qv2x_pyramid_weighted_fuse_i8.argtypes = [C.POINTER(FuseDesc), C.c_int, vp, C.c_int, C.c_float, vp, vp, vp, vp]
    lib.qv2x_conv1x1_i8.argtypes = [C.POINTER(Conv1x1Desc), vp, vp, vp, vp, vp, vp, vp, vp, vp]
    lib.qv2x_gconv3x3_i8.argtypes = [C.POINTER(GconvDesc), vp, vp, vp, vp, vp, vp, vp, vp]
    lib.qv2x_conv3x3_i8_res.argtypes = [C.POINTER(ConvDesc), vp, vp, vp, vp, vp, vp, C.c_int, vp, C.c_int, C.c_float, vp, vp]
    lib.qv2x_deconv_f32in.argtypes = [C.POINTER(DeconvDesc), vp, vp, vp, vp, vp]
    lib.qv2x_codebook_decode_f32.argtypes = [vp, C.c_int64, C.c_int64, C.c_int, C.c_int, C.c_int, C.c_int, C.c_int, vp, vp, vp, vp]
    lib.qv2x_occ_score_i8.argtypes = [C.POINTER(OccDesc), vp, vp, vp, vp, vp, vp]
    lib.qv2x_codebook64_level_floats.argtypes = [C.c_int]
    lib.qv2x_codebook64_level_floats.restype = C.c_int64
    lib.qv2x_codebook64_c2_f32.argtypes = [vp, C.c_int, vp, vp]
    lib.qv2x_codebook_encode64_f32.argtypes = [C.POINTER(EncodeDesc), C.c_int, vp, C.POINTER(vp), vp, vp]
    lib.qv2x_codebook_encode64_f32in.argtypes = [C.POINTER(EncodeDesc), C.c_int, vp, C.POINTER(vp), vp, vp]
    lib.qv2x_add_relu_f32.argtypes = [vp, vp, vp, C.c_int64, vp]
    lib.qv2x_occ_sigmoid_f32.argtypes = [vp, C.c_int, C.c_int, C.c_int, C.c_int, vp, vp, vp]
    lib.qv2x_pyramid_weighted_fuse_f32p.argtypes = [C.POINTER(FuseDesc), C.c_int, vp, vp, vp, vp, vp]
    lib.qv2x_bottleneck_i8.argtypes = [C.POINTER(BottleneckDesc), vp, C.POINTER(vp), C.POINTER(vp), C.POINTER(vp), C.POINTER(vp), C.POINTER(vp), vp, vp]
    lib.qv2x_comm_unique_id.argtypes = [vp]
    lib.qv2x_comm_init.argtypes = [vp, C.c_int, C.c_int, C.POINTER(vp)]
    lib.qv2x_comm_destroy.argtypes = [vp]
    lib.qv2x_allgather_codes.argtypes = [vp, vp, vp, C.c_int64, vp]
    lib.qv2x_pairwise_from_poses_f64.argtypes = [vp, C.c_int, C.c_int64, C.c_int64, C.c_int, vp, vp]
    lib.qv2x_pairwise_from_poses_batch_f64.argtypes = [vp, C.c_int, C.c_int64, C.c_int64, C.c_int, C.c_int64, C.c_int, vp, vp]
    lib.qv2x_fuse_att_band_f32.argtypes = [C.POINTER(FuseDesc), C.c_int, C.POINTER(C.c_int64), C.POINTER(C.c_int32), vp, vp, vp, vp, vp,
                                           C.c_int64, C.c_int64, vp, vp]
    lib.qv2x_heads_band.argtypes = [vp, C.c_int, C.c_int64, C.c_int, C.c_int, vp, vp, vp, vp, C.c_int, vp, vp, vp]
    lib.qv2x_fuse_heads_band.argtypes = [C.POINTER(FuseDesc), C.c_int, C.POINTER(C.c_int64), C.POINTER(C.c_int32), vp, vp, vp, vp, vp,
                                         C.c_int64, C.c_int64, C.c_int, C.c_int, vp, vp, vp, vp, C.c_int, vp, vp, vp, vp]
    lib.qv2x_assemble_bands.argtypes = [vp, C.c_int, C.c_int64, C.c_int, C.c_int, C.c_int, C.c_int, C.c_int, vp, vp, vp, vp]
    for s in SYMBOLS:
        if s not in ("qv2x_last_error", "qv2x_codebook_level_floats", "qv2x_codebook64_level_floats", "qv2x_voxelize_workspace_bytes", "qv2x_postprocess_workspace_bytes",
                     "qv2x_postprocess_late_workspace_bytes", "qv2x_sp_out_sites_workspace_bytes", "qv2x_voxelize_batch_workspace_bytes",
                     "qv2x_postprocess_batch_workspace_bytes", "qv2x_eval_workspace_bytes", "qv2x_range_search_workspace_bytes", "qv2x_lss_workspace_bytes"):
            getattr(lib, s).restype = C.c_int
    _lib = lib
    return lib


def check(rc: int, what: str = "") -> None:
    if rc != 0:
        msg = load().qv2x_last_error().decode(errors="replace")
        raise Qv2xError(f"{what or 'libqv2x'} failed with {rc}: {msg}")


def ptr(t) -> C.c_void_p:
    if t is None:
        return C.c_void_p(0)
    if hasattr(t, "data_ptr"):
        return C.c_void_p(t.data_ptr())
    return C.c_void_p(t.ctypes.data)


def current_stream() -> C.c_void_p:
    import torch
    return C.c_void_p(torch.cuda.current_stream().cuda_stream)
```

Baseline: 6679.

## Classify refine cells by flagged level span and exit exact refine early

```diff
diff --git a/include/qv2x.h b/include/qv2x.h
--- a/include/qv2x.h
+++ b/include/qv2x.h
@@ -112,6 +112,12 @@
 int qv2x_codebook_encode_candidates_seg_i8(const qv2x_encode_desc* desc , const int8_t* in, const int8_t* g_limbs, const double* bias_packed,
                                            const int32_t* tables, const float* tau , uint8_t* codes, uint32_t* list, uint32_t* counters,
                                            void* stream);
+
+int qv2x_codebook_encode_candidates_span_i8(const qv2x_encode_desc* desc , const int8_t* in, const int8_t* g_limbs, const double* bias_packed,
+                                            const int32_t* tables, const float* tau , uint8_t* codes, uint32_t* list, uint32_t* counters,
+                                            void* stream);
+int qv2x_codebook_encode_span_f32(const qv2x_encode_desc* desc , const int8_t* in, const float* const* level_weights ,
+                                  const uint32_t* list, const uint32_t* list_count, uint8_t* codes, void* stream);
 
 typedef struct {
     int32_t agents, h, w, levels, kc;
diff --git a/quantv2x_amd/csrc/codebook_encode.h b/quantv2x_amd/csrc/codebook_encode.h
--- a/quantv2x_amd/csrc/codebook_encode.h
+++ b/quantv2x_amd/csrc/codebook_encode.h
@@ -36,7 +36,33 @@
     i0 = (tile - p.first[cls]) * 32;
 }
 
+constexpr int SPAN_CLASSES = 6;
+__device__ __host__ __forceinline__ constexpr int span_first(int k) { return k < 3 ? k : (k < 5 ? k - 3 : 0); }
+__device__ __host__ __forceinline__ constexpr int span_last(int k) { return k < 3 ? 2 : (k < 5 ? 1 : 0); }
+__device__ __host__ __forceinline__ constexpr int span_class(int first, int last) { return last == 2 ? first : (last == 1 ? 3 + first : 5); }
+struct SpanPlan { int pre[SPAN_CLASSES + 1], total, full; };
+__device__ __forceinline__ SpanPlan span_plan(const EncArgs& a) {
+    SpanPlan p;
+    p.pre[0] = 0;
+#pragma unroll
+    for (int k = 0; k < SPAN_CLASSES; ++k) p.pre[k + 1] = p.pre[k] + (int)a.list_count[1 + k];
+    p.total = (p.pre[SPAN_CLASSES] + 31) >> 5;
+    const int full = p.total / a.list_slots * a.list_slots;
+    p.full = p.total - full > a.list_tail_max ? p.total : full;
+    return p;
+}
+__device__ __forceinline__ int span_cell(const SpanPlan& p, const EncArgs& a, int i, int& cls) {
+    i = i < p.pre[SPAN_CLASSES] ? i : p.pre[SPAN_CLASSES] - 1;
+    int base = 0;
+    cls = 0;
+#pragma unroll
+    for (int k = 1; k < SPAN_CLASSES; ++k)
+        if (i >= p.pre[k]) { cls = k; base = p.pre[k]; }
+    return (int)a.list[(size_t)cls * a.M + (i - base)];
+}
+
 int encode_wave_launch(const EncArgs& a, hipStream_t st);
 int encode_wave_list_launch(const EncArgs& a, int waves, hipStream_t st);
+int encode_wave_span_launch(const EncArgs& a, int waves, hipStream_t st);
 
 }
diff --git a/quantv2x_amd/csrc/codebook_encode.hip b/quantv2x_amd/csrc/codebook_encode.hip
--- a/quantv2x_amd/csrc/codebook_encode.hip
+++ b/quantv2x_amd/csrc/codebook_encode.hip
@@ -102,9 +102,9 @@
 constexpr int ENC_MAX_TILES = 16;
 template <int ER> constexpr int enc_smem_floats() { return 2 * ER * LDF + 4 * ER + 4 * ER + 2 * ENC_MAX_TILES * ER + 4 * ER + QV2X_ENC_LDS_PAD; }
 
-template <int ER, bool EXT, bool LIST = false>
+template <int ER, bool EXT, bool LIST = false, bool SPAN = false>
 __device__ __forceinline__ void encode_rows(const EncArgs& a, const int m0, float* __restrict__ smem, const unsigned* __restrict__ lst = nullptr,
-                                            const int n_listed = 0, const int start = 0) {
+                                            const int n_listed = 0, const int start = 0, const int exitl = -1, int* differs = nullptr) {
     constexpr int ERT = ER / 32;
     const int segs = EXT ? a.segs : 1;
     float* bufA = smem;
@@ -305,12 +305,17 @@
                 const int bi = (int)(unsigned)bk;
                 code_s[sg * ER + tid] = bi;
                 if (LIST) {
-                    if (m0 + tid < n_listed) a.codes[((size_t)l * segs + sg) * a.M + lst[m0 + tid]] = (uint8_t)(bi - sg * a.kc);
+                    if (m0 + tid < n_listed) {
+                        uint8_t* at = a.codes + ((size_t)l * segs + sg) * a.M + lst[m0 + tid];
+                        if (SPAN && l <= exitl && (int)*at != bi - sg * a.kc) *differs = 1;
+                        *at = (uint8_t)(bi - sg * a.kc);
+                    }
                 } else if (m0 + tid < a.m_hi) a.codes[((size_t)l * segs + sg) * a.M + m0 + tid] = (uint8_t)(bi - sg * a.kc);
             }
         }
         lds_barrier();
         EFINE(9);
+        if (SPAN && l == exitl && !*differs) break;
         }
 
         if (l + 1 < a.levels) {
@@ -359,6 +364,29 @@
 }
 
 template <bool EXT>
+__global__ __launch_bounds__(512, 2) void codebook_encode_span_tail_kernel(const EncArgs a) {
+    __shared__ __attribute__((aligned(16))) float smem[enc_smem_floats<32>()];
+    __shared__ unsigned cells[32];
+    __shared__ int span[2], differs;
+    const SpanPlan plan = span_plan(a);
+    for (int t = plan.full + (int)blockIdx.x; t < plan.total; t += (int)gridDim.x) {
+        if (threadIdx.x < 64) {
+            int cls;
+            const unsigned cell = (unsigned)span_cell(plan, a, t * 32 + ((int)threadIdx.x & 31), cls);
+            const int f = span_first(cls), e = span_last(cls);
+            const int start = __builtin_amdgcn_ballot_w64(f == 0) ? 0 : (__builtin_amdgcn_ballot_w64(f == 1) ? 1 : 2);
+            const int exitl = __builtin_amdgcn_ballot_w64(e == 2) ? 2 : (__builtin_amdgcn_ballot_w64(e == 1) ? 1 : 0);
+            if (threadIdx.x < 32) cells[threadIdx.x] = cell;
+            if (threadIdx.x == 0) { span[0] = start; span[1] = exitl; differs = 0; }
+        }
+        __syncthreads();
+        const int n = plan.pre[SPAN_CLASSES] - t * 32;
+        encode_rows<32, EXT, true, true>(a, 0, smem, cells, n < 32 ? n : 32, span[0], span[1], &differs);
+        __syncthreads();
+    }
+}
+
+template <bool EXT>
 __global__ __launch_bounds__(512, 2) void codebook_encode_mixed_kernel(const EncArgs a, const int n64) {
     __shared__ __attribute__((aligned(16))) float smem[enc_smem_floats<64>()];
     if ((int)blockIdx.x < n64) encode_rows<64, EXT>(a, a.m_lo + blockIdx.x * 64, smem);
@@ -408,10 +436,24 @@
     return encode_launch(d, (const int8_t*)in, in, level_weights, codes, stream);
 }
 
+static int encode_listed(const bool span, const qv2x_encode_desc* d, const int8_t* in, const float* const* level_weights,
+                         const uint32_t* list, const uint32_t* list_count, uint8_t* codes, void* stream);
+
 extern "C" int qv2x_codebook_encode_listed_f32(const qv2x_encode_desc* d, const int8_t* in, const float* const* level_weights,
                                                const uint32_t* list, const uint32_t* list_count, uint8_t* codes, void* stream) {
+    return encode_listed(false, d, in, level_weights, list, list_count, codes, stream);
+}
+
+extern "C" int qv2x_codebook_encode_span_f32(const qv2x_encode_desc* d, const int8_t* in, const float* const* level_weights,
+                                             const uint32_t* list, const uint32_t* list_count, uint8_t* codes, void* stream) {
+    if (d && d->levels > 3) return qv2x::fail(QV2X_EINVAL, "qv2x_codebook_encode_span_f32: up to three levels (the span lists have no class beyond level 2)");
+    return encode_listed(true, d, in, level_weights, list, list_count, codes, stream);
+}
+
+static int encode_listed(const bool span, const qv2x_encode_desc* d, const int8_t* in, const float* const* level_weights,
+                         const uint32_t* list, const uint32_t* list_count, uint8_t* codes, void* stream) {
     using namespace qv2x;
-    if (!d || !in || !level_weights || !codes || !list || !list_count) return fail(QV2X_EINVAL, "qv2x_codebook_encode_listed_f32: null pointer");
+    if (!d ||!in || !level_weights || !codes || !list || !list_count) return fail(QV2X_EINVAL, "qv2x_codebook_encode_listed_f32: null pointer");
     if (d->n <= 0 || d->h <= 0 || d->w <= 0 || d->levels < 1 || d->levels > 4) return fail(QV2X_EINVAL, "qv2x_codebook_encode_listed_f32: bad shape");
     const int segs = d->segs ? d->segs : 1;
     if (segs != 1 && segs != 2) return fail(QV2X_EINVAL, "qv2x_codebook_encode_listed_f32: seg_num 1 or 2 (got %d)", d->segs);
@@ -439,11 +481,14 @@
     a.list_slots = 4 * cus; a.list_tail_max = tail_knob > 0 ? tail_knob : 2 * cus;
     const int grid_tail = 2 * cus;
     if (tiles + 3 >= 2 * a.list_slots) {
-        if (int rc = encode_wave_list_launch(a, a.list_slots, (hipStream_t)stream)) return rc;
+        if (int rc = span ? encode_wave_span_launch(a, a.list_slots, (hipStream_t)stream) : encode_wave_list_launch(a, a.list_slots, (hipStream_t)stream)) return rc;
     } else {
         a.list_slots = 1 << 30; a.list_tail_max = 1 << 30;
     }
-    if (ext) codebook_encode_list_tail_kernel<true><<<tiles < grid_tail ? tiles : grid_tail, 512, 0, (hipStream_t)stream>>>(a);
+    if (span) {
+        if (ext) codebook_encode_span_tail_kernel<true><<<tiles < grid_tail ? tiles : grid_tail, 512, 0, (hipStream_t)stream>>>(a);
+        else codebook_encode_span_tail_kernel<false><<<tiles < grid_tail ? tiles : grid_tail, 512, 0, (hipStream_t)stream>>>(a);
+    } else if (ext) codebook_encode_list_tail_kernel<true><<<tiles < grid_tail ? tiles : grid_tail, 512, 0, (hipStream_t)stream>>>(a);
     else codebook_encode_list_tail_kernel<false><<<tiles < grid_tail ? tiles : grid_tail, 512, 0, (hipStream_t)stream>>>(a);
     return hip_check(hipGetLastError(), "qv2x_codebook_encode_listed_f32 launch");
 }
diff --git a/quantv2x_amd/csrc/codebook_encode_cand.hip b/quantv2x_amd/csrc/codebook_encode_cand.hip
--- a/quantv2x_amd/csrc/codebook_encode_cand.hip
+++ b/quantv2x_amd/csrc/codebook_encode_cand.hip
@@ -21,8 +21,11 @@
     return __builtin_bit_cast(double, ((long long)hi << 32) | (unsigned)lo);
 }
 
-template <int CT, int SEGS, int PACK>
+__device__ __forceinline__ int span_class(int first, int last) { return last == 2 ? first : (last == 1 ? 3 + first : 5); }
+
+template <int CT, int SEGS, int PACK, bool SPAN = false>
 __global__ __launch_bounds__(256) __attribute__((amdgpu_waves_per_eu(1, 1))) void encode_candidates_kernel(const CandArgs a) {
+    constexpr int NC = SPAN ? 6 : 3;
     const int lane = threadIdx.x & 63, wave = __builtin_amdgcn_readfirstlane(threadIdx.x >> 6), j = lane & 31, hf = lane >> 5;
     const int m0 = ((int)blockIdx.x * 4 + wave) * (32 * CT);
 
@@ -66,6 +69,7 @@
     const __amdgpu_buffer_rsrc_t trs = __builtin_amdgcn_make_buffer_rsrc((void*)a.tables, 0, a.tbytes, 0x00020000);
     int o[2][SEGS][CT] = {};
     int first[CT];
+    int lastw[SPAN ? CT : 1];
 #pragma unroll
     for (int ct = 0; ct < CT; ++ct) first[ct] = 3;
     const int ntile = a.kc >> 5;
@@ -155,56 +159,69 @@
         segment(IC<0>{});
         if constexpr (SEGS > 1) segment(IC<1>{});
 #pragma unroll
-        for (int ct = 0; ct < CT; ++ct)
+        for (int ct = 0; ct < CT; ++ct) {
             if (weak_l[ct] && first[ct] == 3) first[ct] = l;
+            if constexpr (SPAN) lastw[ct] = (weak_l[ct] || l == 0) ? l : lastw[ct];
+        }
     };
     level(IC<0>{});
     if (a.levels > 1) level(IC<1>{});
     if (a.levels > 2) level(IC<2>{});
-    unsigned long long mask[3][CT];
-    unsigned cnt[3] = {0, 0, 0};
-#pragma unroll
-    for (int c = 0; c < 3; ++c)
-#pragma unroll
-        for (int ct = 0; ct < CT; ++ct) {
-            mask[c][ct] = __builtin_amdgcn_ballot_w64(first[ct] == c && hf == 0 && m[ct] < a.M);
+    int cls[CT];
+#pragma unroll
+    for (int ct = 0; ct < CT; ++ct) {
+        if constexpr (SPAN) cls[ct] = first[ct] == 3 ? NC : span_class(first[ct], lastw[ct]);
+        else cls[ct] = first[ct] == 3 ? NC : first[ct];
+    }
+    unsigned long long mask[NC][CT];
+    unsigned cnt[NC];
+#pragma unroll
+    for (int c = 0; c < NC; ++c) {
+        cnt[c] = 0;
+#pragma unroll
+        for (int ct = 0; ct < CT; ++ct) {
+            mask[c][ct] = __builtin_amdgcn_ballot_w64(cls[ct] == c && hf == 0 && m[ct] < a.M);
             cnt[c] += (unsigned)__builtin_popcountll(mask[c][ct]);
         }
-    __shared__ unsigned wcnt[4][3], wbase[3];
-    if (lane == 0) { wcnt[wave][0] = cnt[0]; wcnt[wave][1] = cnt[1]; wcnt[wave][2] = cnt[2]; }
+    }
+    __shared__ unsigned wcnt[4][NC], wbase[NC];
+    if (lane == 0) {
+#pragma unroll
+        for (int c = 0; c < NC; ++c) wcnt[wave][c] = cnt[c];
+    }
     __syncthreads();
-    if (threadIdx.x < 3) {
+    if (threadIdx.x < NC) {
         const unsigned tot = wcnt[0][threadIdx.x] + wcnt[1][threadIdx.x] + wcnt[2][threadIdx.x] + wcnt[3][threadIdx.x];
         wbase[threadIdx.x] = tot ? atomicAdd(a.counters + 1 + threadIdx.x, tot) : 0u;
         if (tot) atomicAdd(a.counters, tot);
     }
     __syncthreads();
-    unsigned base[3];
-#pragma unroll
-    for (int c = 0; c < 3; ++c) {
+    unsigned base[NC];
+#pragma unroll
+    for (int c = 0; c < NC; ++c) {
         base[c] = wbase[c];
         for (int w2 = 0; w2 < wave; ++w2) base[c] += wcnt[w2][c];
     }
 #pragma unroll
-    for (int c = 0; c < 3; ++c) {
+    for (int c = 0; c < NC; ++c) {
         unsigned at = __builtin_amdgcn_readfirstlane(base[c]);
 #pragma unroll
         for (int ct = 0; ct < CT; ++ct) {
-            if (first[ct] == c && hf == 0 && m[ct] < a.M)
+            if (cls[ct] == c && hf == 0 && m[ct] < a.M)
                 a.list[(size_t)c * a.M + at + (unsigned)__builtin_popcountll(mask[c][ct] & ((1ull << lane) - 1ull))] = (unsigned)m[ct];
             at += (unsigned)__builtin_popcountll(mask[c][ct]);
         }
     }
 }
 
-__global__ void zero_counters_kernel(unsigned* c) { if (threadIdx.x < 4) c[threadIdx.x] = 0; }
-
-template <int CT, int SEGS, int PACK>
+__global__ void zero_counters_kernel(unsigned* c, int n) { if ((int)threadIdx.x < n) c[threadIdx.x] = 0; }
+
+template <int CT, int SEGS, int PACK, bool SPAN>
 void launch(const CandArgs& a, hipStream_t st) {
-    encode_candidates_kernel<CT, SEGS, PACK><<<(a.M + 128 * CT - 1) / (128 * CT), 256, 0, st>>>(a);
-}
-
-template <int PACK, int MAX_SEGS>
+    encode_candidates_kernel<CT, SEGS, PACK, SPAN><<<(a.M + 128 * CT - 1) / (128 * CT), 256, 0, st>>>(a);
+}
+
+template <int PACK, int MAX_SEGS, bool SPAN = false>
 int candidates(const char* me, const qv2x_encode_desc* d, const int8_t* in, const int8_t* g_limbs, const double* bias_packed, const int32_t* tables,
                const float* tau, uint8_t* codes, uint32_t* list, uint32_t* counters, void* stream) {
     if (!d || !in || !g_limbs || !bias_packed || !tau || !codes || !list || !counters) return fail(QV2X_EINVAL, "%s: null pointer", me);
@@ -226,12 +243,12 @@
     a.tbytes = (d->levels > 1 ? d->levels * (d->levels - 1) / 2 : 1) * a.ke * a.ke * 4;
     a.delta = d->in_delta;
     hipStream_t st = (hipStream_t)stream;
-    zero_counters_kernel<<<1, 64, 0, st>>>(counters);
+    zero_counters_kernel<<<1, 64, 0, st>>>(counters, SPAN ? 8 : 4);
     int dev = 0, cus = 256, v = 0;
     if (hipGetDevice(&dev) == hipSuccess && hipDeviceGetAttribute(&v, hipDeviceAttributeMultiprocessorCount, dev) == hipSuccess && v > 0) cus = v;
     const bool large = a.M >= 4 * cus * 32 * (segs == 2 ? 3 : 4) * 2;
-    if (segs == 1) large ? launch<4, 1, PACK>(a, st) : launch<2, 1, PACK>(a, st);
-    else if constexpr (MAX_SEGS > 1) large ? launch<3, 2, PACK>(a, st) : launch<2, 2, PACK>(a, st);
+    if (segs == 1) large ? launch<4, 1, PACK, SPAN>(a, st) : launch<2, 1, PACK, SPAN>(a, st);
+    else if constexpr (MAX_SEGS > 1) large ? launch<3, 2, PACK, SPAN>(a, st) : launch<2, 2, PACK, SPAN>(a, st);
     return hip_check(hipGetLastError(), me);
 }
 
@@ -249,3 +266,12 @@
                                                       void* stream) {
     return qv2x::candidates<256, 2>("qv2x_codebook_encode_candidates_seg_i8", d, in, g_limbs, bias_packed, tables, tau, codes, list, counters, stream);
 }
+
+extern "C" int qv2x_codebook_encode_candidates_span_i8(const qv2x_encode_desc* d, const int8_t* in, const int8_t* g_limbs, const double* bias_packed,
+                                                       const int32_t* tables, const float* tau, uint8_t* codes, uint32_t* list, uint32_t* counters,
+                                                       void* stream) {
+    const char* me = "qv2x_codebook_encode_candidates_span_i8";
+    if (d && (d->segs ? d->segs : 1) == 1 && d->kc <= 128)
+        return qv2x::candidates<128, 1, true>(me, d, in, g_limbs, bias_packed, tables, tau, codes, list, counters, stream);
+    return qv2x::candidates<256, 2, true>(me, d, in, g_limbs, bias_packed, tables, tau, codes, list, counters, stream);
+}
diff --git a/quantv2x_amd/csrc/codebook_encode_wave.hip b/quantv2x_amd/csrc/codebook_encode_wave.hip
--- a/quantv2x_amd/csrc/codebook_encode_wave.hip
+++ b/quantv2x_amd/csrc/codebook_encode_wave.hip
@@ -48,21 +48,32 @@
 
 template <int V> struct IC { static constexpr int value = V; };
 
-template <bool F32IN, int SEGS, bool LIST = false>
+template <bool F32IN, int SEGS, bool LIST = false, bool SPAN = false>
 __global__ __attribute__((amdgpu_flat_work_group_size(64, 64), amdgpu_waves_per_eu(1, 1))) void codebook_encode_wave_kernel(const EncArgs a) {
+    static_assert(LIST || !SPAN, "the span form is a list form");
     __shared__ __attribute__((aligned(16))) float smem[32 * RS];
     const int lane = threadIdx.x, j = lane & 31, h = lane >> 5;
     float* const row = smem + j * RS;
     ListPlan plan{};
-    if (LIST) plan = list_plan(a);
+    SpanPlan splan{};
+    if (LIST && !SPAN) plan = list_plan(a);
+    if (SPAN) { splan = span_plan(a); plan.full = splan.full; }
 #pragma unroll 1
     for (int round = 0; LIST ? round * (int)gridDim.x < plan.full : round == 0; ++round) {
     const int tile = LIST ? round * (int)gridDim.x + ((round & 1) ? (int)gridDim.x - 1 - (int)blockIdx.x : (int)blockIdx.x) : (int)blockIdx.x;
     if (LIST && tile >= plan.full) continue;
     int mrow;
     bool owned;
+    int exitl = -1;
     int start = 0;
-    if (LIST) {
+    if constexpr (SPAN) {
+        int cls;
+        mrow = span_cell(splan, a, tile * 32 + j, cls);
+        owned = tile * 32 + j < splan.pre[SPAN_CLASSES];
+        const int f = span_first(cls), e = span_last(cls);
+        start = __builtin_amdgcn_ballot_w64(f == 0) ? 0 : (__builtin_amdgcn_ballot_w64(f == 1) ? 1 : 2);
+        exitl = __builtin_amdgcn_ballot_w64(e == 2) ? 2 : (__builtin_amdgcn_ballot_w64(e == 1) ? 1 : 0);
+    } else if (LIST) {
         int cls, i0;
         list_tile(plan, tile, cls, i0);
         owned = i0 + j < plan.n[cls];
@@ -104,6 +115,7 @@
         }
     }
 
+    bool differs = false;
     for (int l = 0; l < a.levels; ++l) {
         const float* W = a.lvl[l];
         const float* stage_b = W + D * D;
@@ -210,6 +222,11 @@
 #pragma unroll
             for (int sg = 0; sg < SEGS; ++sg) bcs |= (unsigned)a.codes[((size_t)l * SEGS + sg) * a.M + mrow] << (8 * sg);
         } else {
+        unsigned cand = 0;
+        if (SPAN && l <= exitl) {
+#pragma unroll
+            for (int sg = 0; sg < SEGS; ++sg) cand |= (unsigned)a.codes[((size_t)l * SEGS + sg) * a.M + mrow] << (8 * sg);
+        }
 #pragma unroll 1
         for (int P = 0; P < 4; ++P) {
             tile2(z, true, [&]() __attribute__((always_inline)) { if (P < 3) next_vec(qhead_b, P + 1); else if (SEGS == 1) next_c2(0); else next_c2s(0, 1, 0); });
@@ -324,9 +341,11 @@
             if constexpr (SEGS == 2) seg_pairs(IC<0>{}, IC<1>{}, false);
             else { seg_pairs(IC<0>{}, IC<1>{}, true); seg_pairs(IC<2>{}, IC<3>{}, false); }
         }
+        if (SPAN && l <= exitl) differs |= bcs != cand;
         }
         WFINE(5);
         if (last) break;
+        if (SPAN && l == exitl && !__builtin_amdgcn_ballot_w64(differs)) break;
 #pragma unroll 1
         for (int P = 0; P < 4; ++P) {
             const int seg = (P * a.segs) >> 2;
@@ -371,6 +390,13 @@
     return hip_check(hipGetLastError(), "qv2x_codebook_encode_listed_f32 launch");
 }
 
+int encode_wave_span_launch(const EncArgs& a, int waves, hipStream_t st) {
+    if ((a.segs != 1 && a.segs != 2) || a.in_f32) return fail(QV2X_EINVAL, "qv2x_codebook_encode_span_f32: seg_num 1 | 2, i8 rows");
+    if (a.segs == 2) codebook_encode_wave_kernel<false, 2, true, true><<<(unsigned)waves, 64, 0, st>>>(a);
+    else codebook_encode_wave_kernel<false, 1, true, true><<<(unsigned)waves, 64, 0, st>>>(a);
+    return hip_check(hipGetLastError(), "qv2x_codebook_encode_span_f32 launch");
+}
+
 }
 
 #ifdef QV2X_ENCW_FINE
diff --git a/quantv2x_amd/encode_two_stage.py b/quantv2x_amd/encode_two_stage.py
--- a/quantv2x_amd/encode_two_stage.py
+++ b/quantv2x_amd/encode_two_stage.py
@@ -172,3 +172,40 @@
             flags[p] = (P * second + k2) - (P * best + out[p]) <= P * np.ceil(t) + (P - 1.0)
             gaps[p] = (second - best) * h
     return out, flags.any(0), flags, gaps
+
+
+SPAN_CLASSES = ((0, 2), (1, 2), (2, 2), (0, 1), (1, 1), (0, 0))
+
+
+def span_cost(first: int, last: int) -> float:
+    return 2.0 * first + 2.5 * (last - first + 1) + (last - first)
+
+
+def span_classes(flags: np.ndarray, segs: int = 1):
+    lev = flags.reshape(flags.shape[0] // segs, segs, -1).any(1)
+    levels = lev.shape[0]
+    listed = lev.any(0)
+    first = np.where(listed, lev.argmax(0), -1)
+    last = np.where(listed, levels - 1 - lev[::-1].argmax(0), -1)
+    cls = np.full(first.shape, -1)
+    for k, (f, e) in enumerate(SPAN_CLASSES):
+        cls[(first == f) & (last == e)] = k
+    return first, last, cls
+
+
+def span_rule(cand: np.ndarray, flags: np.ndarray, chain: np.ndarray, segs: int = 1):
+    levels = cand.shape[0] // segs
+    first, last, _ = span_classes(flags, segs)
+    out = cand.copy()
+    exited = np.zeros(cand.shape[1], bool)
+    work = before = 0.0
+    for r in np.nonzero(first >= 0)[0]:
+        f, e = int(first[r]), int(last[r])
+        span = slice(f * segs, (e + 1) * segs)
+        out[span, r] = chain[span, r]
+        exited[r] = bool((chain[span, r] == cand[span, r]).all())
+        if not exited[r]:
+            out[(e + 1) * segs:, r] = chain[(e + 1) * segs:, r]
+        before += span_cost(f, levels - 1)
+        work += span_cost(f, e if exited[r] else levels - 1)
+    return out, exited, work, before
diff --git a/quantv2x_amd/engine.py b/quantv2x_amd/engine.py
--- a/quantv2x_amd/engine.py
+++ b/quantv2x_amd/engine.py
@@ -777,6 +777,7 @@
         self._collapsed, self._two_stage, self.two_stage_refused = None, None, None
         self.encode_form = "auto"
         self.encode_mode = "two_stage" if self.two_stage_supported() else "exact"
+        self.encode_span = True
 
     def _padded(self, n, h, w, c, q):
         t = torch.empty((n, h + 2, w + 2, c), dtype=torch.int8, device=self.dev)
@@ -826,6 +827,8 @@
                 self._build_two_stage()
             b["enc_list"] = torch.zeros(3 * n * hw, dtype=torch.int32, device=self.dev)
             b["enc_counters"] = torch.zeros(4, dtype=torch.int32, device=self.dev)
+            b["enc_span_list"] = torch.zeros(6 * n * hw, dtype=torch.int32, device=self.dev)
+            b["enc_span_counters"] = torch.zeros(8, dtype=torch.int32, device=self.dev)
         if not self.has_codebook or self.heads_single is not None:
             b["feats"] = torch.empty((n, hw, 256), dtype=torch.float32, device=self.dev)
         self._bufs[n] = b
@@ -1048,6 +1051,13 @@
 
     def _encode_two_stage(self, d, b, codes):
         gp, bias, tab, tau, _ = self._two_stage
+        if self.encode_span:
+            L.check(self.lib.qv2x_codebook_encode_candidates_span_i8(C.byref(d), L.ptr(b["s1"]), L.ptr(gp), L.ptr(bias), L.ptr(tab), tau, L.ptr(codes),
+                                                                     L.ptr(b["enc_span_list"]), L.ptr(b["enc_span_counters"]), L.current_stream()),
+                    "qv2x_codebook_encode_candidates_span_i8")
+            L.check(self.lib.qv2x_codebook_encode_span_f32(C.byref(d), L.ptr(b["s1"]), self.level_ptrs, L.ptr(b["enc_span_list"]),
+                                                           L.ptr(b["enc_span_counters"]), L.ptr(codes), L.current_stream()), "qv2x_codebook_encode_span_f32")
+            return codes
         name = self.candidate_entry()
         L.check(getattr(self.lib, name)(C.byref(d), L.ptr(b["s1"]), L.ptr(gp), L.ptr(bias), L.ptr(tab), tau, L.ptr(codes),
                                         L.ptr(b["enc_list"]), L.ptr(b["enc_counters"]), L.current_stream()), name)
@@ -1059,8 +1069,14 @@
         if not (self.encode_mode == "two_stage" and self.encode_form == "auto") or "enc_counters" not in self._bufs.get(n_agents, {}):
             raise L.Qv2xError(f"encode_refine_stats({n_agents}): no two-stage encode of {n_agents} frames here (encode_mode "
                               f"{self.encode_mode!r}, encode_form {self.encode_form!r}, workspaces {sorted(self._bufs)})")
+        cells = n_agents * self.fh * self.fw
+        if self.encode_span:
+            from .encode_two_stage import SPAN_CLASSES
+            c = self._bufs[n_agents]["enc_span_counters"].cpu().numpy().astype(np.int64)
+            first = [int(sum(c[1 + k] for k, (f, _) in enumerate(SPAN_CLASSES) if f == l)) for l in range(self.enc_levels)]
+            return {"cells": cells, "refined": int(c[0]), "refined_fraction": float(c[0]) / cells, "first_flagged_at_level": first,
+                    "undecided_span": {f"{f}-{e}": int(c[1 + k]) for k, (f, e) in enumerate(SPAN_CLASSES)}}
         c = self._bufs[n_agents]["enc_counters"].cpu().numpy().astype(np.int64)
-        cells = n_agents * self.fh * self.fw
         return {"cells": cells, "refined": int(c[0]), "refined_fraction": float(c[0]) / cells, "first_flagged_at_level": [int(v) for v in c[1:1 + self.enc_levels]]}
 
     def encode_into(self, inputs: dict, frames: int, codes_out: torch.Tensor):
diff --git a/quantv2x_amd/lib.py b/quantv2x_amd/lib.py
--- a/quantv2x_amd/lib.py
+++ b/quantv2x_amd/lib.py
@@ -20,7 +20,7 @@
     "qv2x_codebook64_level_floats", "qv2x_codebook64_c2_f32", "qv2x_codebook_encode64_f32", "qv2x_codebook_encode64_f32in",
     "qv2x_add_relu_f32", "qv2x_occ_sigmoid_f32", "qv2x_pyramid_weighted_fuse_f32p", "qv2x_bottleneck_i8",
     "qv2x_comm_unique_id", "qv2x_comm_init", "qv2x_comm_destroy", "qv2x_allgather_codes", "qv2x_pairwise_from_poses_f64", "qv2x_pairwise_from_poses_batch_f64",
-    "qv2x_codebook_encode_collapsed_f32", "qv2x_codebook_encode_candidates_i8", "qv2x_codebook_encode_candidates_seg_i8", "qv2x_codebook_encode_listed_f32", "qv2x_mean_vfe_f32", "qv2x_sp_index_scatter", "qv2x_sp_out_sites_workspace_bytes", "qv2x_sp_out_sites", "qv2x_sp_rulebook", "qv2x_sp_conv_f32in", "qv2x_sp_conv_i8", "qv2x_sp_to_bev_i8",
+    "qv2x_codebook_encode_collapsed_f32", "qv2x_codebook_encode_candidates_i8", "qv2x_codebook_encode_candidates_seg_i8", "qv2x_codebook_encode_listed_f32", "qv2x_codebook_encode_candidates_span_i8", "qv2x_codebook_encode_span_f32", "qv2x_mean_vfe_f32", "qv2x_sp_index_scatter", "qv2x_sp_out_sites_workspace_bytes", "qv2x_sp_out_sites", "qv2x_sp_rulebook", "qv2x_sp_conv_f32in", "qv2x_sp_conv_i8", "qv2x_sp_to_bev_i8",
     "qv2x_fuse_att_band_f32", "qv2x_heads_band", "qv2x_fuse_heads_band", "qv2x_assemble_bands",
     "qv2x_voxelize_batch_workspace_bytes", "qv2x_voxelize_batch_f32", "qv2x_postprocess_batch_workspace_bytes", "qv2x_postprocess_batch_f32",
     "qv2x_eval_workspace_bytes", "qv2x_eval_tp_fp_f32", "qv2x_gt_boxes_f32",
@@ -196,6 +196,8 @@
     lib.qv2x_codebook_encode_candidates_i8.argtypes = [C.POINTER(EncodeDesc), vp, vp, vp, vp, C.POINTER(C.c_float), vp, vp, vp, vp]
     lib.qv2x_codebook_encode_candidates_seg_i8.argtypes = [C.POINTER(EncodeDesc), vp, vp, vp, vp, C.POINTER(C.c_float), vp, vp, vp, vp]
     lib.qv2x_codebook_encode_listed_f32.argtypes = [C.POINTER(EncodeDesc), vp, C.POINTER(vp), vp, vp, vp, vp]
+    lib.qv2x_codebook_encode_candidates_span_i8.argtypes = [C.POINTER(EncodeDesc), vp, vp, vp, vp, C.POINTER(C.c_float), vp, vp, vp, vp]
+    lib.qv2x_codebook_encode_span_f32.argtypes = [C.POINTER(EncodeDesc), vp, C.POINTER(vp), vp, vp, vp, vp]
     lib.qv2x_mean_vfe_f32.argtypes = [vp, vp, vp, C.c_int, C.c_int, vp, vp]
     lib.qv2x_sp_index_scatter.argtypes = [vp, vp, C.c_int, C.c_int, C.c_int, C.c_int, C.c_int, vp, C.c_int, vp]
     lib.qv2x_sp_out_sites_workspace_bytes.argtypes = [C.POINTER(SpconvDesc)]
```

Result: faster. 7022, median of 6 (+5.1%).
